# JianCao92/speaker-diarization

Measured on AMD Instinct MI355X. Metric: diarized audio throughput (CD gw/BIC + CL hi/BIC), higher is better.
Workload: dtype f64

## Files before the change

### include/spkd.h

```cpp
#ifndef SPKD_H
#define SPKD_H

#include <stddef.h>
#include <stdint.h>

#ifdef __cplusplus
extern "C" {
#endif

#define SPKD_ABI_VERSION 2
#define SPKD_DIM 39
#define SPKD_REC 820

typedef enum {
    SPKD_OK = 0,
    SPKD_EINVAL = 1,
    SPKD_EHIP = 2,
    SPKD_ENONFINITE = 3,
    SPKD_EOVERFLOW = 4,
    SPKD_ENOMEM = 5
} spkd_status;

typedef enum { SPKD_BIC = 0, SPKD_GLR = 1, SPKD_KL2 = 2, SPKD_KL2_PINV = 3 } spkd_kind;

// ... 73 lines not shown
                    int32_t *h_n_win, double *h_win_maxd, int32_t *h_win_det,
                    double *h_det_start, double *h_det_maxi, double *h_det_d,
                    double *h_final_start,
                    spkd_cand_log *h_log, int64_t log_cap, int64_t *h_log_count);

spkd_status spkd_gw_ex(spkd_ctx *ctx, const float *d_frames, int64_t n_frames,
                       const int64_t *h_turn_begin, const int64_t *h_turn_end, int64_t n_turns,
                       const spkd_cd_params *params, const int64_t *h_ev_off, int check_capacity,
                       int32_t *h_n_win, double *h_win_maxd, int32_t *h_win_det,
                       double *h_det_start, double *h_det_maxi, double *h_det_d,
                       double *h_final_start,
                       spkd_cand_log *h_log, int64_t log_cap, int64_t *h_log_count);

spkd_status spkd_gw_fused(spkd_ctx *ctx, const float *d_frames, int64_t n_frames,
                          const int64_t *h_turn_begin, const int64_t *h_turn_end, int64_t n_turns,
                          const spkd_cd_params *params, const int64_t *h_ev_off, int check_capacity,
                          int32_t *h_n_win, double *h_win_maxd, int32_t *h_win_det,
                          double *h_det_start, double *h_det_maxi, double *h_det_d,
                          double *h_final_start, double *d_seg_stats,
                          spkd_cand_log *h_log, int64_t log_cap, int64_t *h_log_count);

spkd_status spkd_gather_stats(spkd_ctx *ctx, const double *d_src, int64_t n_src,
                              const int64_t *h_src_index, const int64_t *h_dst_index,
                              int64_t n, int64_t n_dst, double *d_dst);

typedef struct {
    int64_t n_lines;
    int64_t n_redo;
    const int32_t *n_win;
    const double *times;
    const int32_t *turn;
    const int64_t *frame_b;
    const int64_t *frame_e;
    const int64_t *index;
    const int64_t *d_index;
    const int64_t *redo_line;
    const int64_t *redo_begin;
    const int64_t *redo_end;
} spkd_gw_lines_view;

spkd_status spkd_gw_batch(spkd_ctx *ctx, const float *d_frames, int64_t n_frames,
                          const int64_t *h_turn_begin, const int64_t *h_turn_end, int64_t n_turns,
                          const spkd_cd_params *params, const int64_t *h_ev_off,
                          const double *h_turn_start_s, const double *h_turn_end_s,
                          const int64_t *h_turn_file_off, const int64_t *h_turn_file_len,
                          double *d_seg_stats, int want_index, spkd_gw_lines_view *view);

int64_t spkd_sw_window_count(int64_t turn_len, double winsize, double winstep);
spkd_status spkd_sw(spkd_ctx *ctx, const float *d_frames, int64_t n_frames,
                    const int64_t *h_turn_begin, const int64_t *h_turn_end, int64_t n_turns,
                    const spkd_cd_params *params, const int64_t *h_d_off, double *h_d);

enum { SPKD_AHC_AUTO = 0, SPKD_AHC_MONO = 1, SPKD_AHC_WIDE = 2 };

typedef struct {
    int32_t variant;
    int32_t kind;
    int32_t max_spk;
    int32_t path;
    double lambdac;
    double threshold;
} spkd_ahc_params;

spkd_status spkd_ahc(spkd_ctx *ctx, const double *d_stats, const int64_t *h_seg_off,
                     int64_t n_problems, const spkd_ahc_params *params,
                     int32_t *h_n_merges, int32_t *h_merge_a, int32_t *h_merge_b,
                     double *h_merge_d, double *h_stat_max, double *h_stat_min);

spkd_status spkd_ahc_matrix(spkd_ctx *ctx, const double *d_stats, int64_t n, const spkd_ahc_params *params,
                            const double *d_matrix, double stat_max_in, double stat_min_in,
                            int32_t *h_n_merges, int32_t *h_merge_a, int32_t *h_merge_b,
                            double *h_merge_d, double *h_stat_max, double *h_stat_min);

spkd_status spkd_ahc_fused(spkd_ctx *ctx, const float *d_frames, int64_t n_frames,
                           const double *d_records, int64_t n_records, int64_t *d_line_index,
                           const int64_t *h_seg_off, int64_t n_problems,
                           const int64_t *h_redo_line, const int64_t *h_redo_begin,
                           const int64_t *h_redo_end, int64_t n_redo,
                           const spkd_ahc_params *params,
                           const int32_t **h_n_merges, const int32_t **h_merge_a,
                           const int32_t **h_merge_b, const double **h_merge_d,
                           const int32_t **h_labels);

typedef struct {
    int32_t sample_rate, frame_rate, window_width, n_fft, n_mel, n_cep;
    int32_t cms_left, cms_right;
    int32_t delta_width[2];
    float pre_emph;
    float delta_norm[2];
} spkd_mfcc_params;
spkd_status spkd_mfcc(spkd_ctx *ctx, const int16_t *d_pcm, int64_t n_samples,
                      const spkd_mfcc_params *params, const float *h_melfb, const float *h_dct,
                      const float *h_mean, const float *h_scale, const float *h_transform,
                      float *d_features, int64_t *h_n_frames);

typedef struct {
    int32_t n_kernels, n_states, dim;
    const float *mean;
    const float *inv_var;
    const float *log_norm;
    const int32_t *state_off;
    const int32_t *kernel;
    const float *log_weight;
} spkd_gmm_params;
spkd_status spkd_gmm_loglik(spkd_ctx *ctx, const float *d_features, int64_t n_frames,
                            const spkd_gmm_params *params, float *d_scores);

void spkd_py2_roundtrip(double *h_values, int64_t n);
spkd_status spkd_labels_from_merges(int64_t n, int64_t n_merges, const int32_t *h_a,
                                    const int32_t *h_b, int32_t *h_labels);
spkd_status spkd_labels_from_merges_batch(int64_t n_problems, const int64_t *h_seg_off,
                                          const int32_t *h_n_merges, const int32_t *h_a,
                                          const int32_t *h_b, int32_t *h_labels);

spkd_status spkd_count_flags(const int32_t *h_flags, const int64_t *h_off, const int32_t *h_n,
                             int64_t n_groups, int32_t *h_out);

spkd_status spkd_gw_lines(int64_t n_turns, const int64_t *h_off, const int32_t *h_n_det,
                          const double *h_det_start, const double *h_det_maxi,
                          const double *h_final_start, const double *h_turn_start_s,
                          const double *h_turn_end_s, const int64_t *h_turn_begin,
                          const int64_t *h_turn_end, double rate, int text_contract,
                          int64_t n_lines, double *h_times, int64_t *h_frame_b,
                          int64_t *h_frame_e, int64_t *h_index, int32_t *h_line_turn);

spkd_status spkd_vad_viterbi(int64_t n_frames, int32_t n_states, const float *h_scores,
                             int32_t n_words, const int32_t *h_word_state, const double *h_stay,
                             const double *h_exit, const double *h_enter, int64_t *h_tok_frame,
                             int32_t *h_tok_word, int64_t *h_n_tokens, double *h_score);

#ifdef __cplusplus
}
#endif
#endif
```

### speaker-diarization_amd/csrc/spkd_cluster.hpp

```cpp
#pragma once
#include "spkd_device.hpp"
#include "spkd_quad.hpp"
#include "spkd_tri.hpp"
#include "../../include/spkd.h"

namespace spkd {

constexpr double MAXINT_F = 9223372036854775808.0;
constexpr double PEN_UNIT = 39.0 + 0.5 * 39.0 * 40.0;
constexpr int AUX = 3 * DA;
constexpr int ERR_DEGENERATE_MERGE = 2;

__device__ __forceinline__ unsigned long long dkey(double v) {
    unsigned long long b = (unsigned long long)__double_as_longlong(v);
    return (b >> 63) ? ~b : (b | 0x8000000000000000ull);
}
__device__ __forceinline__ double dkey_inv(unsigned long long k) {
    unsigned long long b = (k >> 63) ? (k & 0x7fffffffffffffffull) : ~k;
    return __longlong_as_double((long long)b);
}
template <bool MAXOP>
__device__ __forceinline__ unsigned wave_red_u32(unsigned x) {
    auto op = [](unsigned a, unsigned b) { return MAXOP ? (a > b ? a : b) : (a < b ? a : b); };
    x = op(x, (unsigned)__builtin_amdgcn_update_dpp((int)x, (int)x, 0xB1, 0xf, 0xf, false));
// ... 271 lines not shown
    const int lane = lane_id();
    const int64_t pair = (int64_t)blockIdx.x * PT2_WAVES + wave;
    if (pair >= n_pairs) return;
    double* ldsA = slabs[wave][0];
    double* ldsB = slabs[wave][1];
    const double* A = stats + (int64_t)ia[pair] * REC;
    const double* B = stats + (int64_t)ib[pair] * REC;
    const double n1 = A[REC - 1], n2 = B[REC - 1];
    const double n = n1 + n2;
    const QuadLane L = quad_lane();
    int ta = L.t;
    asm volatile("" : "+v"(ta));
    QuadRows q;
    double sc[QS];
    quad_load_packed(B, ta, q, sc);
    quad_from_packed_lds(ldsA, A, lane);
    quad_from_packed_lds(ldsB, B, lane);
    const bool want_glr = (flags & SPKD_WANT_GLR) != 0;
    const int mode = (L.m == 3 && !want_glr) ? 2 : L.m;
    double wa, wc, k1a, k1c, w1, k2c, w2;
    {
        const double fA = 1.0 / (n1 - 1.0), fB = 1.0 / (n2 - 1.0), fU = 1.0 / (n - 1.0);
        const double al1 = (n1 / n) / (n1 - 1.0), al2 = (n2 / n) / (n2 - 1.0);
        wa = mode == 0 ? fA : (mode == 1 ? 0.0 : (mode == 2 ? fU : al1));
        wc = mode == 0 ? 0.0 : (mode == 1 ? fB : (mode == 2 ? fU : al2));
        k1a = mode == 1 ? 0.0 : 1.0;
        k1c = (mode == 1 || mode == 2) ? 1.0 : 0.0;
        w1 = mode == 0 ? -(fA / n1) : (mode == 1 ? -(fB / n2) : (mode == 2 ? -(fU / n) : -(al1 / n1)));
        k2c = mode == 3 ? 1.0 : 0.0;
        w2 = mode == 3 ? -(al2 / n2) : 0.0;
    }
    double v1[QS], v2[QS], c1[QS], c2[QS];
#pragma unroll
    for (int s = 0; s < QS; ++s) {
#pragma unroll
        for (int j = 0; j < tri_cols(s); ++j)
            q.r[s][j] = fma(wa, ldsA[(s * DA + j) * 16 + ta], wc * q.r[s][j]);
        const double sa = ldsA[(s * DA + D) * 16 + ta];
        v1[s] = fma(k1c, sc[s], k1a * sa);
        v2[s] = k2c * sc[s];
        c1[s] = w1 * v1[s];
        c2[s] = w2 * v2[s];
        __builtin_amdgcn_sched_barrier(0);
    }
    TriRank1<0>::run(q, c1, v1);
    TriRank1<0>::run(q, c2, v2);
    auto form_single = [&](int mi, double (&a)[DA]) {
        const int md = (mi == 3 && !want_glr) ? 2 : mi;
        if (md == 0) single_pair_matrix(SPKD_BIC, ldsA, ldsA, true, a);
        else if (md == 1) single_pair_matrix(SPKD_BIC, ldsB, ldsB, true, a);
        else single_pair_matrix(md == 2 ? SPKD_BIC : SPKD_GLR, ldsA, ldsB, false, a);
    };
    const double ld = log(tri_det(q, L.m, err, form_single));
    double res[4];
#pragma unroll
    for (int mi = 0; mi < 4; ++mi) res[mi] = __shfl(ld, 16 * mi);
    double kl = __builtin_nan("");
    if (flags & SPKD_WANT_KL2) {
        double* slab = ldsA;
        double a[DA];
        double ds[2], dp[2], mu[2];
#pragma unroll 1
        for (int t = 0; t < 2; ++t) {
            stage1(slab, t ? B : A);
            row_from_slab(slab, a);
            const double nn = t ? n2 : n1;
            const double mean_i = a[D] / nn;
            cov_rows(a, nn);
            kl2_lane_terms(a, mean_i, ds[t], dp[t], mu[t], pinv_ws);
        }
        kl = kl2_combine(ds[0], dp[0], mu[0], ds[1], dp[1], mu[1]);
    }
    if (lane == 0) {
        double* o = out + pair * 8;
        o[0] = n1; o[1] = n2; o[2] = res[0]; o[3] = res[1]; o[4] = res[2];
        o[5] = want_glr ? res[3] : __builtin_nan("");
        o[6] = kl; o[7] = 0.0;
    }
}

__global__ __launch_bounds__(PT_WAVES * WAVE) void k_cluster_prep(
        const double* __restrict__ qr, int64_t n_rec, int kind,
        double* __restrict__ ld, double* __restrict__ aux, int* err,
        double* pinv_ws) {
    const int wave = threadIdx.x >> 6;
    const int64_t w = (int64_t)blockIdx.x * PT_WAVES + wave;
    if (kind == SPKD_KL2) {
        if (w >= n_rec) return;
        const double* R = qr + w * QREC;
        double a[DA];
        single_rows_from_qr(R, a);
        const double n = qr_count(R);
        const double mean_i = a[D] / n;
        cov_rows(a, n);
        kl2_aux_from_cov(a, mean_i, aux + w * AUX, pinv_ws);
        if (lane_id() == 0) ld[w] = 0.0;
        return;
    }
    if (w * 4 >= n_rec) return;
    const QuadLane L = quad_lane();
    const double* recs[4];
    bool selfs[4];
#pragma unroll
    for (int mi = 0; mi < 4; ++mi) {
        int64_t c = w * 4 + mi;
        c = c < n_rec ? c : n_rec - 1;
        recs[mi] = qr + c * QREC;
        selfs[mi] = true;
    }
    int64_t c = w * 4 + L.m;
    const bool valid = c < n_rec;
    c = valid ? c : n_rec - 1;
    const double* R = qr + c * QREC;
    QuadRows q;
    double sv[QS];
    const double nR = qr_count(R), fR = fast_recip(nR - 1.0);
    quad_load_scaled(R, L.t, fR, q, sv);
    double c1[QS];
    const double gR = -(fR * fast_recip(nR));
#pragma unroll
    for (int s = 0; s < QS; ++s) c1[s] = gR * sv[s];
    TriRank1<0>::run(q, c1, sv);
    auto form_single = [&](int mi, double (&a)[DA]) { single_pair_matrix(kind, recs[mi], recs[mi], true, a); };
    const double v = tri_logdet(q, L.m, err, form_single);
    if (valid && L.t == 0) ld[c] = v;
}

__device__ __forceinline__ double finish_distance(int kind, double lambdac, double nA, double ldA,
                                                  double nC, double ldC, double ldx) {
#pragma clang fp contract(off)
    const double n = nA + nC;
    if (kind == SPKD_BIC) {
        double d = 0.5 * n * ldx - 0.5 * nA * ldA - 0.5 * nC * ldC;
        d -= lambdac * 0.5 * PEN_UNIT * log(n);
        return d;
    }
    return -(n / 2.0) * ((nA / n) * ldA + (nC / n) * ldC - ldx);
}

__device__ __forceinline__ int find_problem(const int64_t* __restrict__ seg_off, int64_t n_prob, int64_t g) {
    int64_t lo = 0, hi = n_prob;
    while (hi - lo > 1) {
        int64_t mid = (lo + hi) >> 1;
        if (seg_off[mid] <= g) lo = mid; else hi = mid;
    }
    return (int)lo;
}

#ifndef SPKD_MX_WAVES
#define SPKD_MX_WAVES 4
#endif
constexpr int MX_WAVES = SPKD_MX_WAVES;

template <bool TWO>
__global__ __launch_bounds__(MX_WAVES * WAVE, 2) void k_matrix(
        const double* __restrict__ ex, const double* __restrict__ pk, const int64_t* __restrict__ seg_off,
        const int32_t* __restrict__ rec_prob, const int32_t* __restrict__ sched, int variant, int kind, double lambdac,
        const double* __restrict__ ld, const double* __restrict__ aux,
        double* __restrict__ mat, const int64_t* __restrict__ mat_off,
        unsigned long long* stat_max, unsigned long long* stat_min, int* err) {
    __shared__ double ldsA[QREC];
    const int64_t g = sched[blockIdx.x];
    if (g < 0) return;
    const int p = rec_prob[g];
    const int64_t off = seg_off[p];
    const int64_t N = seg_off[p + 1] - off;
    const int64_t ra = g - off;
// ... 1053 lines not shown
```

### speaker-diarization_amd/csrc/spkd_handoff.hpp

```cpp
#pragma once
#include "spkd_cd.hpp"
#include "spkd_cluster.hpp"
#include "spkd_device.hpp"

namespace spkd {

__host__ __device__ inline int32_t count_detections(const int32_t* flags, int64_t n_win) {
    int32_t cnt = 0;
    for (int64_t i = 0; i < n_win; ++i) cnt += flags[i] != 0;
    return cnt;
}

struct RecipeLine {
    double start_s, end_s;
    int64_t frame_b, frame_e;
    int64_t index;
};

__host__ __device__ inline RecipeLine recipe_line(int64_t begin, int64_t len, int64_t ev_off, int64_t j, int64_t nd,
                                                  const double* det_start, const double* det_maxi,
                                                  const double* final_start, double ls, double le, double rate) {
#pragma clang fp contract(off)
    RecipeLine L;
    const bool tail = j == nd;
    double fs, fe;
    if (tail) {
        fs = *final_start;
        L.start_s = fs / rate + ls;
        L.end_s = ((le - ls) * rate) / rate + ls;
        fe = 0.0;
    } else {
        fs = det_start[ev_off + j];
        fe = fs + det_maxi[ev_off + j];
        L.start_s = fs / rate + ls;
        L.end_s = fe / rate + ls;
    }
    L.frame_b = begin + (int64_t)fs;
    L.frame_e = tail ? begin + len : begin + (int64_t)fe;
    L.index = ev_off + j;
    return L;
}

constexpr int CP_TPB = 256;
constexpr int CP_SCAN_TPB = 1024;

__global__ __launch_bounds__(CP_TPB) void k_cp_count(const TurnDesc* __restrict__ turns, int64_t n_turns,
                                                     const int32_t* __restrict__ n_win,
                                                     const int32_t* __restrict__ win_det, const int* __restrict__ err,
                                                     int32_t* __restrict__ n_det, int32_t* __restrict__ pos) {
    if (*err) return;
    const int64_t p = (int64_t)blockIdx.x * CP_TPB + threadIdx.x;
    if (p >= n_turns) return;
    const TurnDesc T = turns[p];
    int64_t nw = n_win[T.id];
    nw = nw < 0 ? 0 : (nw > T.ev_cap ? T.ev_cap : nw);
    n_det[T.id] = count_detections(win_det + T.ev_off, nw);
    pos[T.id] = (int32_t)p;
}

__global__ __launch_bounds__(CP_SCAN_TPB) void k_cp_scan(const int32_t* __restrict__ n_det, int64_t n_turns,
                                                         const int* __restrict__ err, int64_t* __restrict__ line_off) {
    __shared__ int64_t part[CP_SCAN_TPB];
    const int tid = threadIdx.x;
    if (*err) {
        if (tid == 0) line_off[n_turns] = 0;
        return;
    }
    const int64_t per = (n_turns + CP_SCAN_TPB - 1) / CP_SCAN_TPB;
    const int64_t lo = tid * per < n_turns ? tid * per : n_turns;
    const int64_t hi = lo + per < n_turns ? lo + per : n_turns;
    int64_t sum = 0;
    for (int64_t t = lo; t < hi; ++t) sum += (int64_t)n_det[t] + 1;
    part[tid] = sum;
    __syncthreads();
    for (int d = 1; d < CP_SCAN_TPB; d <<= 1) {
        const int64_t v = tid >= d ? part[tid - d] : 0;
        __syncthreads();
        part[tid] += v;
        __syncthreads();
    }
    int64_t run = part[tid] - sum;
    for (int64_t t = lo; t < hi; ++t) {
        line_off[t] = run;
        run += (int64_t)n_det[t] + 1;
    }
    if (tid == CP_SCAN_TPB - 1) line_off[n_turns] = part[tid];
}

__global__ __launch_bounds__(CP_TPB) void k_cp_lines(const TurnDesc* __restrict__ turns, int64_t n_turns,
                                                     const int32_t* __restrict__ n_det, const int32_t* __restrict__ pos,
                                                     const int64_t* __restrict__ line_off, int64_t n_lines,
                                                     const double* __restrict__ det_start,
                                                     const double* __restrict__ det_maxi,
                                                     const double* __restrict__ final_start,
                                                     const double* __restrict__ turn_start_s,
                                                     const double* __restrict__ turn_end_s, double rate,
                                                     const int* __restrict__ err, double* __restrict__ times,
                                                     int64_t* __restrict__ frame_b, int64_t* __restrict__ frame_e,
                                                     int64_t* __restrict__ index, int32_t* __restrict__ line_turn) {
    if (*err) return;
    const int64_t t = (int64_t)blockIdx.x * CP_TPB + threadIdx.x;
    if (t >= n_turns) return;
    const TurnDesc T = turns[pos[t]];
    const int64_t nd = n_det[t];
    const double ls = turn_start_s[t], le = turn_end_s[t];
    int64_t i = line_off[t];
    for (int64_t j = 0; j <= nd && i < n_lines; ++j, ++i) {
        const RecipeLine L = recipe_line(T.begin, T.len, T.ev_off, j, nd, det_start, det_maxi, final_start + t, ls, le, rate);
        times[2 * i] = L.start_s;
        times[2 * i + 1] = L.end_s;
        frame_b[i] = L.frame_b;
        frame_e[i] = L.frame_e;
        index[i] = L.index;
        line_turn[i] = (int32_t)t;
    }
}

__global__ __launch_bounds__(256) void k_patch_map(const int64_t* __restrict__ line, int64_t n, int64_t* __restrict__ map) {
    const int64_t k = (int64_t)blockIdx.x * 256 + threadIdx.x;
    if (k < n) map[line[k]] = -(k + 1);
}

__global__ __launch_bounds__(256) void k_records_from_map(const double* __restrict__ recs, int64_t n_recs,
                                                          const int64_t* __restrict__ map,
                                                          const double* __restrict__ redo, int64_t n_redo,
                                                          int64_t n_rec, double* __restrict__ qr,
                                                          double* __restrict__ packed, int* __restrict__ err) {
    const int64_t c = blockIdx.x;
    if (c >= n_rec) return;
    const int64_t m = map[c];
    const double* g;
    if (m >= 0 && m < n_recs) {
        g = recs + m * REC;
    } else if (m < 0 && -(m + 1) < n_redo) {
        g = redo + (-(m + 1)) * REC;
    } else {
        if (threadIdx.x == 0) atomicOr(err, 4);
        return;
    }
    quadrec_from_packed(g, qr + c * QREC, threadIdx.x);
    double* p = packed + c * REC;
    for (int e = threadIdx.x; e < REC; e += 256) p[e] = g[e];
}

__global__ __launch_bounds__(256) void k_gather_records(const double* __restrict__ src, const int64_t* __restrict__ si,
                                                        const int64_t* __restrict__ di, int64_t n,
                                                        double* __restrict__ dst) {
    const int64_t i = blockIdx.x;
    if (i >= n) return;
    const double2* s = reinterpret_cast<const double2*>(src + si[i] * REC);
    double2* d = reinterpret_cast<double2*>(dst + (di ? di[i] : i) * REC);
    for (int e = threadIdx.x; e < REC / 2; e += 256) d[e] = s[e];
}

__global__ __launch_bounds__(256) void k_take_pair_distance(const double* __restrict__ mat, int64_t n, double* __restrict__ out) {
    const int64_t p = (int64_t)blockIdx.x * 256 + threadIdx.x;
    if (p < n) out[p] = mat[4 * p + 1];
}

}
```

### speaker-diarization_amd/csrc/spkd_hip.hip

```cpp
#include <hip/hip_runtime.h>

#include <algorithm>
#include <cmath>
#include <cstdio>
#include <cstdlib>
#include <cstring>
#include <string>
#include <atomic>
#include <thread>
#include <vector>

#include "../../include/spkd.h"
#include "spkd_cd.hpp"
#include "spkd_cluster.hpp"
#include "spkd_device.hpp"
#include "spkd_handoff.hpp"
#include "spkd_stats.hpp"
#include "spkd_mfcc.hpp"
#include "spkd_vad.hpp"

using namespace spkd;

namespace {
constexpr int N_SLOTS = 40;
enum { PIN_GW_TURNS = 0, PIN_GW_LINES, PIN_AHC_OUT, N_PIN };
}

struct spkd_ctx {
    int device = 0;
    hipStream_t stream = nullptr;
    bool own_stream = false;
    bool gw_lds_ok = false;
    int gw_waves = 0;
    unsigned long long init_keys[2] = {0ull, ~0ull};
    int step_waves = 0;
    int step_partners = 0;
    int64_t last_gw_items = 0;
    std::string err;
    int* d_err = nullptr;
    unsigned long long* d_counter = nullptr;
    hipEvent_t ev0 = nullptr, ev1 = nullptr;
    float last_ms = 0.f;
    hipEvent_t ka[SPKD_N_TIMERS] = {}, kb[SPKD_N_TIMERS] = {};
    bool kused[SPKD_N_TIMERS] = {};
    float kms[SPKD_N_TIMERS] = {};
    void* slot[N_SLOTS] = {};
    size_t slot_bytes[N_SLOTS] = {};
    void* pinv_ws = nullptr;
    double* pinv_cur = nullptr;
    void* pin[N_PIN] = {};
    size_t pin_bytes[N_PIN] = {};
    std::vector<int64_t> redo_line, redo_begin, redo_end;
    std::vector<Chunk> redo_chunks;
    std::vector<int64_t> redo_setoff;
    std::vector<int32_t> redo_sets;
};

namespace {

spkd_status fail(spkd_ctx* c, spkd_status s, const std::string& msg) {
    if (c) c->err = msg;
    return s;
}

#define HIPCHK(c, call)                                                              \
    do {                                                                             \
        hipError_t e_ = (call);                                                      \
        if (e_ != hipSuccess)                                                        \
            return fail((c), SPKD_EHIP, std::string(#call) + ": " + hipGetErrorString(e_)); \
    } while (0)

#define TRY(expr) do { const spkd_status s_ = (expr); if (s_ != SPKD_OK) return s_; } while (0)

spkd_status scratch(spkd_ctx* c, int slot, size_t bytes, void** out) {
    if (bytes == 0) bytes = 16;
    if (c->slot_bytes[slot] < bytes) {
        if (c->slot[slot]) HIPCHK(c, hipFree(c->slot[slot]));
        c->slot[slot] = nullptr;
        c->slot_bytes[slot] = 0;
        size_t want = bytes + bytes / 4;
        hipError_t e = hipMalloc(&c->slot[slot], want);
        if (e != hipSuccess) {
            want = bytes;
            e = hipMalloc(&c->slot[slot], want);
        }
        if (e != hipSuccess) return fail(c, SPKD_ENOMEM, "scratch allocation failed");
        c->slot_bytes[slot] = want;
    }
    *out = c->slot[slot];
    return SPKD_OK;
}

spkd_status pinned(spkd_ctx* c, int which, size_t bytes, void** out) {
    if (bytes == 0) bytes = 16;
    if (c->pin_bytes[which] < bytes) {
        if (c->pin[which]) HIPCHK(c, hipHostFree(c->pin[which]));
        c->pin[which] = nullptr;
        c->pin_bytes[which] = 0;
        const size_t want = bytes + bytes / 4;
        if (hipHostMalloc(&c->pin[which], want, hipHostMallocDefault) != hipSuccess) {
            c->pin[which] = nullptr;
            return fail(c, SPKD_ENOMEM, "pinned host allocation failed");
        }
        c->pin_bytes[which] = want;
    }
    *out = c->pin[which];
    return SPKD_OK;
}

template <class T>
spkd_status upload(spkd_ctx* c, int slot, const T* h, size_t n, T** d) {
    void* p = nullptr;
    TRY(scratch(c, slot, n * sizeof(T), &p));
    if (n) HIPCHK(c, hipMemcpyAsync(p, h, n * sizeof(T), hipMemcpyHostToDevice, c->stream));
    *d = (T*)p;
    return SPKD_OK;
}

struct Call {
    spkd_ctx* const c;
    spkd_status opened;
    int herr = 0;
    bool drained = false;
    explicit Call(spkd_ctx* ctx) : c(ctx) { opened = open(); }
    ~Call() { if (!drained) (void)hipStreamSynchronize(c->stream); }
    spkd_status open() {
        HIPCHK(c, hipSetDevice(c->device));
        for (int i = 0; i < SPKD_N_TIMERS; ++i) c->kused[i] = false;
        HIPCHK(c, hipMemsetAsync(c->d_err, 0, sizeof(int), c->stream));
        HIPCHK(c, hipEventRecord(c->ev0, c->stream));
        return SPKD_OK;
    }

    spkd_status finish() {
        HIPCHK(c, hipEventRecord(c->ev1, c->stream));
        HIPCHK(c, hipMemcpyAsync(&herr, c->d_err, sizeof(int), hipMemcpyDeviceToHost, c->stream));
        HIPCHK(c, hipStreamSynchronize(c->stream));
        drained = true;
        HIPCHK(c, hipEventElapsedTime(&c->last_ms, c->ev0, c->ev1));
        c->kms[0] = c->last_ms;
        for (int i = 1; i < SPKD_N_TIMERS; ++i)
            if (c->kused[i]) HIPCHK(c, hipEventElapsedTime(&c->kms[i], c->ka[i], c->kb[i]));
        if (herr & ERR_SWEEP) return fail(c, SPKD_EHIP, "internal error: growing-window sweep order");
        if (herr & 4) return fail(c, SPKD_EOVERFLOW, "device scratch capacity exceeded");
        if (herr & ERR_DEGENERATE_MERGE) return fail(c, SPKD_EINVAL, "degenerate merge: a diagonal cell was the minimum");
        if (herr & ERR_NONFINITE) return fail(c, SPKD_ENONFINITE, "array must not contain infs or NaNs");
        return SPKD_OK;
    }
};

spkd_status use_kind(spkd_ctx* c, int kind, int* base) {
    c->pinv_cur = nullptr;
    *base = kind;
    if (kind != SPKD_KL2_PINV) return SPKD_OK;
    *base = SPKD_KL2;
    if (!c->pinv_ws) {
        if (hipMalloc(&c->pinv_ws, PINV_WS_BYTES) != hipSuccess) {
            c->pinv_ws = nullptr;
            return fail(c, SPKD_ENOMEM, "pinv workspace allocation failed");
        }
        HIPCHK(c, hipMemsetAsync(c->pinv_ws, 0, PINV_LOCK_BYTES, c->stream));
    }
    c->pinv_cur = (double*)c->pinv_ws;
    return SPKD_OK;
}

struct Timer {
    spkd_ctx* const c;
    const int idx;
    Timer(spkd_ctx* ctx, int i) : c(ctx), idx(i) { (void)hipEventRecord(c->ka[idx], c->stream); }
    ~Timer() { (void)hipEventRecord(c->kb[idx], c->stream); c->kused[idx] = true; }
};

enum {
    S_CHUNKS = 0, S_SETOFF, S_PARTIAL, S_IDXA, S_IDXB, S_TERMS, S_TURNS, S_SNAP, S_CAND,
    S_EV_I32A, S_EV_I32B, S_EV_D0, S_EV_D1, S_EV_D2, S_EV_D3, S_EV_D4, S_LOG,
    S_AHC_STATS, S_AHC_LD, S_AHC_AUX, S_AHC_MAT, S_AHC_MISC, S_AHC_OUT, S_AHC_OFF, S_AHC_PROB, S_AHC_PACKED, S_MFCC_TAB, S_MFCC_STATIC,
    S_STEP_EXM, S_STEP_PKM, S_STEP_MISC, S_GMM_TAB, S_GMM_IDX,
    S_CP_TURNS, S_CP_TIMES, S_CP_LINES, S_REDO_STATS, S_REDO_IDX, S_COUNT
};
static_assert(S_COUNT <= N_SLOTS, "scratch slot table too small");

}

extern "C" {

int spkd_abi_version(void) { return SPKD_ABI_VERSION; }

static spkd_status create_ctx(int device, void* stream, bool borrow, spkd_ctx** out) {
    if (!out) return SPKD_EINVAL;
    *out = nullptr;
    int count = 0;
    if (hipGetDeviceCount(&count) != hipSuccess || device < 0 || device >= count) return SPKD_EHIP;
    spkd_ctx* c = new spkd_ctx();
    c->device = device;
    if (hipSetDevice(device) != hipSuccess) { delete c; return SPKD_EHIP; }
    if (borrow) {
        c->stream = (hipStream_t)stream;
    } else {
        if (hipStreamCreateWithFlags(&c->stream, hipStreamDefault) != hipSuccess) { delete c; return SPKD_EHIP; }
        c->own_stream = true;
    }
    if (hipMalloc(&c->d_err, sizeof(int)) != hipSuccess ||
        hipMalloc(&c->d_counter, 2 * sizeof(unsigned long long)) != hipSuccess ||
        hipEventCreate(&c->ev0) != hipSuccess || hipEventCreate(&c->ev1) != hipSuccess) {
        spkd_destroy(c);
        return SPKD_EHIP;
    }
    for (int i = 0; i < SPKD_N_TIMERS; ++i)
        if (hipEventCreate(&c->ka[i]) != hipSuccess || hipEventCreate(&c->kb[i]) != hipSuccess) {
            spkd_destroy(c);
            return SPKD_EHIP;
        }
    int lds_max = 0;
    c->gw_lds_ok = hipDeviceGetAttribute(&lds_max, hipDeviceAttributeMaxSharedMemoryPerBlock, device) == hipSuccess &&
                   Gw<4>::LDS_BYTES <= lds_max &&
                   hipFuncSetAttribute((const void*)k_gw<8>, hipFuncAttributeMaxDynamicSharedMemorySize, Gw<8>::LDS_BYTES) == hipSuccess &&
                   hipFuncSetAttribute((const void*)k_gw<4>, hipFuncAttributeMaxDynamicSharedMemorySize, Gw<4>::LDS_BYTES) == hipSuccess &&
                   hipFuncSetAttribute((const void*)k_gw<2>, hipFuncAttributeMaxDynamicSharedMemorySize, Gw<2>::LDS_BYTES) == hipSuccess &&
                   hipFuncSetAttribute((const void*)k_gw<1>, hipFuncAttributeMaxDynamicSharedMemorySize, Gw<1>::LDS_BYTES) == hipSuccess;
    if (const char* e = getenv("SPKD_GW_WAVES")) c->gw_waves = atoi(e);
    if (const char* e = getenv("SPKD_STEP_WAVES")) { const int v = atoi(e); c->step_waves = (v == 4 || v == 8) ? v : 0; }
    if (const char* e = getenv("SPKD_STEP_PARTNERS")) { const int v = atoi(e); c->step_partners = (v == 3 || v == 7 || v == 15) ? v : 0; }
    *out = c;
    return SPKD_OK;
}

spkd_status spkd_create(int device, void* stream, spkd_ctx** out) {
    return create_ctx(device, stream, stream != nullptr, out);
}

spkd_status spkd_create_on_stream(int device, void* stream, spkd_ctx** out) {
    return create_ctx(device, stream, true, out);
}

void spkd_destroy(spkd_ctx* c) {
    if (!c) return;
    (void)hipSetDevice(c->device);
    if (c->stream) (void)hipStreamSynchronize(c->stream);
    for (int i = 0; i < N_SLOTS; ++i)
        if (c->slot[i]) (void)hipFree(c->slot[i]);
    if (c->d_err) (void)hipFree(c->d_err);
    if (c->pinv_ws) (void)hipFree(c->pinv_ws);
    for (int i = 0; i < N_PIN; ++i)
        if (c->pin[i]) (void)hipHostFree(c->pin[i]);
    if (c->d_counter) (void)hipFree(c->d_counter);
    if (c->ev0) (void)hipEventDestroy(c->ev0);
    if (c->ev1) (void)hipEventDestroy(c->ev1);
    for (int i = 0; i < SPKD_N_TIMERS; ++i) {
        if (c->ka[i]) (void)hipEventDestroy(c->ka[i]);
        if (c->kb[i]) (void)hipEventDestroy(c->kb[i]);
    }
    if (c->own_stream && c->stream) (void)hipStreamDestroy(c->stream);
    delete c;
}

const char* spkd_last_error(const spkd_ctx* c) { return c ? c->err.c_str() : "null context"; }

spkd_status spkd_sync(spkd_ctx* c) {
    if (!c) return SPKD_EINVAL;
    HIPCHK(c, hipStreamSynchronize(c->stream));
    return SPKD_OK;
}

spkd_status spkd_malloc(spkd_ctx* c, size_t bytes, void** d_ptr) {
    if (!c || !d_ptr) return SPKD_EINVAL;
    HIPCHK(c, hipSetDevice(c->device));
    hipError_t e = hipMalloc(d_ptr, bytes ? bytes : 16);
    if (e != hipSuccess) return fail(c, SPKD_ENOMEM, hipGetErrorString(e));
    return SPKD_OK;
}

spkd_status spkd_free(spkd_ctx* c, void* d_ptr) {
    if (!c) return SPKD_EINVAL;
    HIPCHK(c, hipFree(d_ptr));
    return SPKD_OK;
}

spkd_status spkd_memcpy_h2d(spkd_ctx* c, void* d_dst, const void* h_src, size_t bytes) {
    if (!c) return SPKD_EINVAL;
    HIPCHK(c, hipMemcpyAsync(d_dst, h_src, bytes, hipMemcpyHostToDevice, c->stream));
    HIPCHK(c, hipStreamSynchronize(c->stream));
    return SPKD_OK;
}

spkd_status spkd_memcpy_d2h(spkd_ctx* c, void* h_dst, const void* d_src, size_t bytes) {
    if (!c) return SPKD_EINVAL;
    HIPCHK(c, hipMemcpyAsync(h_dst, d_src, bytes, hipMemcpyDeviceToHost, c->stream));
    HIPCHK(c, hipStreamSynchronize(c->stream));
    return SPKD_OK;
}

spkd_status spkd_memcpy_d2d(spkd_ctx* c, void* d_dst, const void* d_src, size_t bytes) {
    if (!c) return SPKD_EINVAL;
    HIPCHK(c, hipMemcpyAsync(d_dst, d_src, bytes, hipMemcpyDeviceToDevice, c->stream));
    HIPCHK(c, hipStreamSynchronize(c->stream));
    return SPKD_OK;
}

spkd_status spkd_last_gw_items(spkd_ctx* c, int64_t* items) {
    if (!c || !items) return SPKD_EINVAL;
    *items = c->last_gw_items;
    return SPKD_OK;
}

spkd_status spkd_last_kernel_ms(spkd_ctx* c, int which, float* ms) {
    if (!c || !ms || which < 0 || which >= SPKD_N_TIMERS) return SPKD_EINVAL;
    *ms = c->kms[which];
    return SPKD_OK;
}

namespace {
spkd_status set_stats_launch(spkd_ctx* c, const float* d_frames, int64_t n_frames,
                             const int64_t* h_begin, const int64_t* h_end, const int32_t* h_set,
                             int64_t n_ranges, int64_t n_sets, double* d_stats,
                             std::vector<Chunk>& chunks, std::vector<int64_t>& set_off) {
    chunks.clear();
    set_off.assign((size_t)n_sets + 1, 0);
    int32_t prev = 0;
    for (int64_t r = 0; r < n_ranges; ++r) {
        const int64_t b = h_begin[r], e = h_end[r];
        const int32_t s = h_set[r];
        if (b < 0 || e < b || e > n_frames || s < prev || s >= n_sets)
            return fail(c, SPKD_EINVAL, "bad frame range or set id");
        prev = s;
        for (int64_t t = b; t < e; t += STATS_CHUNK) {
            Chunk ch;
            ch.begin = t;
            ch.len = (int32_t)std::min<int64_t>(STATS_CHUNK, e - t);
// ... 59 lines not shown
        hipLaunchKernelGGL(k_pair_terms, dim3(blocks), dim3(PT2_WAVES * WAVE), 0, c->stream,
                           d_stats, d_a, d_b, n_pairs, flags, (double*)d_terms, c->d_err, c->pinv_cur);
    }
    HIPCHK(c, hipGetLastError());
    HIPCHK(c, hipMemcpyAsync(h_terms, d_terms, (size_t)n_pairs * 8 * sizeof(double), hipMemcpyDeviceToHost, c->stream));
    return call.finish();
}

namespace {
struct AhcBuffers {
    double* ex;
    double* pk;
    double* ld;
    double* aux;
    double* mat;
    int64_t* seg_off;
    int64_t* mat_off;
    unsigned long long* smax;
    unsigned long long* smin;
};

unsigned long long host_dkey(double v) {
    unsigned long long b;
    std::memcpy(&b, &v, sizeof b);
    return (b >> 63) ? ~b : (b | 0x8000000000000000ull);
}

struct MatrixPlan {
    const double* d_init = nullptr;
    double init_max = NAN, init_min = NAN;
    int64_t row_begin = -1, row_end = -1;
    int64_t* d_map = nullptr;
    int64_t n_src = 0;
    const float* d_frames = nullptr;
    int64_t n_frames = 0;
    const int64_t *redo_line = nullptr, *redo_begin = nullptr, *redo_end = nullptr;
    int64_t n_redo = 0;
};

spkd_status ahc_prepare(spkd_ctx* c, const double* d_stats, const int64_t* h_seg_off, int64_t n_prob,
                        int variant, int kind, double lambdac, AhcBuffers& B, int64_t& n_total,
                        std::vector<int64_t>& offs, std::vector<int32_t>& prob_of,
                        const MatrixPlan& plan = MatrixPlan()) {
    n_total = h_seg_off[n_prob];
    offs.clear();
    offs.insert(offs.end(), h_seg_off, h_seg_off + n_prob + 1);
    int64_t cells = 0;
    for (int64_t p = 0; p < n_prob; ++p) {
        const int64_t n = h_seg_off[p + 1] - h_seg_off[p];
        if (n < 0) return fail(c, SPKD_EINVAL, "seg_off must be non-decreasing");
        offs.push_back(cells);
        cells += n * n;
    }
    offs.push_back(cells);
    prob_of.assign((size_t)n_total, 0);
    for (int64_t p = 0; p < n_prob; ++p)
        for (int64_t r = h_seg_off[p]; r < h_seg_off[p + 1]; ++r) prob_of[(size_t)r] = (int32_t)p;
    int64_t grid_rows = 0;
    {
        const int X = 8;
        std::vector<std::vector<int32_t>> lists(X);
        if (plan.row_begin >= 0) {
            for (int64_t r = plan.row_begin; r < plan.row_end; ++r) lists[(size_t)((r - plan.row_begin) % X)].push_back((int32_t)r);
        } else if (n_prob >= X) {
            std::vector<int64_t> order((size_t)n_prob);
            for (int64_t p = 0; p < n_prob; ++p) order[(size_t)p] = p;
            std::stable_sort(order.begin(), order.end(), [&](int64_t a, int64_t b) {
                return h_seg_off[a + 1] - h_seg_off[a] > h_seg_off[b + 1] - h_seg_off[b];
            });
            double load[X] = {0, 0, 0, 0, 0, 0, 0, 0};
            for (int64_t p : order) {
                int x = 0;
                for (int i = 1; i < X; ++i) if (load[i] < load[x]) x = i;
                const double n = (double)(h_seg_off[p + 1] - h_seg_off[p]);
                load[x] += n * n;
                for (int64_t r = h_seg_off[p]; r < h_seg_off[p + 1]; ++r) lists[x].push_back((int32_t)r);
            }
        } else {
            for (int64_t r = 0; r < n_total; ++r) lists[(size_t)(r % X)].push_back((int32_t)r);
        }
        size_t longest = 0;
        for (auto& l : lists) longest = std::max(longest, l.size());
        grid_rows = (int64_t)longest * X;
        prob_of.resize((size_t)(n_total + grid_rows), -1);
        for (int x = 0; x < X; ++x)
            for (size_t i = 0; i < lists[x].size(); ++i) prob_of[(size_t)n_total + i * X + x] = lists[x][i];
    }
    int64_t* d_offs = nullptr;
    int32_t* d_prob = nullptr;
    TRY(upload(c, S_AHC_OFF, offs.data(), offs.size(), &d_offs));
    TRY(upload(c, S_AHC_PROB, prob_of.data(), prob_of.size(), &d_prob));
    B.seg_off = d_offs;
    B.mat_off = d_offs + n_prob + 1;
    void* p = nullptr;
    TRY(scratch(c, S_AHC_LD, (size_t)n_total * sizeof(double), &p));
    B.ld = (double*)p;
    TRY(scratch(c, S_AHC_AUX, (size_t)n_total * AUX * sizeof(double), &p));
    B.aux = (double*)p;
    TRY(scratch(c, S_AHC_MAT, (size_t)cells * sizeof(double), &p));
    B.mat = (double*)p;
    TRY(scratch(c, S_AHC_MISC, (size_t)n_prob * 2 * sizeof(unsigned long long), &p));
    B.smax = (unsigned long long*)p;
    B.smin = B.smax + n_prob;
    HIPCHK(c, hipMemsetAsync(B.smax, 0x00, (size_t)n_prob * sizeof(unsigned long long), c->stream));
    HIPCHK(c, hipMemsetAsync(B.smin, 0xff, (size_t)n_prob * sizeof(unsigned long long), c->stream));
    if (plan.d_init && n_prob == 1) {
        c->init_keys[0] = plan.init_max == plan.init_max ? host_dkey(plan.init_max) : 0ull;
        c->init_keys[1] = plan.init_min == plan.init_min ? host_dkey(plan.init_min) : ~0ull;
        HIPCHK(c, hipMemcpyAsync(B.smax, &c->init_keys[0], sizeof(unsigned long long), hipMemcpyHostToDevice, c->stream));
        HIPCHK(c, hipMemcpyAsync(B.smin, &c->init_keys[1], sizeof(unsigned long long), hipMemcpyHostToDevice, c->stream));
    }
    TRY(scratch(c, S_AHC_STATS, (size_t)n_total * QREC * sizeof(double), &p));
    B.ex = (double*)p;
    TRY(scratch(c, S_AHC_PACKED, (size_t)n_total * REC * sizeof(double), &p));
    B.pk = (double*)p;
    if (n_total > 0) {
        if (plan.d_map) {
            void* d_redo = nullptr;
            if (plan.n_redo > 0) {
                int64_t* d_rl = nullptr;
                TRY(scratch(c, S_REDO_STATS, (size_t)plan.n_redo * REC * sizeof(double), &d_redo));
                TRY(upload(c, S_REDO_IDX, plan.redo_line, (size_t)plan.n_redo, &d_rl));
                c->redo_sets.resize((size_t)plan.n_redo);
                for (int64_t k = 0; k < plan.n_redo; ++k) c->redo_sets[(size_t)k] = (int32_t)k;
                TRY(set_stats_launch(c, plan.d_frames, plan.n_frames, plan.redo_begin, plan.redo_end, c->redo_sets.data(),
                                     plan.n_redo, plan.n_redo, (double*)d_redo, c->redo_chunks, c->redo_setoff));
                hipLaunchKernelGGL(k_patch_map, dim3((unsigned)((plan.n_redo + 255) / 256)), dim3(256), 0, c->stream,
                                   (const int64_t*)d_rl, plan.n_redo, plan.d_map);
            }
            hipLaunchKernelGGL(k_records_from_map, dim3((unsigned)n_total), dim3(256), 0, c->stream, d_stats, plan.n_src,
                               (const int64_t*)plan.d_map, (const double*)d_redo, plan.n_redo, n_total, B.ex, B.pk, c->d_err);
        } else {
            hipLaunchKernelGGL(k_to_quadrec, dim3((unsigned)n_total), dim3(256), 0, c->stream, d_stats, n_total, B.ex);
            HIPCHK(c, hipMemcpyAsync(B.pk, d_stats, (size_t)n_total * REC * sizeof(double), hipMemcpyDeviceToDevice, c->stream));
        }
        const int64_t per_block = kind == SPKD_KL2 ? PT_WAVES : 4 * PT_WAVES;
        const unsigned blocks = (unsigned)((n_total + per_block - 1) / per_block);
        {
            Timer t(c, SPKD_T_CLUSTER_PREP);
            hipLaunchKernelGGL(k_cluster_prep, dim3(blocks), dim3(PT_WAVES * WAVE), 0, c->stream,
                               (const double*)B.ex, n_total, kind, B.ld, B.aux, c->d_err, c->pinv_cur);
        }
        auto kmat = kind == SPKD_GLR ? k_matrix<true> : k_matrix<false>;
        if (plan.d_init) {
            HIPCHK(c, hipMemcpyAsync(B.mat, plan.d_init, (size_t)cells * sizeof(double), hipMemcpyDeviceToDevice, c->stream));
        } else if (grid_rows > 0) {
            Timer t(c, SPKD_T_MATRIX);
            hipLaunchKernelGGL(kmat, dim3((unsigned)grid_rows), dim3(MX_WAVES * WAVE), 0, c->stream,
                               (const double*)B.ex, (const double*)B.pk, (const int64_t*)B.seg_off, (const int32_t*)d_prob,
                               (const int32_t*)d_prob + n_total, variant, kind, lambdac,
                               (const double*)B.ld, (const double*)B.aux, B.mat, (const int64_t*)B.mat_off,
                               B.smax, B.smin, c->d_err);
        }
    }
    HIPCHK(c, hipGetLastError());
    return SPKD_OK;
}

double key_to_double(unsigned long long k, bool is_max) {
    if (is_max ? (k == 0ull) : (k == ~0ull)) return std::nan("");
    unsigned long long b = (k >> 63) ? (k & 0x7fffffffffffffffull) : ~k;
    double v;
    std::memcpy(&v, &b, sizeof v);
    return v;
}
}

spkd_status spkd_distance_matrix(spkd_ctx* c, int kind, double lambdac, const double* d_stats,
                                 int64_t n, double* d_matrix) {
    if (!c || n < 0 || kind < 0 || kind > 3) return SPKD_EINVAL;
    if (n == 0) return SPKD_OK;
    if (!d_stats || !d_matrix) return fail(c, SPKD_EINVAL, "null argument");
    const int64_t seg_off[2] = {0, n};
    AhcBuffers B;
    int64_t n_total = 0;
    std::vector<int64_t> offs;
    std::vector<int32_t> prob_of;
    Call call(c);
    TRY(call.opened);
    TRY(use_kind(c, kind, &kind));
    TRY(ahc_prepare(c, d_stats, seg_off, 1, 1, kind, lambdac, B, n_total, offs, prob_of));
    HIPCHK(c, hipMemcpyAsync(d_matrix, B.mat, (size_t)n * n * sizeof(double), hipMemcpyDeviceToDevice, c->stream));
    return call.finish();
}

spkd_status spkd_cluster_in(spkd_ctx* c, const double* d_stats, int64_t n, int kind, double lambdac, double threshold,
                            int32_t* h_label, double* h_dist, int64_t dist_cap, int64_t* h_dist_off,
                            int64_t* h_n_done, int64_t* h_n_clusters) {
    if (!c || n < 0 || dist_cap < 0 || kind < 0 || kind > 3) return SPKD_EINVAL;
    if (h_n_done) *h_n_done = 0;
    if (h_n_clusters) *h_n_clusters = 0;
    if (n == 0) return SPKD_OK;
    if (!d_stats || !h_label || !h_dist_off || !h_n_done || !h_n_clusters || (dist_cap > 0 && !h_dist))
        return fail(c, SPKD_EINVAL, "null argument");
    long long done2[2] = {0, 0};
    Call call(c);
    TRY(call.opened);
    TRY(use_kind(c, kind, &kind));
    void *p_ex = nullptr, *p_ld = nullptr, *p_aux = nullptr, *p_cex = nullptr, *p_cpk = nullptr, *p_misc = nullptr, *p_dist = nullptr;
    const size_t nn = (size_t)n;
    TRY(scratch(c, S_AHC_STATS, nn * QREC * sizeof(double), &p_ex));
    TRY(scratch(c, S_AHC_LD, nn * sizeof(double), &p_ld));
    TRY(scratch(c, S_AHC_AUX, nn * AUX * sizeof(double), &p_aux));
    TRY(scratch(c, S_STEP_EXM, nn * QREC * sizeof(double), &p_cex));
    TRY(scratch(c, S_STEP_PKM, nn * REC * sizeof(double), &p_cpk));
    const size_t misc_bytes = (2 + AUX) * nn * sizeof(double) + (nn + 1 + 2) * sizeof(long long) + nn * sizeof(int32_t) + 64;
    TRY(scratch(c, S_STEP_MISC, misc_bytes, &p_misc));
    TRY(scratch(c, S_AHC_MAT, (size_t)std::max<int64_t>(dist_cap, 1) * sizeof(double), &p_dist));
    double* clu_ld = (double*)p_misc;
    double* tmp = clu_ld + nn;
    double* clu_aux = tmp + nn;
    long long* d_off = (long long*)(clu_aux + nn * AUX);
    long long* d_done = d_off + nn + 1;
    int32_t* d_label = (int32_t*)(d_done + 2);
    HIPCHK(c, hipMemsetAsync(d_done, 0, 2 * sizeof(long long), c->stream));
    hipLaunchKernelGGL(k_to_quadrec, dim3((unsigned)n), dim3(256), 0, c->stream, d_stats, n, (double*)p_ex);
    {
        const int64_t per_block = 4 * PT_WAVES;
        const unsigned blocks = (unsigned)((n + per_block - 1) / per_block);
        {
            Timer t(c, SPKD_T_CLUSTER_PREP);
            hipLaunchKernelGGL(k_cluster_prep, dim3(blocks), dim3(PT_WAVES * WAVE), 0, c->stream,
                               (const double*)p_ex, n, kind == SPKD_KL2 ? (int)SPKD_BIC : kind, (double*)p_ld, (double*)p_aux, c->d_err,
                               c->pinv_cur);
        }
        if (kind == SPKD_KL2) {
            void* p_ld2 = nullptr;
            TRY(scratch(c, S_AHC_OUT, nn * sizeof(double), &p_ld2));
            const unsigned blocks1 = (unsigned)((n + PT_WAVES - 1) / PT_WAVES);
            hipLaunchKernelGGL(k_cluster_prep, dim3(blocks1), dim3(PT_WAVES * WAVE), 0, c->stream,
                               (const double*)p_ex, n, (int)SPKD_KL2, (double*)p_ld2, (double*)p_aux, c->d_err, c->pinv_cur);
        }
    }
    auto kin = kind == SPKD_GLR ? k_cluster_in<true> : k_cluster_in<false>;
    {
        Timer t(c, SPKD_T_AHC);
        hipLaunchKernelGGL(kin, dim3(1), dim3(CIN_TPB), 0, c->stream,
                           (const double*)p_ex, d_stats, (const double*)p_ld, (const double*)p_aux, (long long)n, kind, lambdac, threshold,
                           (double*)p_cex, (double*)p_cpk, clu_ld, clu_aux, tmp, d_label, (double*)p_dist, (long long)dist_cap,
                           d_off, d_done, c->d_err, c->pinv_cur);
    }
    HIPCHK(c, hipGetLastError());
    HIPCHK(c, hipMemcpyAsync(done2, d_done, sizeof done2, hipMemcpyDeviceToHost, c->stream));
    HIPCHK(c, hipMemcpyAsync(h_label, d_label, nn * sizeof(int32_t), hipMemcpyDeviceToHost, c->stream));
    HIPCHK(c, hipMemcpyAsync(h_dist_off, d_off, (nn + 1) * sizeof(long long), hipMemcpyDeviceToHost, c->stream));
    if (dist_cap > 0)
        HIPCHK(c, hipMemcpyAsync(h_dist, p_dist, (size_t)dist_cap * sizeof(double), hipMemcpyDeviceToHost, c->stream));
    const spkd_status st = call.finish();
    *h_n_done = done2[0];
    *h_n_clusters = done2[1];
    return st;
}

spkd_status spkd_distance_rows(spkd_ctx* c, int variant, int kind, double lambdac, const double* d_stats,
                               int64_t n, int64_t row_begin, int64_t row_end, double* d_rows,
                               double* h_stat_max, double* h_stat_min) {
    if (!c || n < 0 || kind < 0 || kind > 3 || (variant != 1 && variant != 2)) return SPKD_EINVAL;
    if (row_begin < 0 || row_end < row_begin || row_end > n) return fail(c, SPKD_EINVAL, "distance_rows: bad row block");
    if (h_stat_max) *h_stat_max = std::nan("");
    if (h_stat_min) *h_stat_min = std::nan("");
    if (n == 0 || row_end == row_begin) return SPKD_OK;
    if (!d_stats || !d_rows) return fail(c, SPKD_EINVAL, "null argument");
    const int64_t seg_off[2] = {0, n};
    AhcBuffers B;
    int64_t n_total = 0;
    std::vector<int64_t> offs;
    std::vector<int32_t> prob_of;
    MatrixPlan plan;
    plan.row_begin = row_begin;
    plan.row_end = row_end;
    unsigned long long keys[2] = {0ull, ~0ull};
    Call call(c);
    TRY(call.opened);
    TRY(use_kind(c, kind, &kind));
    TRY(ahc_prepare(c, d_stats, seg_off, 1, variant, kind, lambdac, B, n_total, offs, prob_of, plan));
    HIPCHK(c, hipMemcpyAsync(d_rows, B.mat + row_begin * n, (size_t)(row_end - row_begin) * n * sizeof(double),
                             hipMemcpyDeviceToDevice, c->stream));
    HIPCHK(c, hipMemcpyAsync(&keys[0], B.smax, sizeof(unsigned long long), hipMemcpyDeviceToHost, c->stream));
    HIPCHK(c, hipMemcpyAsync(&keys[1], B.smin, sizeof(unsigned long long), hipMemcpyDeviceToHost, c->stream));
    const spkd_status st = call.finish();
    if (h_stat_max) *h_stat_max = key_to_double(keys[0], true);
    if (h_stat_min) *h_stat_min = key_to_double(keys[1], false);
    return st;
}

namespace {
spkd_status ahc_impl(spkd_ctx* c, const double* d_stats, const int64_t* h_seg_off, int64_t n_prob,
                     const spkd_ahc_params* P, const MatrixPlan& plan, int32_t* h_n_merges, int32_t* h_merge_a,
                     int32_t* h_merge_b, double* h_merge_d, double* h_stat_max, double* h_stat_min) {
    if (!c || !P || n_prob < 0) return SPKD_EINVAL;
    if (n_prob == 0) return SPKD_OK;
    if (!d_stats || !h_seg_off || !h_n_merges || !h_merge_a || !h_merge_b || !h_merge_d ||
        !h_stat_max || !h_stat_min)
        return fail(c, SPKD_EINVAL, "null argument");
    if ((P->variant != 1 && P->variant != 2) || P->kind < 0 || P->kind > 3)
        return fail(c, SPKD_EINVAL, "bad variant / kind");
    for (int64_t p = 0; p < n_prob; ++p)
        if (h_seg_off[p + 1] - h_seg_off[p] < 1) return fail(c, SPKD_EINVAL, "empty clustering problem");
    int64_t n_max = 0;
    for (int64_t p = 0; p < n_prob; ++p) n_max = std::max<int64_t>(n_max, h_seg_off[p + 1] - h_seg_off[p]);
    if (n_max > AHC_MAX_N) return fail(c, SPKD_EINVAL, "clustering problem larger than 65536 records");
    int path = P->path;
    if (path != SPKD_AHC_MONO && path != SPKD_AHC_WIDE) path = n_prob <= 64 ? SPKD_AHC_WIDE : SPKD_AHC_MONO;
    const size_t lds = (size_t)(n_max + 4) * sizeof(int32_t);
    if (path == SPKD_AHC_MONO && lds > 150 * 1024) path = SPKD_AHC_WIDE;
    if (path == SPKD_AHC_WIDE && n_max > STEP_MAX_N)
        return fail(c, SPKD_EINVAL, "clustering problem larger than 16384 records (wide merge loop)");
    AhcBuffers B;
    int64_t n_total = 0;
    std::vector<int64_t> offs;
    std::vector<int32_t> prob_of;
    std::vector<unsigned long long> kmax((size_t)n_prob), kmin((size_t)n_prob);
    std::vector<double> fmax((size_t)n_prob), fmin((size_t)n_prob);
    Call call(c);
// ... 186 lines not shown
};

spkd_status gw_batch_upload(spkd_ctx* c, GwBatch& G, int64_t n_turns) {
    const size_t nt = (size_t)n_turns;
    void *p = nullptr, *h = nullptr;
    TRY(scratch(c, S_CP_TURNS, nt * (2 * sizeof(double) + 2 * sizeof(int32_t)) + (nt + 1) * sizeof(int64_t), &p));
    G.d_ls = (double*)p;
    G.d_le = G.d_ls + nt;
    G.d_line_off = (int64_t*)(G.d_le + nt);
    G.d_n_det = (int32_t*)(G.d_line_off + nt + 1);
    G.d_pos = G.d_n_det + nt;
    HIPCHK(c, hipMemcpyAsync(G.d_ls, G.turn_start_s, nt * sizeof(double), hipMemcpyHostToDevice, c->stream));
    HIPCHK(c, hipMemcpyAsync(G.d_le, G.turn_end_s, nt * sizeof(double), hipMemcpyHostToDevice, c->stream));
    TRY(pinned(c, PIN_GW_TURNS, 2 * sizeof(int64_t) + nt * sizeof(int32_t), &h));
    G.h_head = (int64_t*)h;
    G.h_n_win = (int32_t*)(G.h_head + 2);
    return SPKD_OK;
}

spkd_status gw_batch_compact(spkd_ctx* c, GwBatch& G, const TurnDesc* d_turns, int64_t n_turns,
                             const int32_t* d_n_win, const int32_t* d_win_det, const double* d_det_start,
                             const double* d_det_maxi, const double* d_final_start, double rate) {
    const unsigned blocks = (unsigned)((n_turns + CP_TPB - 1) / CP_TPB);
    hipLaunchKernelGGL(k_cp_count, dim3(blocks), dim3(CP_TPB), 0, c->stream, d_turns, n_turns, d_n_win, d_win_det,
                       (const int*)c->d_err, G.d_n_det, G.d_pos);
    hipLaunchKernelGGL(k_cp_scan, dim3(1), dim3(CP_SCAN_TPB), 0, c->stream, (const int32_t*)G.d_n_det, n_turns,
                       (const int*)c->d_err, G.d_line_off);
    HIPCHK(c, hipGetLastError());
    G.h_head[0] = 0;
    G.h_head[1] = 0;
    HIPCHK(c, hipMemcpyAsync(&G.h_head[0], G.d_line_off + n_turns, sizeof(int64_t), hipMemcpyDeviceToHost, c->stream));
    HIPCHK(c, hipMemcpyAsync(&G.h_head[1], c->d_err, sizeof(int), hipMemcpyDeviceToHost, c->stream));
    HIPCHK(c, hipMemcpyAsync(G.h_n_win, d_n_win, (size_t)n_turns * sizeof(int32_t), hipMemcpyDeviceToHost, c->stream));
    HIPCHK(c, hipStreamSynchronize(c->stream));
    if (G.h_head[1] != 0) return SPKD_OK;
    const int64_t n = G.h_head[0];
    if (n < n_turns) return fail(c, SPKD_EHIP, "internal error: fewer lines than turns");
    const size_t nn = (size_t)n;
    void *d_t = nullptr, *d_l = nullptr, *h = nullptr;
    TRY(scratch(c, S_CP_TIMES, nn * 2 * sizeof(double), &d_t));
    TRY(scratch(c, S_CP_LINES, nn * (3 * sizeof(int64_t) + sizeof(int32_t)), &d_l));
    TRY(pinned(c, PIN_GW_LINES, nn * (2 * sizeof(double) + 3 * sizeof(int64_t) + sizeof(int32_t)), &h));
    int64_t* d_fb = (int64_t*)d_l;
    int64_t* d_ix = d_fb + 2 * nn;
    int32_t* d_tn = (int32_t*)(d_ix + nn);
    hipLaunchKernelGGL(k_cp_lines, dim3(blocks), dim3(CP_TPB), 0, c->stream, d_turns, n_turns,
                       (const int32_t*)G.d_n_det, (const int32_t*)G.d_pos, (const int64_t*)G.d_line_off, n, d_det_start,
                       d_det_maxi, d_final_start, (const double*)G.d_ls, (const double*)G.d_le, rate,
                       (const int*)c->d_err, (double*)d_t, d_fb, d_fb + nn, d_ix, d_tn);
    HIPCHK(c, hipGetLastError());
    double* h_times = (double*)h;
    int64_t* h_fb = (int64_t*)(h_times + 2 * nn);
    int64_t* h_ix = h_fb + 2 * nn;
    int32_t* h_tn = (int32_t*)(h_ix + nn);
    HIPCHK(c, hipMemcpyAsync(h_times, d_t, nn * 2 * sizeof(double), hipMemcpyDeviceToHost, c->stream));
    HIPCHK(c, hipMemcpyAsync(h_fb, d_fb, nn * 2 * sizeof(int64_t), hipMemcpyDeviceToHost, c->stream));
    HIPCHK(c, hipMemcpyAsync(h_tn, d_tn, nn * sizeof(int32_t), hipMemcpyDeviceToHost, c->stream));
    if (G.want_index)
        HIPCHK(c, hipMemcpyAsync(h_ix, d_ix, nn * sizeof(int64_t), hipMemcpyDeviceToHost, c->stream));
    spkd_gw_lines_view& V = *G.view;
    V.n_lines = n;
    V.n_win = G.h_n_win;
    V.times = h_times;
    V.turn = h_tn;
    V.frame_b = h_fb;
    V.frame_e = h_fb + nn;
    V.index = G.want_index ? h_ix : nullptr;
    V.d_index = d_ix;
    G.n_lines = n;
    G.have_lines = true;
    return SPKD_OK;
}

spkd_status gw_batch_finish(spkd_ctx* c, GwBatch& G, int64_t n_turns, double rate) {
    spkd_gw_lines_view& V = *G.view;
    double* times = const_cast<double*>(V.times);
    spkd_py2_roundtrip(times, 2 * V.n_lines);
    c->redo_line.clear();
    c->redo_begin.clear();
    c->redo_end.clear();
    for (int64_t i = 0; i < V.n_lines; ++i) {
        const int64_t t = V.turn[i];
        if (t < 0 || t >= n_turns) return fail(c, SPKD_EHIP, "internal error: line of no turn");
        const int64_t fn = G.file_len[t];
        int64_t a0 = (int64_t)(times[2 * i] * rate), a1 = (int64_t)(times[2 * i + 1] * rate);
        a0 = a0 < 0 ? 0 : (a0 > fn ? fn : a0);
        a1 = a1 < 0 ? 0 : (a1 > fn ? fn : a1);
        if (a1 < a0) a1 = a0;
        const int64_t b = G.file_off[t] + a0, e = G.file_off[t] + a1;
        if (b != V.frame_b[i] || e != V.frame_e[i]) {
            c->redo_line.push_back(i);
            c->redo_begin.push_back(b);
            c->redo_end.push_back(e);
        }
    }
    V.n_redo = (int64_t)c->redo_line.size();
    V.redo_line = c->redo_line.data();
    V.redo_begin = c->redo_begin.data();
    V.redo_end = c->redo_end.data();
    return SPKD_OK;
}

struct GwIn {
    const float* d_frames = nullptr;
    int64_t n_frames = 0, n_turns = 0;
    const int64_t *hb = nullptr, *he = nullptr, *h_ev_off = nullptr;
    const spkd_cd_params* P = nullptr;
    int check_capacity = 0;
    double* d_seg_stats = nullptr;
};
struct GwOut {
    int32_t *h_n_win = nullptr, *h_win_det = nullptr;
    double *h_win_maxd = nullptr, *h_det_start = nullptr, *h_det_maxi = nullptr, *h_det_d = nullptr,
           *h_final_start = nullptr;
    spkd_cand_log* h_log = nullptr;
    int64_t log_cap = 0;
    int64_t* h_log_count = nullptr;
};

constexpr int64_t GW_WAVE_PER_TURN_FROM = 4096;
constexpr int64_t GW_EIGHT_WAVES_UP_TO = 256;
spkd_status gw_impl(spkd_ctx* c, const GwIn& in, const GwOut& out, GwBatch* batch = nullptr) {
    const int64_t n_turns = in.n_turns, log_cap = out.log_cap;
    const spkd_cd_params* P = in.P;
    if (!c || !P || n_turns < 0) return SPKD_EINVAL;
    if (out.h_log_count) *out.h_log_count = 0;
    if (n_turns == 0) return SPKD_OK;
    if (!in.d_frames || !in.hb || !in.he || !in.h_ev_off) return fail(c, SPKD_EINVAL, "null argument");
    if (!batch && (!out.h_n_win || !out.h_win_maxd || !out.h_win_det || !out.h_det_start || !out.h_det_maxi ||
                   !out.h_det_d || !out.h_final_start))
        return fail(c, SPKD_EINVAL, "null argument");
    if (P->kind < 0 || P->kind > 3) return fail(c, SPKD_EINVAL, "gw: bad kind");
    if (!(P->rate >= 10.0) || !(P->winsize >= 1.0) || !(P->winstep >= 1.0))
        return fail(c, SPKD_EINVAL, "gw: rate >= 10, winsize >= 1 frame and winstep >= 1 frame required");
    if (log_cap < 0 || (log_cap > 0 && !out.h_log)) return fail(c, SPKD_EINVAL, "gw: log capacity without a log buffer");
    if (!c->gw_lds_ok) return fail(c, SPKD_EHIP, "gw: the kernel's dynamic LDS size was not admitted on this device");
    std::vector<TurnDesc> turns;
    int64_t n_cand;
    TRY(build_turns(c, in.n_frames, in.hb, in.he, n_turns, P, in.h_ev_off, true, turns, n_cand));
    for (int64_t t = 0; in.check_capacity && t < n_turns; ++t)
        if (turns[(size_t)t].ev_cap < spkd_gw_event_capacity_p(turns[(size_t)t].len, P))
            return fail(c, SPKD_EINVAL, "gw: event capacity too small, see spkd_gw_event_capacity_p");
    unsigned long long cnt2[2] = {0ull, 0ull};
    Call call(c);
    TRY(call.opened);
    spkd_cd_params Pk = *P;
    TRY(use_kind(c, P->kind, &Pk.kind));
    P = &Pk;
    const int64_t n_ev = in.h_ev_off[n_turns];
    TurnDesc* d_turns = nullptr;
    void *d_snap = nullptr, *d_cand = nullptr, *d_i32a = nullptr, *d_i32b = nullptr, *d_d0 = nullptr, *d_d1 = nullptr,
         *d_d2 = nullptr, *d_d3 = nullptr, *d_d4 = nullptr, *d_log = nullptr;
    TRY(upload(c, S_TURNS, turns.data(), turns.size(), &d_turns));
    TRY(scratch(c, S_SNAP, (size_t)n_cand * REC * sizeof(double), &d_snap));
    TRY(scratch(c, S_CAND, (size_t)n_cand * 4 * sizeof(double), &d_cand));
    TRY(scratch(c, S_EV_I32A, (size_t)n_turns * sizeof(int32_t), &d_i32a));
    TRY(scratch(c, S_EV_I32B, (size_t)n_ev * sizeof(int32_t), &d_i32b));
    TRY(scratch(c, S_EV_D0, (size_t)n_ev * sizeof(double), &d_d0));
    TRY(scratch(c, S_EV_D1, (size_t)n_ev * sizeof(double), &d_d1));
    TRY(scratch(c, S_EV_D2, (size_t)n_ev * sizeof(double), &d_d2));
    TRY(scratch(c, S_EV_D3, (size_t)n_ev * sizeof(double), &d_d3));
    TRY(scratch(c, S_EV_D4, (size_t)n_turns * sizeof(double), &d_d4));
    TRY(scratch(c, S_LOG, (size_t)std::max<int64_t>(log_cap, 1) * sizeof(spkd_cand_log), &d_log));
    if (!d_turns || !d_snap || !d_cand || !d_i32a || !d_i32b || !d_d0 || !d_d1 || !d_d2 || !d_d3 || !d_d4 ||
        !d_log || !c->d_counter || !c->d_err)
        return fail(c, SPKD_EHIP, "gw: a device scratch buffer is missing");
    HIPCHK(c, hipMemsetAsync(c->d_counter, 0, 2 * sizeof(unsigned long long), c->stream));
    if (batch) TRY(gw_batch_upload(c, *batch, n_turns));
    int nw = c->gw_waves;
    if (nw != 1 && nw != 2 && nw != 4 && nw != 8)
        nw = n_turns >= GW_WAVE_PER_TURN_FROM ? 1 : (n_turns <= GW_EIGHT_WAVES_UP_TO ? 8 : 4);
#define SPKD_GW_LAUNCH(NW_)                                                                                     \
    hipLaunchKernelGGL(k_gw<NW_>, dim3((unsigned)n_turns), dim3(Gw<NW_>::TPB), Gw<NW_>::LDS_BYTES, c->stream, \
                       in.d_frames, (const TurnDesc*)d_turns, *P, (double*)d_snap, (double*)d_cand,            \
                       (int32_t*)d_i32a, (double*)d_d0, (int32_t*)d_i32b, (double*)d_d1, (double*)d_d2,        \
                       (double*)d_d3, (double*)d_d4, in.d_seg_stats, (spkd_cand_log*)d_log, (long long)log_cap,   \
                       c->d_counter, c->d_err, c->pinv_cur)
    {
        Timer t(c, SPKD_T_GW);
        if (nw == 1) SPKD_GW_LAUNCH(1); else if (nw == 2) SPKD_GW_LAUNCH(2);
        else if (nw == 8) SPKD_GW_LAUNCH(8); else SPKD_GW_LAUNCH(4);
    }
#undef SPKD_GW_LAUNCH
    HIPCHK(c, hipGetLastError());
    unsigned long long& cnt = cnt2[0];
    if (batch) {
        TRY(gw_batch_compact(c, *batch, d_turns, n_turns, (const int32_t*)d_i32a, (const int32_t*)d_i32b,
                             (const double*)d_d1, (const double*)d_d2, (const double*)d_d4, P->rate));
        HIPCHK(c, hipMemcpyAsync(cnt2, c->d_counter, sizeof cnt2, hipMemcpyDeviceToHost, c->stream));
        const spkd_status st = call.finish();
        c->last_gw_items = (int64_t)cnt2[1];
        if (st != SPKD_OK) return st;
        if (!batch->have_lines) return fail(c, SPKD_EHIP, "internal error: no lines from a clean call");
        return gw_batch_finish(c, *batch, n_turns, P->rate);
    }
    HIPCHK(c, hipMemcpyAsync(out.h_n_win, d_i32a, (size_t)n_turns * sizeof(int32_t), hipMemcpyDeviceToHost, c->stream));
    HIPCHK(c, hipMemcpyAsync(out.h_win_maxd, d_d0, (size_t)n_ev * sizeof(double), hipMemcpyDeviceToHost, c->stream));
    HIPCHK(c, hipMemcpyAsync(out.h_win_det, d_i32b, (size_t)n_ev * sizeof(int32_t), hipMemcpyDeviceToHost, c->stream));
    HIPCHK(c, hipMemcpyAsync(out.h_det_start, d_d1, (size_t)n_ev * sizeof(double), hipMemcpyDeviceToHost, c->stream));
    HIPCHK(c, hipMemcpyAsync(out.h_det_maxi, d_d2, (size_t)n_ev * sizeof(double), hipMemcpyDeviceToHost, c->stream));
    HIPCHK(c, hipMemcpyAsync(out.h_det_d, d_d3, (size_t)n_ev * sizeof(double), hipMemcpyDeviceToHost, c->stream));
    HIPCHK(c, hipMemcpyAsync(out.h_final_start, d_d4, (size_t)n_turns * sizeof(double), hipMemcpyDeviceToHost, c->stream));
    HIPCHK(c, hipMemcpyAsync(cnt2, c->d_counter, sizeof cnt2, hipMemcpyDeviceToHost, c->stream));
    const spkd_status st = call.finish();
    c->last_gw_items = (int64_t)cnt2[1];
    if (out.h_log_count) *out.h_log_count = (int64_t)cnt;
    if (out.h_log && log_cap > 0 && cnt > 0) {
        const size_t ncopy = (size_t)std::min<int64_t>((int64_t)cnt, log_cap);
        HIPCHK(c, hipMemcpy(out.h_log, d_log, ncopy * sizeof(spkd_cand_log), hipMemcpyDeviceToHost));
    }
    if (st == SPKD_OK && (int64_t)cnt > log_cap && out.h_log)
        return fail(c, SPKD_EOVERFLOW, "candidate log too small");
    return st;
}
}

spkd_status spkd_gw(spkd_ctx* c, const float* d_frames, int64_t n_frames, const int64_t* hb,
                    const int64_t* he, int64_t n_turns, const spkd_cd_params* P, const int64_t* h_ev_off,
                    int32_t* h_n_win, double* h_win_maxd, int32_t* h_win_det, double* h_det_start,
                    double* h_det_maxi, double* h_det_d, double* h_final_start, spkd_cand_log* h_log,
                    int64_t log_cap, int64_t* h_log_count) {
    GwIn in;
    in.d_frames = d_frames; in.n_frames = n_frames; in.hb = hb; in.he = he; in.n_turns = n_turns;
    in.P = P; in.h_ev_off = h_ev_off; in.check_capacity = 1;
    GwOut out;
    out.h_n_win = h_n_win; out.h_win_maxd = h_win_maxd; out.h_win_det = h_win_det; out.h_det_start = h_det_start;
    out.h_det_maxi = h_det_maxi; out.h_det_d = h_det_d; out.h_final_start = h_final_start;
    out.h_log = h_log; out.log_cap = log_cap; out.h_log_count = h_log_count;
    return gw_impl(c, in, out);
}

spkd_status spkd_gw_ex(spkd_ctx* c, const float* d_frames, int64_t n_frames, const int64_t* hb,
                       const int64_t* he, int64_t n_turns, const spkd_cd_params* P, const int64_t* h_ev_off,
                       int check_capacity, int32_t* h_n_win, double* h_win_maxd, int32_t* h_win_det,
                       double* h_det_start, double* h_det_maxi, double* h_det_d, double* h_final_start,
                       spkd_cand_log* h_log, int64_t log_cap, int64_t* h_log_count) {
    GwIn in;
    in.d_frames = d_frames; in.n_frames = n_frames; in.hb = hb; in.he = he; in.n_turns = n_turns;
    in.P = P; in.h_ev_off = h_ev_off; in.check_capacity = check_capacity;
    GwOut out;
    out.h_n_win = h_n_win; out.h_win_maxd = h_win_maxd; out.h_win_det = h_win_det; out.h_det_start = h_det_start;
    out.h_det_maxi = h_det_maxi; out.h_det_d = h_det_d; out.h_final_start = h_final_start;
    out.h_log = h_log; out.log_cap = log_cap; out.h_log_count = h_log_count;
    return gw_impl(c, in, out);
}

spkd_status spkd_gw_fused(spkd_ctx* c, const float* d_frames, int64_t n_frames, const int64_t* hb,
                          const int64_t* he, int64_t n_turns, const spkd_cd_params* P, const int64_t* h_ev_off,
                          int check_capacity, int32_t* h_n_win, double* h_win_maxd, int32_t* h_win_det,
                          double* h_det_start, double* h_det_maxi, double* h_det_d, double* h_final_start,
                          double* d_seg_stats, spkd_cand_log* h_log, int64_t log_cap, int64_t* h_log_count) {
    if (c && !d_seg_stats) return fail(c, SPKD_EINVAL, "gw_fused: null statistics buffer");
    GwIn in;
    in.d_frames = d_frames; in.n_frames = n_frames; in.hb = hb; in.he = he; in.n_turns = n_turns;
    in.P = P; in.h_ev_off = h_ev_off; in.check_capacity = check_capacity; in.d_seg_stats = d_seg_stats;
    GwOut out;
    out.h_n_win = h_n_win; out.h_win_maxd = h_win_maxd; out.h_win_det = h_win_det; out.h_det_start = h_det_start;
    out.h_det_maxi = h_det_maxi; out.h_det_d = h_det_d; out.h_final_start = h_final_start;
    out.h_log = h_log; out.log_cap = log_cap; out.h_log_count = h_log_count;
    return gw_impl(c, in, out);
}

spkd_status spkd_gw_batch(spkd_ctx* c, const float* d_frames, int64_t n_frames, const int64_t* hb,
                          const int64_t* he, int64_t n_turns, const spkd_cd_params* P, const int64_t* h_ev_off,
                          const double* h_turn_start_s, const double* h_turn_end_s, const int64_t* h_turn_file_off,
                          const int64_t* h_turn_file_len, double* d_seg_stats, int want_index,
                          spkd_gw_lines_view* view) {
    if (!c || !view) return SPKD_EINVAL;
    std::memset(view, 0, sizeof *view);
    if (!d_seg_stats) return fail(c, SPKD_EINVAL, "gw_batch: null statistics buffer");
    if (n_turns > 0 && (!h_turn_start_s || !h_turn_end_s || !h_turn_file_off || !h_turn_file_len))
        return fail(c, SPKD_EINVAL, "gw_batch: null turn arrays");
    GwBatch G;
    G.turn_start_s = h_turn_start_s;
    G.turn_end_s = h_turn_end_s;
    G.file_off = h_turn_file_off;
    G.file_len = h_turn_file_len;
    G.want_index = want_index;
    G.view = view;
    GwIn in;
    in.d_frames = d_frames; in.n_frames = n_frames; in.hb = hb; in.he = he; in.n_turns = n_turns;
    in.P = P; in.h_ev_off = h_ev_off; in.d_seg_stats = d_seg_stats;
    const spkd_status st = gw_impl(c, in, GwOut(), &G);
    if (st != SPKD_OK) std::memset(view, 0, sizeof *view);
    return st;
}

spkd_status spkd_ahc_fused(spkd_ctx* c, const float* d_frames, int64_t n_frames, const double* d_records,
                           int64_t n_records, int64_t* d_line_index, const int64_t* h_seg_off, int64_t n_prob,
                           const int64_t* h_redo_line, const int64_t* h_redo_begin, const int64_t* h_redo_end,
                           int64_t n_redo, const spkd_ahc_params* P, const int32_t** h_n_merges,
                           const int32_t** h_merge_a, const int32_t** h_merge_b, const double** h_merge_d,
                           const int32_t** h_labels) {
    if (!c || !P || n_prob < 0 || n_redo < 0) return SPKD_EINVAL;
    if (!h_n_merges || !h_merge_a || !h_merge_b || !h_merge_d || !h_labels)
        return fail(c, SPKD_EINVAL, "ahc_fused: null output");
    *h_n_merges = *h_merge_a = *h_merge_b = *h_labels = nullptr;
    *h_merge_d = nullptr;
    if (n_prob == 0) return SPKD_OK;
    if (!d_records || !d_line_index || !h_seg_off || n_records < 1 || h_seg_off[0] != 0)
        return fail(c, SPKD_EINVAL, "ahc_fused: null argument or first offset not 0");
    for (int64_t p = 0; p < n_prob; ++p)
        if (h_seg_off[p + 1] < h_seg_off[p]) return fail(c, SPKD_EINVAL, "seg_off must be non-decreasing");
    const int64_t n_total = h_seg_off[n_prob];
    if (n_redo > 0 && (!h_redo_line || !h_redo_begin || !h_redo_end || !d_frames))
        return fail(c, SPKD_EINVAL, "ahc_fused: null redo arrays");
    for (int64_t k = 0; k < n_redo; ++k)
        if (h_redo_line[k] < 0 || h_redo_line[k] >= n_total || (k > 0 && h_redo_line[k] <= h_redo_line[k - 1]))
            return fail(c, SPKD_EINVAL, "ahc_fused: redo lines must be ascending line indices");
    const size_t nt = (size_t)n_total, np = (size_t)n_prob;
    void* h = nullptr;
    TRY(pinned(c, PIN_AHC_OUT, (nt + 2 * np) * sizeof(double) + (3 * nt + np) * sizeof(int32_t), &h));
    double* md = (double*)h;
    double* smax = md + nt;
    double* smin = smax + np;
    int32_t* ma = (int32_t*)(smin + np);
    int32_t* mb = ma + nt;
    int32_t* lab = mb + nt;
    int32_t* nm = lab + nt;
    MatrixPlan plan;
    plan.d_map = d_line_index;
    plan.n_src = n_records;
    plan.d_frames = d_frames;
    plan.n_frames = n_frames;
    plan.redo_line = h_redo_line;
    plan.redo_begin = h_redo_begin;
    plan.redo_end = h_redo_end;
    plan.n_redo = n_redo;
    TRY(ahc_impl(c, d_records, h_seg_off, n_prob, P, plan, nm, ma, mb, md, smax, smin));
    if (spkd_labels_from_merges_batch(n_prob, h_seg_off, nm, ma, mb, lab) != SPKD_OK)
        return fail(c, SPKD_EHIP, "internal error: merge log does not replay");
    *h_n_merges = nm;
    *h_merge_a = ma;
    *h_merge_b = mb;
    *h_merge_d = md;
    *h_labels = lab;
    return SPKD_OK;
}

spkd_status spkd_gather_stats(spkd_ctx* c, const double* d_src, int64_t n_src, const int64_t* h_src_index,
                              const int64_t* h_dst_index, int64_t n, int64_t n_dst, double* d_dst) {
    if (!c || n < 0) return SPKD_EINVAL;
    if (n == 0) return SPKD_OK;
    if (!d_src || !h_src_index || !d_dst) return fail(c, SPKD_EINVAL, "null argument");
    for (int64_t i = 0; i < n; ++i) {
        if (h_src_index[i] < 0 || h_src_index[i] >= n_src) return fail(c, SPKD_EINVAL, "gather: source index out of range");
        const int64_t d = h_dst_index ? h_dst_index[i] : i;
        if (d < 0 || d >= n_dst) return fail(c, SPKD_EINVAL, "gather: destination index out of range");
    }
    Call call(c);
    TRY(call.opened);
    int64_t *d_si = nullptr, *d_di = nullptr;
    TRY(upload(c, S_IDXA, h_src_index, (size_t)n, &d_si));
    if (h_dst_index) TRY(upload(c, S_IDXB, h_dst_index, (size_t)n, &d_di));
    hipLaunchKernelGGL(k_gather_records, dim3((unsigned)n), dim3(256), 0, c->stream, d_src,
                       (const int64_t*)d_si, (const int64_t*)d_di, n, d_dst);
    HIPCHK(c, hipGetLastError());
    return call.finish();
}

spkd_status spkd_sw(spkd_ctx* c, const float* d_frames, int64_t n_frames, const int64_t* hb,
                    const int64_t* he, int64_t n_turns, const spkd_cd_params* P, const int64_t* h_d_off,
                    double* h_d) {
    if (!c || !P || n_turns < 0) return SPKD_EINVAL;
    if (n_turns == 0) return SPKD_OK;
    if (!d_frames || !hb || !he || !h_d_off || !h_d) return fail(c, SPKD_EINVAL, "null argument");
    if (P->kind < 0 || P->kind > 3) return fail(c, SPKD_EINVAL, "bad kind");
    if (!(P->winsize >= 1.0) || !(P->winstep >= 1.0)) return fail(c, SPKD_EINVAL, "sw: window and step must be >= 1 frame");
    const int64_t n_d = h_d_off[n_turns];
    std::vector<int64_t> rb, re;
    std::vector<int32_t> rs;
    rb.reserve((size_t)(2 * n_d)); re.reserve((size_t)(2 * n_d)); rs.reserve((size_t)(2 * n_d));
    const int64_t wsz = (int64_t)P->winsize;
    for (int64_t t = 0; t < n_turns; ++t) {
        if (hb[t] < 0 || he[t] < hb[t] || he[t] > n_frames) return fail(c, SPKD_EINVAL, "bad turn range");
        const int64_t len = he[t] - hb[t];
        const int64_t W = spkd_sw_window_count(len, P->winsize, P->winstep);
        if (h_d_off[t + 1] - h_d_off[t] != W) return fail(c, SPKD_EINVAL, "sw: offsets do not match spkd_sw_window_count");
        for (int64_t w = 0; w < W; ++w) {
            const int64_t a = hb[t] + (int64_t)((double)w * P->winstep);
            const int32_t s0 = (int32_t)(2 * (h_d_off[t] + w));
            rb.push_back(a); re.push_back(a + wsz); rs.push_back(s0);
            rb.push_back(a + wsz); re.push_back(a + 2 * wsz); rs.push_back(s0 + 1);
        }
    }
    if (n_d == 0) return SPKD_OK;
    if (2 * n_d > 0x7fffffffLL) return fail(c, SPKD_EINVAL, "sw: too many windows in one call");
    std::vector<Chunk> chunks;
    std::vector<int64_t> set_off, offs;
    std::vector<int32_t> prob_of;
    Call call(c);
    TRY(call.opened);
    spkd_cd_params Pk = *P;
    TRY(use_kind(c, P->kind, &Pk.kind));
    P = &Pk;
    void *d_rec = nullptr, *d_out = nullptr;
    TRY(scratch(c, S_SNAP, (size_t)(2 * n_d) * REC * sizeof(double), &d_rec));
    TRY(scratch(c, S_EV_D0, (size_t)n_d * sizeof(double), &d_out));
    {
        Timer t(c, SPKD_T_SW);
        TRY(set_stats_launch(c, d_frames, n_frames, rb.data(), re.data(), rs.data(), 2 * n_d, 2 * n_d, (double*)d_rec,
                             chunks, set_off));
        std::vector<int64_t> seg_off((size_t)n_d + 1);
        for (int64_t w = 0; w <= n_d; ++w) seg_off[(size_t)w] = 2 * w;
        AhcBuffers B;
        int64_t n_total = 0;
        TRY(ahc_prepare(c, (const double*)d_rec, seg_off.data(), n_d, 1, P->kind, P->lambdac, B, n_total, offs, prob_of));
        hipLaunchKernelGGL(k_take_pair_distance, dim3((unsigned)((n_d + 255) / 256)), dim3(256), 0, c->stream,
                           (const double*)B.mat, n_d, (double*)d_out);
    }
    HIPCHK(c, hipGetLastError());
    HIPCHK(c, hipMemcpyAsync(h_d, d_out, (size_t)n_d * sizeof(double), hipMemcpyDeviceToHost, c->stream));
    return call.finish();
}

spkd_status spkd_mfcc(spkd_ctx* c, const int16_t* d_pcm, int64_t n_samples, const spkd_mfcc_params* P,
                      const float* h_melfb, const float* h_dct, const float* h_mean, const float* h_scale,
                      const float* h_transform, float* d_features, int64_t* h_n_frames) {
    if (!c || !P || !h_n_frames) return SPKD_EINVAL;
// ... 19 lines not shown
    if (!d_pcm || !d_features) return fail(c, SPKD_EINVAL, "mfcc: null device buffer");
    std::vector<float> tab;
    tab.insert(tab.end(), h_melfb, h_melfb + MF_MEL * MF_BINS);
    tab.insert(tab.end(), h_dct, h_dct + MF_CEP * MF_MEL);
    tab.insert(tab.end(), h_mean, h_mean + MF_DIM);
    tab.insert(tab.end(), h_scale, h_scale + MF_DIM);
    tab.insert(tab.end(), h_transform, h_transform + MF_DIM * MF_DIM);
    Call call(c);
    TRY(call.opened);
    float* d_tab = nullptr;
    void* d_static = nullptr;
    TRY(upload(c, S_MFCC_TAB, tab.data(), tab.size(), &d_tab));
    TRY(scratch(c, S_MFCC_STATIC, (size_t)T * MF_STATIC * sizeof(float), &d_static));
    const float* d_fb = d_tab;
    const float* d_dct = d_fb + MF_MEL * MF_BINS;
    const float* d_mean = d_dct + MF_CEP * MF_MEL;
    const float* d_scale = d_mean + MF_DIM;
    const float* d_tr = d_scale + MF_DIM;
    if (P->window_width == MF_WIN)
        hipLaunchKernelGGL(k_mfcc_static<MF_WIN>, dim3((unsigned)((T + MF_FR - 1) / MF_FR)), dim3(MF_TPB), 0, c->stream,
                           d_pcm, (long long)n_samples, (long long)T, hop, P->pre_emph, d_fb, d_dct, (float*)d_static);
    else
        hipLaunchKernelGGL(k_mfcc_static<MF_WIN_VAD>, dim3((unsigned)((T + MF_FR - 1) / MF_FR)), dim3(MF_TPB), 0,
                           c->stream, d_pcm, (long long)n_samples, (long long)T, hop, P->pre_emph, d_fb, d_dct,
                           (float*)d_static);
    hipLaunchKernelGGL(k_mfcc_post, dim3((unsigned)((T + MP_FR - 1) / MP_FR)), dim3(MF_TPB), lds, c->stream,
                       (const float*)d_static, (long long)T, P->cms_left, P->cms_right, P->delta_width[0],
                       P->delta_norm[0], P->delta_width[1], P->delta_norm[1], d_mean, d_scale, d_tr, d_features);
    if (hipGetLastError() != hipSuccess) return fail(c, SPKD_EHIP, "mfcc: kernel launch failed");
    return call.finish();
}

spkd_status spkd_gmm_loglik(spkd_ctx* c, const float* d_features, int64_t n_frames, const spkd_gmm_params* P,
                            float* d_scores) {
    if (!c || !P) return SPKD_EINVAL;
    const int K = P->n_kernels, S = P->n_states;
    if (P->dim != GM_DIM || K < 1 || K > GM_MAX_K || S < 1 || S > GM_MAX_S || n_frames < 0)
        return fail(c, SPKD_EINVAL, "gmm_loglik: dim must be 39, 1 <= kernels <= 256, 1 <= states <= 16");
    if (!P->mean || !P->inv_var || !P->log_norm || !P->state_off || !P->kernel || !P->log_weight)
        return fail(c, SPKD_EINVAL, "gmm_loglik: null model array");
    if (P->state_off[0] != 0) return fail(c, SPKD_EINVAL, "gmm_loglik: state_off[0] must be 0");
    for (int s = 0; s < S; ++s)
        if (P->state_off[s + 1] < P->state_off[s] || P->state_off[s + 1] - P->state_off[s] > K)
            return fail(c, SPKD_EINVAL, "gmm_loglik: state_off must be non-decreasing, at most 256 kernels a state");
    const int nnz = P->state_off[S];
    for (int j = 0; j < nnz; ++j) {
        const float lw = P->log_weight[j];
        if (P->kernel[j] < 0 || P->kernel[j] >= K || std::isnan(lw) || lw == INFINITY)
            return fail(c, SPKD_EINVAL, "gmm_loglik: kernel index out of range or log weight NaN / +inf");
    }
    for (int64_t i = 0; i < (int64_t)K * GM_DIM; ++i)
        if (!std::isfinite(P->mean[i]) || !std::isfinite(P->inv_var[i]) || !(P->inv_var[i] > 0.f))
            return fail(c, SPKD_EINVAL, "gmm_loglik: means must be finite, inverse variances finite and positive");
    for (int k = 0; k < K; ++k)
        if (!std::isfinite(P->log_norm[k])) return fail(c, SPKD_EINVAL, "gmm_loglik: non-finite normalising constant");
    if (n_frames == 0) return SPKD_OK;
    if (!d_features || !d_scores) return fail(c, SPKD_EINVAL, "gmm_loglik: null device buffer");
    const int64_t n_blocks = (n_frames + GM_TPB - 1) / GM_TPB;
    if (n_blocks > 0x7fffffffLL) return fail(c, SPKD_EINVAL, "gmm_loglik: too many frames in one call");
    std::vector<float> tab;
    tab.insert(tab.end(), P->mean, P->mean + (size_t)K * GM_DIM);
    tab.insert(tab.end(), P->inv_var, P->inv_var + (size_t)K * GM_DIM);
    tab.insert(tab.end(), P->log_norm, P->log_norm + K);
    tab.insert(tab.end(), P->log_weight, P->log_weight + nnz);
    std::vector<int32_t> idx(P->state_off, P->state_off + S + 1);
    idx.insert(idx.end(), P->kernel, P->kernel + nnz);
    Call call(c);
    TRY(call.opened);
    float* d_tab = nullptr;
    int32_t* d_idx = nullptr;
    TRY(upload(c, S_GMM_TAB, tab.data(), tab.size(), &d_tab));
    TRY(upload(c, S_GMM_IDX, idx.data(), idx.size(), &d_idx));
    const float* d_mean = d_tab;
    const float* d_iv = d_mean + (size_t)K * GM_DIM;
    const float* d_c = d_iv + (size_t)K * GM_DIM;
    const float* d_lw = d_c + K;
    hipLaunchKernelGGL(k_gmm_loglik, dim3((unsigned)n_blocks), dim3(GM_TPB), 0, c->stream, d_features,
                       (long long)n_frames, d_mean, d_iv, d_c, (const int*)d_idx, (const int*)(d_idx + S + 1), d_lw,
                       S, d_scores);
    if (hipGetLastError() != hipSuccess) return fail(c, SPKD_EHIP, "gmm_loglik: kernel launch failed");
    return call.finish();
}

static const double kPow10[23] = {1e0, 1e1, 1e2, 1e3, 1e4, 1e5, 1e6, 1e7, 1e8, 1e9, 1e10, 1e11,
                                  1e12, 1e13, 1e14, 1e15, 1e16, 1e17, 1e18, 1e19, 1e20, 1e21, 1e22};
static const uint64_t kPow10u[20] = {1ull, 10ull, 100ull, 1000ull, 10000ull, 100000ull, 1000000ull,
                                     10000000ull, 100000000ull, 1000000000ull, 10000000000ull,
                                     100000000000ull, 1000000000000ull, 10000000000000ull,
                                     100000000000000ull, 1000000000000000ull, 10000000000000000ull,
                                     100000000000000000ull, 1000000000000000000ull,
                                     10000000000000000000ull};

static bool roundtrip_fast(double x, double* out) {
    if (!(x >= 1e-3 && x < 1e11)) return false;
    int e10 = (int)std::floor(std::log10(x));
    if (e10 < -3) e10 = -3;
    if (e10 >= 0) { if (x < kPow10[e10]) --e10; else if (e10 + 1 <= 22 && x >= kPow10[e10 + 1]) ++e10; }
    else { if (x * kPow10[-e10] < 1.0) --e10; else if (x * kPow10[-e10 - 1] >= 1.0) ++e10; }
    if (e10 < -3 || e10 > 10) return false;
    int s = 11 - e10;
    int k;
    const double fr = std::frexp(x, &k);
    const uint64_t m = (uint64_t)std::ldexp(fr, 53);
    k -= 53;
    unsigned __int128 prod = (unsigned __int128)m * kPow10u[s];
    uint64_t q;
    if (k >= 0) {
        if (k > 20) return false;
        q = (uint64_t)(prod << k);
    } else {
        const int sh = -k;
        if (sh >= 120) return false;
        const unsigned __int128 one = 1;
        const unsigned __int128 fl = prod >> sh;
        const unsigned __int128 remn = prod & ((one << sh) - 1);
        const unsigned __int128 half = one << (sh - 1);
        q = (uint64_t)fl;
        if (remn > half || (remn == half && (q & 1))) ++q;
    }
    if (q >= 1000000000000ull) {
        if (q != 1000000000000ull) return false;
        q = 100000000000ull;
        s -= 1;
    } else if (q < 100000000000ull) {
        return false;
    }
    *out = s >= 0 ? (double)q / kPow10[s] : (double)q * kPow10[-s];
    return true;
}

static void roundtrip_range(double* v, int64_t lo, int64_t hi) {
    char buf[64];
    for (int64_t i = lo; i < hi; ++i) {
        double r;
        if (roundtrip_fast(v[i], &r)) { v[i] = r; continue; }
        std::snprintf(buf, sizeof buf, "%.12g", v[i]);
        v[i] = std::strtod(buf, nullptr);
    }
}

void spkd_py2_roundtrip(double* v, int64_t n) {
    const int64_t kMinPerThread = 8192;
    int nthreads = (int)std::min<int64_t>(8, n / kMinPerThread);
    if (nthreads <= 1) { roundtrip_range(v, 0, n); return; }
    std::vector<std::thread> pool;
    const int64_t step = (n + nthreads - 1) / nthreads;
    for (int t = 0; t < nthreads; ++t) {
        const int64_t lo = t * step, hi = std::min<int64_t>(n, lo + step);
        if (lo < hi) pool.emplace_back(roundtrip_range, v, lo, hi);
    }
    for (auto& th : pool) th.join();
}

spkd_status spkd_labels_from_merges(int64_t n, int64_t n_merges, const int32_t* h_a, const int32_t* h_b,
                                    int32_t* h_labels) {
    if (n < 0 || n_merges < 0 || (n > 0 && !h_labels) || (n_merges > 0 && (!h_a || !h_b))) return SPKD_EINVAL;
    std::vector<int32_t> ids((size_t)n), parent((size_t)n);
    for (int64_t i = 0; i < n; ++i) ids[(size_t)i] = parent[(size_t)i] = (int32_t)i;
    int64_t m = n;
    for (int64_t k = 0; k < n_merges; ++k) {
        const int32_t a = h_a[k], b = h_b[k];
        if (a < 0 || b <= a || b >= m) return SPKD_EINVAL;
        parent[(size_t)ids[(size_t)b]] = ids[(size_t)a];
        ids.erase(ids.begin() + b);
        --m;
    }
    std::vector<int32_t> where((size_t)n, -1);
    for (int64_t p = 0; p < m; ++p) where[(size_t)ids[(size_t)p]] = (int32_t)p;
    for (int64_t i = 0; i < n; ++i) {
        int32_t r = (int32_t)i;
        while (parent[(size_t)r] != r) r = parent[(size_t)r];
        int32_t c = (int32_t)i;
        while (parent[(size_t)c] != r) { const int32_t nx = parent[(size_t)c]; parent[(size_t)c] = r; c = nx; }
        h_labels[i] = where[(size_t)r] + 1;
    }
    return SPKD_OK;
}

spkd_status spkd_count_flags(const int32_t* h_flags, const int64_t* h_off, const int32_t* h_n, int64_t n_groups,
                             int32_t* h_out) {
    if (n_groups < 0 || (n_groups > 0 && (!h_flags || !h_off || !h_n || !h_out))) return SPKD_EINVAL;
    for (int64_t g = 0; g < n_groups; ++g) {
        if (h_n[g] < 0 || h_off[g] < 0) return SPKD_EINVAL;
        h_out[g] = count_detections(h_flags + h_off[g], h_n[g]);
    }
    return SPKD_OK;
}

spkd_status spkd_gw_lines(int64_t n_turns, const int64_t* h_off, const int32_t* h_n_det, const double* h_det_start,
                          const double* h_det_maxi, const double* h_final_start, const double* h_turn_start_s,
                          const double* h_turn_end_s, const int64_t* h_turn_begin, const int64_t* h_turn_end,
                          double rate, int text_contract, int64_t n_lines, double* h_times, int64_t* h_frame_b,
                          int64_t* h_frame_e, int64_t* h_index, int32_t* h_line_turn) {
    if (n_turns < 0 || n_lines < 0) return SPKD_EINVAL;
    if (n_turns > 0 && (!h_off || !h_n_det || !h_det_start || !h_det_maxi || !h_final_start || !h_turn_start_s ||
                        !h_turn_end_s || !h_turn_begin || !h_turn_end || !h_times))
        return SPKD_EINVAL;
    int64_t i = 0;
    for (int64_t t = 0; t < n_turns; ++t) {
        const int64_t nd = h_n_det[t];
        if (nd < 0 || i + nd + 1 > n_lines) return SPKD_EINVAL;
        const double ls = h_turn_start_s[t], le = h_turn_end_s[t];
        for (int64_t j = 0; j <= nd; ++j, ++i) {
            const RecipeLine L = recipe_line(h_turn_begin[t], h_turn_end[t] - h_turn_begin[t], h_off[t], j, nd,
                                             h_det_start, h_det_maxi, h_final_start + t, ls, le, rate);
            h_times[2 * i] = L.start_s;
            h_times[2 * i + 1] = L.end_s;
            if (h_frame_b) h_frame_b[i] = L.frame_b;
            if (h_frame_e) h_frame_e[i] = L.frame_e;
            if (h_index) h_index[i] = L.index;
            if (h_line_turn) h_line_turn[i] = (int32_t)t;
        }
    }
    if (i != n_lines) return SPKD_EINVAL;
    if (text_contract) spkd_py2_roundtrip(h_times, 2 * n_lines);
    return SPKD_OK;
}

spkd_status spkd_vad_viterbi(int64_t n_frames, int32_t n_states, const float* h_scores, int32_t n_words,
                             const int32_t* h_word_state, const double* h_stay, const double* h_exit,
                             const double* h_enter, int64_t* h_tok_frame, int32_t* h_tok_word, int64_t* h_n_tokens,
// ... 115 lines not shown
```

### speaker-diarization_amd/hipabi.py

```python
import ctypes as C
import os

import numpy as np

HERE = os.path.dirname(os.path.abspath(__file__))
LIB_PATH = os.environ.get('SPKD_HIP_LIBRARY') or os.path.join(HERE, 'csrc', 'libspkd_hip.so')

SPKD_OK, SPKD_EINVAL, SPKD_EHIP, SPKD_ENONFINITE, SPKD_EOVERFLOW, SPKD_ENOMEM = range(6)
KINDS = {'BIC': 0, 'GLR': 1, 'KL2': 2, 'KL2P': 3}
WANT_GLR, WANT_KL2, WANT_KL2_PINV = 1, 2, 4
TIMERS = {n: i for i, n in enumerate(['call', 'chunk_stats', 'reduce_sets', 'pair_terms',
                                        'cluster_prep', 'matrix', 'ahc', 'gw', 'sw'])}
REC = 820
DIM = 39

EXPORTS = ['spkd_abi_version', 'spkd_create', 'spkd_create_on_stream', 'spkd_destroy', 'spkd_last_error', 'spkd_sync',
           'spkd_malloc', 'spkd_free', 'spkd_memcpy_h2d', 'spkd_memcpy_d2h', 'spkd_memcpy_d2d',
           'spkd_last_kernel_ms', 'spkd_last_gw_items', 'spkd_set_stats', 'spkd_pair_terms',
           'spkd_distance_matrix', 'spkd_gw_event_capacity', 'spkd_gw_event_capacity_p', 'spkd_gw', 'spkd_gw_ex', 'spkd_gw_fused', 'spkd_gw_batch', 'spkd_ahc_fused', 'spkd_gather_stats', 'spkd_mfcc',
           'spkd_sw_window_count', 'spkd_sw', 'spkd_ahc', 'spkd_ahc_matrix', 'spkd_distance_rows', 'spkd_cluster_in', 'spkd_py2_roundtrip',
           'spkd_labels_from_merges', 'spkd_labels_from_merges_batch', 'spkd_count_flags', 'spkd_gw_lines',
           'spkd_gmm_loglik', 'spkd_vad_viterbi']


class CdParams(C.Structure):
    _fields_ = [('kind', C.c_int32), ('trace', C.c_int32), ('lambdac', C.c_double),
                ('threshold', C.c_double), ('winsize', C.c_double), ('winstep', C.c_double),
                ('deltaws', C.c_double), ('rate', C.c_double)]


class CandLog(C.Structure):
    _fields_ = [('turn', C.c_int32), ('coarse', C.c_int32), ('seq', C.c_int64),
                ('start', C.c_double), ('i', C.c_double), ('d', C.c_double),
                ('n1', C.c_int64), ('n2', C.c_int64)]


class GwLinesView(C.Structure):
    _fields_ = [('n_lines', C.c_int64), ('n_redo', C.c_int64), ('n_win', C.c_void_p), ('times', C.c_void_p),
                ('turn', C.c_void_p), ('frame_b', C.c_void_p), ('frame_e', C.c_void_p), ('index', C.c_void_p),
                ('d_index', C.c_void_p), ('redo_line', C.c_void_p), ('redo_begin', C.c_void_p),
                ('redo_end', C.c_void_p)]


AHC_AUTO, AHC_MONO, AHC_WIDE = 0, 1, 2


class MfccParams(C.Structure):
    _fields_ = [('sample_rate', C.c_int32), ('frame_rate', C.c_int32), ('window_width', C.c_int32),
                ('n_fft', C.c_int32), ('n_mel', C.c_int32), ('n_cep', C.c_int32), ('cms_left', C.c_int32),
                ('cms_right', C.c_int32), ('delta_width', C.c_int32 * 2), ('pre_emph', C.c_float),
                ('delta_norm', C.c_float * 2)]


class GmmParams(C.Structure):
    _fields_ = [('n_kernels', C.c_int32), ('n_states', C.c_int32), ('dim', C.c_int32), ('mean', C.c_void_p),
                ('inv_var', C.c_void_p), ('log_norm', C.c_void_p), ('state_off', C.c_void_p), ('kernel', C.c_void_p),
                ('log_weight', C.c_void_p)]


class AhcParams(C.Structure):
    _fields_ = [('variant', C.c_int32), ('kind', C.c_int32), ('max_spk', C.c_int32),
                ('path', C.c_int32), ('lambdac', C.c_double), ('threshold', C.c_double)]


class SpkdError(RuntimeError):
    def __init__(self, status, text):
        RuntimeError.__init__(self, 'spkd status %d: %s' % (status, text))
        self.status = status


_lib = None


def _one_hip_runtime():
    import sys
    if 'torch' in sys.modules or os.environ.get('SPKD_SYSTEM_HIP'):
        return
    try:
        import importlib.util
        spec = importlib.util.find_spec('torch')
        where = list(spec.submodule_search_locations)[0] if spec and spec.submodule_search_locations else None
    except (ImportError, ValueError, AttributeError):
        where = None
    if where:
        rt = os.path.join(where, 'lib', 'libamdhip64.so')
        if os.path.exists(rt):
            try:
                C.CDLL(rt, mode=C.RTLD_GLOBAL)
            except OSError:
                pass


def mapped_hip_runtimes():
    found = set()
    try:
        with open('/proc/self/maps') as f:
            for line in f:
                path = line.rsplit(None, 1)[-1] if '/' in line else ''
                if os.path.basename(path).startswith('libamdhip64.so'):
                    found.add(os.path.realpath(path))
    except OSError:
        pass
    return sorted(found)


def _check_one_runtime():
    rts = mapped_hip_runtimes()
    if len(rts) > 1:
        raise ImportError('two HIP runtimes are mapped into this process (%s): libspkd_hip.so and the PyTorch '
                          'wheel link against different libamdhip64 sonames.  Set SPKD_SYSTEM_HIP=1 for a '
                          'torch-free process, or import torch before this package.' % ', '.join(rts))


def load_library(path=None):
    global _lib
    if _lib is not None and path is None:
        return _lib
    p = path or LIB_PATH
    if not os.path.exists(p):
        raise ImportError('HIP extension %s is not built: run `python -c "import __graft_entry__ as g; '
                          'g.build()"` (or make -C speaker-diarization_amd/csrc)' % p)
    _one_hip_runtime()
    lib = C.CDLL(p)
    _check_one_runtime()
    vp, i64, i32, dbl = C.c_void_p, C.c_int64, C.c_int32, C.c_double
    P = C.POINTER
    lib.spkd_abi_version.restype = C.c_int
    lib.spkd_create.argtypes = [C.c_int, vp, P(vp)]
    lib.spkd_create_on_stream.argtypes = [C.c_int, vp, P(vp)]
    lib.spkd_destroy.argtypes = [vp]
    lib.spkd_destroy.restype = None
    lib.spkd_last_error.argtypes = [vp]
    lib.spkd_last_error.restype = C.c_char_p
    lib.spkd_sync.argtypes = [vp]
    lib.spkd_malloc.argtypes = [vp, C.c_size_t, P(vp)]
    lib.spkd_free.argtypes = [vp, vp]
    lib.spkd_memcpy_h2d.argtypes = [vp, vp, vp, C.c_size_t]
    lib.spkd_memcpy_d2h.argtypes = [vp, vp, vp, C.c_size_t]
    lib.spkd_memcpy_d2d.argtypes = [vp, vp, vp, C.c_size_t]
    lib.spkd_last_kernel_ms.argtypes = [vp, C.c_int, P(C.c_float)]
    lib.spkd_last_gw_items.argtypes = [vp, P(C.c_int64)]
    lib.spkd_set_stats.argtypes = [vp, vp, i64, vp, vp, vp, i64, i64, vp]
    lib.spkd_pair_terms.argtypes = [vp, vp, vp, vp, i64, C.c_int, vp]
    lib.spkd_distance_matrix.argtypes = [vp, C.c_int, dbl, vp, i64, vp]
    lib.spkd_gw_event_capacity.argtypes = [i64, dbl]
    lib.spkd_gw_event_capacity.restype = i64
    lib.spkd_gw_event_capacity_p.argtypes = [i64, P(CdParams)]
    lib.spkd_gw_event_capacity_p.restype = i64
    lib.spkd_gw.argtypes = [vp, vp, i64, vp, vp, i64, P(CdParams), vp, vp, vp, vp, vp, vp, vp, vp,
                            vp, i64, P(i64)]
    lib.spkd_gw_ex.argtypes = [vp, vp, i64, vp, vp, i64, P(CdParams), vp, C.c_int, vp, vp, vp, vp, vp, vp,
                               vp, vp, i64, P(i64)]
    lib.spkd_gw_fused.argtypes = [vp, vp, i64, vp, vp, i64, P(CdParams), vp, C.c_int, vp, vp, vp, vp, vp, vp,
                                  vp, vp, vp, i64, P(i64)]
    lib.spkd_gw_batch.argtypes = [vp, vp, i64, vp, vp, i64, P(CdParams), vp, vp, vp, vp, vp, vp, C.c_int, P(GwLinesView)]
    lib.spkd_ahc_fused.argtypes = [vp, vp, i64, vp, i64, vp, vp, i64, vp, vp, vp, i64, P(AhcParams),
                                   P(vp), P(vp), P(vp), P(vp), P(vp)]
    lib.spkd_gather_stats.argtypes = [vp, vp, i64, vp, vp, i64, i64, vp]
    lib.spkd_mfcc.argtypes = [vp, vp, i64, P(MfccParams), vp, vp, vp, vp, vp, vp, P(i64)]
    lib.spkd_sw_window_count.argtypes = [i64, dbl, dbl]
    lib.spkd_sw_window_count.restype = i64
    lib.spkd_sw.argtypes = [vp, vp, i64, vp, vp, i64, P(CdParams), vp, vp]
    lib.spkd_ahc.argtypes = [vp, vp, vp, i64, P(AhcParams), vp, vp, vp, vp, vp, vp]
    lib.spkd_ahc_matrix.argtypes = [vp, vp, i64, P(AhcParams), vp, dbl, dbl, vp, vp, vp, vp, vp, vp]
    lib.spkd_distance_rows.argtypes = [vp, C.c_int, C.c_int, dbl, vp, i64, i64, i64, vp, P(dbl), P(dbl)]
    lib.spkd_cluster_in.argtypes = [vp, vp, i64, C.c_int, dbl, dbl, vp, vp, i64, vp, P(i64), P(i64)]
    lib.spkd_py2_roundtrip.argtypes = [vp, i64]
    lib.spkd_py2_roundtrip.restype = None
    lib.spkd_labels_from_merges.argtypes = [i64, i64, vp, vp, vp]
    lib.spkd_labels_from_merges_batch.argtypes = [i64, vp, vp, vp, vp, vp]
    lib.spkd_count_flags.argtypes = [vp, vp, vp, i64, vp]
    lib.spkd_gmm_loglik.argtypes = [vp, vp, i64, P(GmmParams), vp]
    lib.spkd_vad_viterbi.argtypes = [i64, i32, vp, i32, vp, vp, vp, vp, vp, vp, P(i64), P(dbl)]
    lib.spkd_gw_lines.argtypes = [i64, vp, vp, vp, vp, vp, vp, vp, vp, vp, dbl, C.c_int, i64, vp, vp, vp, vp, vp]
    if lib.spkd_abi_version() != 2:
        raise ImportError('libspkd_hip.so ABI version mismatch')
    if path is None:
        _lib = lib
    return lib


def _ptr(a):
    return a.ctypes.data_as(C.c_void_p)


def _view(addr, n, dtype):
    if not addr or n <= 0:
        return np.zeros(0, dtype=dtype)
    ct = {np.int32: C.c_int32, np.int64: C.c_int64, np.float64: C.c_double}[dtype]
    return np.ctypeslib.as_array(C.cast(C.c_void_p(addr), C.POINTER(ct)), shape=(int(n),))


def py2_roundtrip(values):
    v = np.ascontiguousarray(values, dtype=np.float64).copy()
    if v.size:
        load_library().spkd_py2_roundtrip(_ptr(v), v.size)
    return v


def labels_from_merges(n, a, b):
    a = np.ascontiguousarray(a, dtype=np.int32)
    b = np.ascontiguousarray(b, dtype=np.int32)
    out = np.zeros(n, dtype=np.int32)
    st = load_library().spkd_labels_from_merges(n, len(a), _ptr(a), _ptr(b), _ptr(out))
    if st != SPKD_OK:
        raise SpkdError(st, 'bad merge log')
    return out


def count_flags(flags, off, n):
    flags = np.ascontiguousarray(flags, dtype=np.int32)
    off = np.ascontiguousarray(off, dtype=np.int64)
    n = np.ascontiguousarray(n, dtype=np.int32)
    if len(off) != len(n):
        raise SpkdError(SPKD_EINVAL, 'one offset per group')
    if len(n) and (int((off + n).max()) > len(flags) or int(n.min()) < 0 or int(off.min()) < 0):
        raise SpkdError(SPKD_EINVAL, 'flag ranges outside the array')
    out = np.zeros(len(n), dtype=np.int32)
    st = load_library().spkd_count_flags(_ptr(flags), _ptr(off), _ptr(n), len(n), _ptr(out))
    if st != SPKD_OK:
        raise SpkdError(st, 'bad flag ranges')
    return out


def gw_lines(off, n_det, det_start, det_maxi, final_start, turn_start_s, turn_end_s, turn_begin, turn_end,
             rate, text_contract=True, want_frames=False):
    c = np.ascontiguousarray
    off = c(off, dtype=np.int64); n_det = c(n_det, dtype=np.int32)
    nt = len(n_det)
    arrs = [c(det_start, dtype=np.float64), c(det_maxi, dtype=np.float64), c(final_start, dtype=np.float64),
            c(turn_start_s, dtype=np.float64), c(turn_end_s, dtype=np.float64), c(turn_begin, dtype=np.int64),
            c(turn_end, dtype=np.int64)]
    if len(off) != nt or any(len(a) != nt for a in arrs[2:]):
        raise SpkdError(SPKD_EINVAL, 'one entry per turn')
    if nt and (int(n_det.min()) < 0 or int(off.min()) < 0 or int((off + n_det).max()) > min(len(arrs[0]), len(arrs[1]))):
        raise SpkdError(SPKD_EINVAL, 'detections outside the event arrays')
    n_lines = int(n_det.sum(dtype=np.int64)) + nt
    times = np.empty((n_lines, 2), dtype=np.float64)
    turn = np.empty(n_lines, dtype=np.int32)
    fb = np.empty(n_lines, dtype=np.int64) if want_frames else None
    fe = np.empty(n_lines, dtype=np.int64) if want_frames else None
    ix = np.empty(n_lines, dtype=np.int64) if want_frames else None
    p = lambda a: _ptr(a) if a is not None else None
    st = load_library().spkd_gw_lines(nt, _ptr(off), _ptr(n_det), *[_ptr(a) for a in arrs], float(rate),
                                      1 if text_contract else 0, n_lines, _ptr(times), p(fb), p(fe), p(ix), _ptr(turn))
    if st != SPKD_OK:
        raise SpkdError(st, 'bad growing-window result')
    return {'times': times, 'turn': turn, 'frame_b': fb, 'frame_e': fe, 'index': ix}


def vad_viterbi(scores, word_state, stay, exit_, enter):
    c = np.ascontiguousarray
    scores = c(scores, dtype=np.float32)
    if scores.ndim != 2:
        raise SpkdError(SPKD_EINVAL, 'scores must be [frames, states]')
    ws = c(word_state, dtype=np.int32)
    consts = [c(a, dtype=np.float64) for a in (stay, exit_, enter)]
    if any(len(a) != len(ws) for a in consts):
        raise SpkdError(SPKD_EINVAL, 'one constant of each kind per word')
    T, S = scores.shape
    tf = np.zeros(max(T, 1), dtype=np.int64)
    tw = np.zeros(max(T, 1), dtype=np.int32)
    n = C.c_int64(0)
    sc = C.c_double(0.0)
    st = load_library().spkd_vad_viterbi(T, S, _ptr(scores), len(ws), _ptr(ws), *[_ptr(a) for a in consts],
                                         _ptr(tf), _ptr(tw), C.byref(n), C.byref(sc))
    if st != SPKD_OK:
        raise SpkdError(st, 'bad decoder input')
    return tf[:n.value].copy(), tw[:n.value].copy(), sc.value


def labels_from_merges_batch(seg_off, n_merges, a, b):
    seg_off = np.ascontiguousarray(seg_off, dtype=np.int64)
    n_merges = np.ascontiguousarray(n_merges, dtype=np.int32)
    a = np.ascontiguousarray(a, dtype=np.int32)
    b = np.ascontiguousarray(b, dtype=np.int32)
    out = np.zeros(int(seg_off[-1]), dtype=np.int32)
    st = load_library().spkd_labels_from_merges_batch(len(seg_off) - 1, _ptr(seg_off), _ptr(n_merges),
                                                      _ptr(a), _ptr(b), _ptr(out))
    if st != SPKD_OK:
# ... 111 lines not shown
        self.check(st, allow=(SPKD_ENONFINITE,))
        return out, st

    def distance_matrix(self, kind, lambdac, d_stats, n, d_matrix):
        st = self.lib.spkd_distance_matrix(self.h, KINDS[kind], lambdac, C.c_void_p(d_stats), n,
                                           C.c_void_p(d_matrix))
        return self.check(st, allow=(SPKD_ENONFINITE,))

    def _buf(self, name, n, dtype):
        cache = self.__dict__.setdefault('_bufs', {})
        arr = cache.get(name)
        if arr is None or arr.shape[0] < n or arr.dtype != np.dtype(dtype):
            arr = cache[name] = np.empty(max(n, 1), dtype=dtype)
        return arr[:n]

    def gather_stats(self, d_src, n_src, src_index, d_dst, n_dst, dst_index=None):
        si = np.ascontiguousarray(src_index, dtype=np.int64)
        di = None if dst_index is None else np.ascontiguousarray(dst_index, dtype=np.int64)
        self.check(self.lib.spkd_gather_stats(self.h, C.c_void_p(d_src), n_src, _ptr(si),
                                              None if di is None else _ptr(di), len(si), n_dst,
                                              C.c_void_p(d_dst)))

    def gw(self, d_frames, n_frames, begins, ends, params, log_cap=4096, tight=False, reuse=False,
           seg_stats=None, first_guess_scale=1.0):
        b = np.ascontiguousarray(begins, dtype=np.int64)
        e = np.ascontiguousarray(ends, dtype=np.int64)
        nt = len(b)
        for off in _gw_capacity_ladder(e - b, params, tight, first_guess_scale):
            nev = int(off[-1])
            mk = self._buf if reuse else (lambda name, n, dt: np.empty(n, dtype=dt))
            n_win = mk('n_win', nt, np.int32)
            win_maxd = mk('win_maxd', nev, np.float64)
            win_det = mk('win_det', nev, np.int32)
            det_start = mk('det_start', nev, np.float64)
            det_maxi = mk('det_maxi', nev, np.float64)
            det_d = mk('det_d', nev, np.float64)
            final_start = mk('final_start', nt, np.float64)
            d_seg = None if seg_stats is None else seg_stats(nev)
            while True:
                log = (CandLog * max(log_cap, 1))()
                cnt = C.c_int64(0)
                if seg_stats is None:
                    st = self.lib.spkd_gw_ex(self.h, C.c_void_p(d_frames), n_frames, _ptr(b), _ptr(e), nt,
                                             C.byref(params), _ptr(off), 0, _ptr(n_win),
                                             _ptr(win_maxd), _ptr(win_det), _ptr(det_start), _ptr(det_maxi),
                                             _ptr(det_d), _ptr(final_start), C.cast(log, C.c_void_p), log_cap,
                                             C.byref(cnt))
                else:
                    st = self.lib.spkd_gw_fused(self.h, C.c_void_p(d_frames), n_frames, _ptr(b), _ptr(e), nt,
                                                C.byref(params), _ptr(off), 0, _ptr(n_win),
                                                _ptr(win_maxd), _ptr(win_det), _ptr(det_start), _ptr(det_maxi),
                                                _ptr(det_d), _ptr(final_start), C.c_void_p(d_seg),
                                                C.cast(log, C.c_void_p), log_cap, C.byref(cnt))
                if not (st == SPKD_EOVERFLOW and cnt.value > log_cap):
                    break
                log_cap = int(cnt.value) + 16
            if st != SPKD_EOVERFLOW:
                break
        self.check(st, allow=(SPKD_ENONFINITE,))
        return dict(status=st, off=off, n_ev=nev, n_win=n_win, win_maxd=win_maxd, win_det=win_det,
                    det_start=det_start, det_maxi=det_maxi, det_d=det_d, final_start=final_start,
                    log=log, log_count=min(int(cnt.value), log_cap))

    def gw_batch(self, d_frames, n_frames, begins, ends, params, turn_start_s, turn_end_s, file_off, file_len,
                 seg_stats, tight=True, first_guess_scale=1.0, want_index=False):
        c = np.ascontiguousarray
        b = c(begins, dtype=np.int64)
        e = c(ends, dtype=np.int64)
        nt = len(b)
        host = [c(turn_start_s, dtype=np.float64), c(turn_end_s, dtype=np.float64), c(file_off, dtype=np.int64),
                c(file_len, dtype=np.int64)]
        if any(len(a) != nt for a in host):
            raise SpkdError(SPKD_EINVAL, 'one entry per turn')
        view = GwLinesView()
        for off in _gw_capacity_ladder(e - b, params, tight, first_guess_scale):
            nev = int(off[-1])
            d_seg = seg_stats(nev)
            st = self.lib.spkd_gw_batch(self.h, C.c_void_p(d_frames), n_frames, _ptr(b), _ptr(e), nt, C.byref(params),
                                        _ptr(off), *[_ptr(a) for a in host], C.c_void_p(d_seg),
                                        1 if want_index else 0, C.byref(view))
            if st != SPKD_EOVERFLOW:
                break
        self.check(st, allow=(SPKD_ENONFINITE,))
        n, nr = int(view.n_lines), int(view.n_redo)
        return dict(status=st, off=off, n_ev=nev, d_seg=d_seg, n_lines=n, n_win=_view(view.n_win, nt if n else 0, np.int32),
                    times=_view(view.times, 2 * n, np.float64).reshape(-1, 2), turn=_view(view.turn, n, np.int32),
                    frame_b=_view(view.frame_b, n, np.int64), frame_e=_view(view.frame_e, n, np.int64),
                    index=_view(view.index, n, np.int64) if want_index else None, d_index=view.d_index,
                    redo_line=_view(view.redo_line, nr, np.int64), redo_begin=_view(view.redo_begin, nr, np.int64),
                    redo_end=_view(view.redo_end, nr, np.int64))

    def ahc_fused(self, d_frames, n_frames, d_records, n_records, d_line_index, seg_off, redo_line, redo_begin,
                  redo_end, params):
        c = np.ascontiguousarray
        seg_off = c(seg_off, dtype=np.int64)
        rl, rb, re_ = c(redo_line, dtype=np.int64), c(redo_begin, dtype=np.int64), c(redo_end, dtype=np.int64)
        if not (len(rl) == len(rb) == len(re_)):
            raise SpkdError(SPKD_EINVAL, 'one range per redo line')
        npb, nt = len(seg_off) - 1, int(seg_off[-1])
        out = [C.c_void_p() for _ in range(5)]
        st = self.lib.spkd_ahc_fused(self.h, C.c_void_p(d_frames), n_frames, C.c_void_p(d_records), n_records,
                                     C.c_void_p(d_line_index), _ptr(seg_off), npb, _ptr(rl), _ptr(rb), _ptr(re_), len(rl),
                                     C.byref(params), *[C.byref(o) for o in out])
        self.check(st, allow=(SPKD_ENONFINITE,))
        if st != SPKD_OK:
            return dict(status=st)
        return dict(status=st, n_merges=_view(out[0].value, npb, np.int32), a=_view(out[1].value, nt, np.int32),
                    b=_view(out[2].value, nt, np.int32), d=_view(out[3].value, nt, np.float64),
                    labels=_view(out[4].value, nt, np.int32))

    def sw(self, d_frames, n_frames, begins, ends, params):
        b = np.ascontiguousarray(begins, dtype=np.int64)
        e = np.ascontiguousarray(ends, dtype=np.int64)
        nt = len(b)
        cnt = [self.lib.spkd_sw_window_count(int(e[t] - b[t]), params.winsize, params.winstep)
               for t in range(nt)]
        if any(c < 0 for c in cnt):
            raise SpkdError(SPKD_EINVAL, 'window size and step must be at least one frame')
        off = np.zeros(nt + 1, dtype=np.int64)
        off[1:] = np.cumsum(cnt)
        d = np.zeros(int(off[-1]), dtype=np.float64)
        st = self.lib.spkd_sw(self.h, C.c_void_p(d_frames), n_frames, _ptr(b), _ptr(e), nt,
                              C.byref(params), _ptr(off), _ptr(d))
        self.check(st, allow=(SPKD_ENONFINITE,))
        return st, off, d

    def mfcc(self, d_pcm, n_samples, params, melfb, dct, mean, scale, transform, d_features):
        arrs = [np.ascontiguousarray(a, dtype=np.float32) for a in (melfb, dct, mean, scale, transform)]
        n = C.c_int64(0)
        self.check(self.lib.spkd_mfcc(self.h, C.c_void_p(d_pcm), n_samples, C.byref(params), *[_ptr(a) for a in arrs],
                                      C.c_void_p(d_features), C.byref(n)))
        return int(n.value)

    def gmm_loglik(self, d_features, n_frames, gmm, d_scores):
        a = {k: np.ascontiguousarray(gmm[k], dtype=np.int32 if k in ('state_off', 'kernel') else np.float32)
             for k in ('mean', 'inv_var', 'log_norm', 'state_off', 'kernel', 'log_weight')}
        K, S = len(a['log_norm']), len(a['state_off']) - 1
        if a['mean'].size != K * DIM or a['inv_var'].size != K * DIM or S < 1 or \
                len(a['kernel']) != len(a['log_weight']) or int(a['state_off'][-1]) != len(a['kernel']):
            raise SpkdError(SPKD_EINVAL, 'inconsistent model array sizes')
        p = GmmParams(K, S, a['mean'].shape[-1] if a['mean'].ndim == 2 else DIM,
                      *[_ptr(a[k]) for k in ('mean', 'inv_var', 'log_norm', 'state_off', 'kernel', 'log_weight')])
        self.check(self.lib.spkd_gmm_loglik(self.h, C.c_void_p(d_features), int(n_frames), C.byref(p),
                                            C.c_void_p(d_scores)))

    def ahc(self, d_stats, seg_off, params):
        seg_off = np.ascontiguousarray(seg_off, dtype=np.int64)
        npb = len(seg_off) - 1
        nt = int(seg_off[-1])
        n_merges = np.zeros(npb, dtype=np.int32)
        ma = np.zeros(nt, dtype=np.int32)
        mb = np.zeros(nt, dtype=np.int32)
        md = np.zeros(nt, dtype=np.float64)
        smax = np.zeros(npb, dtype=np.float64)
        smin = np.zeros(npb, dtype=np.float64)
        st = self.lib.spkd_ahc(self.h, C.c_void_p(d_stats), _ptr(seg_off), npb, C.byref(params),
                               _ptr(n_merges), _ptr(ma), _ptr(mb), _ptr(md), _ptr(smax), _ptr(smin))
        self.check(st, allow=(SPKD_ENONFINITE,))
        return dict(status=st, n_merges=n_merges, a=ma, b=mb, d=md, stat_max=smax, stat_min=smin)

    def distance_rows(self, variant, kind, lambdac, d_stats, n, row_begin, row_end, d_rows):
        smax, smin = C.c_double(), C.c_double()
        st = self.lib.spkd_distance_rows(self.h, int(variant), KINDS[kind] if isinstance(kind, str) else int(kind),
                                         float(lambdac), C.c_void_p(d_stats), int(n), int(row_begin), int(row_end),
                                         C.c_void_p(d_rows), C.byref(smax), C.byref(smin))
        self.check(st, allow=(SPKD_ENONFINITE,))
        if st == SPKD_ENONFINITE:
            raise ValueError('array must not contain infs or NaNs')
        return smax.value, smin.value

    def cluster_in(self, d_stats, n, kind, lambdac, threshold):
        n = int(n)
        label = np.zeros(max(n, 1), dtype=np.int32)
# ... 32 lines not shown
```

### speaker-diarization_amd/pipeline.py

```python
import time

import numpy as np

from . import hipabi
from .recipe import py2_float_str

DIA2_CD = dict(kind='BIC', lambdac=1.0, threshold=0.0, winsize_s=1.0, winstep_s=3.0, deltaws_s=0.1)
DIA2_CL = dict(variant=1, kind='BIC', lambdac=1.3, threshold=0.0, max_spk=0)


class BatchFile(object):

    def __init__(self, frame_off, n_frames, vad):
        self.frame_off = int(frame_off)
        self.n_frames = int(n_frames)
        self.vad = [(float(s), float(e)) for (s, e) in vad]
        self.vad_arr = np.array(self.vad, dtype=np.float64).reshape(-1, 2)


class FusedStats(object):

    def __init__(self, d_buf, n_buf, index, begin, end):
        self.d_buf, self.n_buf, self.index, self.begin, self.end = d_buf, n_buf, index, begin, end

# ... 112 lines not shown
    return out


def segment_stats(ctx, d_frames, total_frames, files, segments, rate=125.0, timings=None, fused=None,
                  scratch_name='segment_stats'):
    cnt = [len(s) for s in segments]
    seg_off = np.zeros(len(files) + 1, dtype=np.int64)
    seg_off[1:] = np.cumsum(cnt)
    n = int(seg_off[-1])
    allseg = np.concatenate([np.asarray(s, dtype=np.float64).reshape(-1, 2) for s in segments]) if n else np.zeros((0, 2))
    owner = np.repeat(np.arange(len(files)), cnt)
    foff = np.array([f.frame_off for f in files], dtype=np.int64)[owner]
    fn = np.array([f.n_frames for f in files], dtype=np.int64)[owner]
    a0 = np.clip((allseg[:, 0] * rate).astype(np.int64), 0, fn)
    a1 = np.maximum(a0, np.clip((allseg[:, 1] * rate).astype(np.int64), 0, fn))
    b, e = foff + a0, foff + a1
    d_stats = ctx.dev_scratch(scratch_name, max(n, 1) * hipabi.REC * 8)
    _t1 = time.perf_counter()
    if fused is None:
        ctx.set_stats(d_frames, total_frames, b, e, np.arange(n, dtype=np.int32), n, d_stats)
        redo = np.arange(n)
    else:
        same = (fused.begin == b) & (fused.end == e)
        keep = np.nonzero(same)[0]
        redo = np.nonzero(~same)[0]
        ctx.gather_stats(fused.d_buf, fused.n_buf, fused.index[keep], d_stats, n, keep)
        if len(redo):
            d_tmp = ctx.dev_scratch(scratch_name + '_redo', len(redo) * hipabi.REC * 8)
            ctx.set_stats(d_frames, total_frames, b[redo], e[redo], np.arange(len(redo), dtype=np.int32),
                          len(redo), d_tmp)
            ctx.gather_stats(d_tmp, len(redo), np.arange(len(redo)), d_stats, n, redo)
    if timings is not None:
        _time_stats(ctx, timings, n, b[redo], e[redo])
    return d_stats, seg_off, n, _t1


def cluster_batch(ctx, d_frames, total_frames, files, segments, rate=125.0, cl=DIA2_CL, timings=None,
                  want_merges=False, fused=None):
    rate = float(rate)
    cnt = [len(s) for s in segments]
    keep = _problems(cnt)[0]
    if len(keep) < len(files):
        out = [(np.zeros(0, dtype=np.int32), [] if want_merges else None) for _ in files]
        if len(keep):
            sub = cluster_batch(ctx, d_frames, total_frames, [files[i] for i in keep],
                                [segments[i] for i in keep], rate, cl, timings, want_merges, fused)
            for i, r in zip(keep, sub):
                out[i] = r
        return out
    _t0 = time.perf_counter()
    d_stats, seg_off, n, _t1 = segment_stats(ctx, d_frames, total_frames, files, segments, rate, timings, fused)
    _t2 = time.perf_counter()
    r = ctx.ahc(d_stats, seg_off, _ahc_params(cl))
    _t3 = time.perf_counter()
    _clustering_done(ctx, timings, seg_off, r)
    all_labels = hipabi.labels_from_merges_batch(seg_off, r['n_merges'], r['a'], r['b'])
    out = []
    for fi in range(len(files)):
        o, c = int(seg_off[fi]), cnt[fi]
        merges = None
        if want_merges:
            nm = int(r['n_merges'][fi])
            merges = list(zip(r['a'][o:o + nm].tolist(), r['b'][o:o + nm].tolist(), r['d'][o:o + nm].tolist()))
        out.append((all_labels[o:o + c], merges))
    if timings is not None:
        _t4 = time.perf_counter()
        timings.setdefault('wall_cl_prepare', []).append(1e3 * (_t1 - _t0))
        timings.setdefault('wall_cl_stats_call', []).append(1e3 * (_t2 - _t1))
        timings.setdefault('wall_cl_ahc_call', []).append(1e3 * (_t3 - _t2))
        timings.setdefault('wall_cl_finish', []).append(1e3 * (_t4 - _t3))
    return out


def diarize_batch_device(ctx, d_frames, total_frames, files, rate=125.0, cd=DIA2_CD, cl=DIA2_CL, timings=None,
                         detail=None, first_guess_scale=1.0):
    rate = float(rate)
    _t0 = time.perf_counter()
    table = _turn_table(files, rate)
    if table is None:
        return [np.zeros((0, 3)) for _ in files]
    owner, foff, fn, ls, le, tb, te = table
    ls, le = np.ascontiguousarray(ls), np.ascontiguousarray(le)
    p = _cd_params(cd, rate)
    _t1 = time.perf_counter()
    r = ctx.gw_batch(d_frames, total_frames, tb, te, p, ls, le, foff, fn,
                     lambda n_rec: ctx.dev_scratch('fused_segment_stats', max(n_rec, 1) * hipabi.REC * 8),
                     tight=True, first_guess_scale=first_guess_scale, want_index=detail is not None)
    _t2 = time.perf_counter()
    _detector_done(ctx, timings, tb, te, r)
    line_file = owner[r['turn']]
    bounds = np.searchsorted(line_file, np.arange(len(files) + 1))
    _t3 = time.perf_counter()
    seg_off = _problems(np.diff(bounds))[1]
    ap = _ahc_params(cl)
    _t4 = time.perf_counter()
    a = ctx.ahc_fused(d_frames, total_frames, r['d_seg'], r['n_ev'], r['d_index'], seg_off, r['redo_line'],
                      r['redo_begin'], r['redo_end'], ap)
    _t5 = time.perf_counter()
    if timings is not None:
        _time_stats(ctx, timings, r['n_lines'], r['redo_begin'], r['redo_end'])
    _clustering_done(ctx, timings, seg_off, a)
    if detail is not None:
        detail['lines'] = {k: (np.array(v) if isinstance(v, np.ndarray) else v) for k, v in r.items()}
        detail['merges'] = [list(zip(a['a'][o:o + m].tolist(), a['b'][o:o + m].tolist(), a['d'][o:o + m].tolist()))
                            for o, m in zip(seg_off[:-1].tolist(), a['n_merges'].tolist())]
    rows = _recipe_rows(r['times'], line_file, a['labels'], rate)
    out = [rows[bounds[i]:bounds[i + 1]] for i in range(len(files))]
    if timings is not None:
        _t6 = time.perf_counter()
        timings.setdefault('wall_cd_prepare', []).append(1e3 * (_t1 - _t0))
        timings.setdefault('wall_cd_call', []).append(1e3 * (_t2 - _t1))
        timings.setdefault('wall_cd_finish', []).append(1e3 * (_t3 - _t2))
        timings.setdefault('wall_cl_prepare', []).append(1e3 * (_t4 - _t3))
        timings.setdefault('wall_cl_stats_call', []).append(0.0)
        timings.setdefault('wall_cl_ahc_call', []).append(1e3 * (_t5 - _t4))
        timings.setdefault('wall_cl_finish', []).append(1e3 * (_t6 - _t5))
    return out


def diarize_batch(ctx, d_frames, total_frames, files, rate=125.0, cd=DIA2_CD, cl=DIA2_CL, timings=None,
                  text_contract=True, fused=False, handoff=None):
    if handoff is None:
        handoff = 'device' if fused and text_contract else 'host'
    if handoff == 'device':
        if not (fused and text_contract):
            raise ValueError('the device hand-off is the fused mode with the text contract')
        return diarize_batch_device(ctx, d_frames, total_frames, files, rate, cd, cl, timings)
    if handoff != 'host':
        raise ValueError('handoff: device or host')
    box = [] if fused else None
    segs = change_detect_batch(ctx, d_frames, total_frames, files, rate, cd, timings, text_contract, box)
    fs = box[0] if box else None
    if fused and fs is None:
        return [np.zeros((0, 3)) for _ in files]
    return _cluster_and_order(ctx, d_frames, total_frames, files, segs, rate, cl, timings, fs)


def _cluster_and_order(ctx, d_frames, total_frames, files, segs, rate, cl, timings, fs):
    res = cluster_batch(ctx, d_frames, total_frames, files, segs, rate, cl, timings, fused=fs)
    cnt = [len(s) for s in segs]
    if sum(cnt) == 0:
        return [np.zeros((0, 3)) for _ in segs]
    allseg = np.concatenate([np.asarray(s, dtype=np.float64).reshape(-1, 2) for s in segs])
    labels = np.concatenate([lab for (lab, _) in res])
    rows = _recipe_rows(allseg, np.repeat(np.arange(len(segs)), cnt), labels, rate)
    bounds = np.zeros(len(segs) + 1, dtype=np.int64)
    bounds[1:] = np.cumsum(cnt)
    out = [rows[bounds[i]:bounds[i + 1]] for i in range(len(segs))]
    return out


def in_flight(contexts, n_jobs, job):
    import threading
    if len(contexts) == 1 or n_jobs <= 1:
        for k in range(n_jobs):
            yield job(contexts[0], k)
        return
    results = [None] * n_jobs
    done = [threading.Event() for _ in range(n_jobs)]
    nxt = [0]
    lock = threading.Lock()
    failure = []

    def worker(ctx):
        while not failure:
            with lock:
                k = nxt[0]
                nxt[0] += 1
            if k >= n_jobs:
                return
            try:
                results[k] = job(ctx, k)
            except BaseException as e:
                failure.append(e)
            finally:
                done[k].set()

    threads = [threading.Thread(target=worker, args=(c,)) for c in contexts]
    for th in threads:
        th.start()
# ... 15 lines not shown
```

Before: 1456.

## Fuse change detection and clustering handoff into one device-side batch step

Adds a spkd_batch_step entry point that runs the detector-to-clustering handoff on the GPU. New kernels do the py2 float roundtrip of line times, recompute clustering ranges, build the redo/chunk lists, and lay out problem offsets and the XCD schedule. Clustering prep now reads its record count from device memory, which avoids host round trips and synchronisation between the gw and AHC calls. Cases the fast path cannot handle (inexact roundtrip, capacity overflow) fall back to the old two-call path, at the cost of added complexity and serial single-block scans.

```diff
diff --git a/include/spkd.h b/include/spkd.h
--- a/include/spkd.h
+++ b/include/spkd.h
@@ -179,6 +179,29 @@
                            const int32_t **h_merge_b, const double **h_merge_d,
                            const int32_t **h_labels);
 
+enum { SPKD_STEP_WANT_INDEX = 1, SPKD_STEP_FORCE_SLOW = 2 };
+enum { SPKD_STEP_DONE = 0, SPKD_STEP_NOT_APPLICABLE = 1, SPKD_STEP_CAPACITY = 2, SPKD_STEP_SLOW_PATH = 3 };
+
+typedef struct {
+    int32_t fallback;
+    int32_t reserved;
+    const int64_t *seg_off;
+    const int32_t *n_merges;
+    const int32_t *merge_a;
+    const int32_t *merge_b;
+    const double *merge_d;
+    const int32_t *labels;
+} spkd_batch_step_result;
+
+spkd_status spkd_batch_step(spkd_ctx *ctx, const float *d_frames, int64_t n_frames,
+                            const int64_t *h_turn_begin, const int64_t *h_turn_end, int64_t n_turns,
+                            const spkd_cd_params *params, const int64_t *h_ev_off,
+                            const double *h_turn_start_s, const double *h_turn_end_s,
+                            const int64_t *h_turn_file_off, const int64_t *h_turn_file_len,
+                            const int32_t *h_turn_problem, int64_t n_problems, double *d_seg_stats,
+                            const spkd_ahc_params *ahc_params, int flags, spkd_gw_lines_view *view,
+                            spkd_batch_step_result *result);
+
 typedef struct {
     int32_t sample_rate, frame_rate, window_width, n_fft, n_mel, n_cep;
     int32_t cms_left, cms_right;
@@ -204,6 +227,7 @@
                             const spkd_gmm_params *params, float *d_scores);
 
 void spkd_py2_roundtrip(double *h_values, int64_t n);
+int64_t spkd_py2_roundtrip_rule(const double *h_values, int64_t n, double *h_out, int32_t *h_decided);
 spkd_status spkd_labels_from_merges(int64_t n, int64_t n_merges, const int32_t *h_a,
                                     const int32_t *h_b, int32_t *h_labels);
 spkd_status spkd_labels_from_merges_batch(int64_t n_problems, const int64_t *h_seg_off,
diff --git a/speaker-diarization_amd/csrc/spkd_cluster.hpp b/speaker-diarization_amd/csrc/spkd_cluster.hpp
--- a/speaker-diarization_amd/csrc/spkd_cluster.hpp
+++ b/speaker-diarization_amd/csrc/spkd_cluster.hpp
@@ -377,7 +377,8 @@
 __global__ __launch_bounds__(PT_WAVES * WAVE) void k_cluster_prep(
         const double* __restrict__ qr, int64_t n_rec, int kind,
         double* __restrict__ ld, double* __restrict__ aux, int* err,
-        double* pinv_ws) {
+        double* pinv_ws, const int64_t* __restrict__ n_rec_dev) {
+    if (n_rec_dev) n_rec = *n_rec_dev;
     const int wave = threadIdx.x >> 6;
     const int64_t w = (int64_t)blockIdx.x * PT_WAVES + wave;
     if (kind == SPKD_KL2) {
diff --git a/speaker-diarization_amd/csrc/spkd_handoff.hpp b/speaker-diarization_amd/csrc/spkd_handoff.hpp
--- a/speaker-diarization_amd/csrc/spkd_handoff.hpp
+++ b/speaker-diarization_amd/csrc/spkd_handoff.hpp
@@ -1,7 +1,10 @@
 #pragma once
+#include <cstdint>
+#include <cstring>
 #include "spkd_cd.hpp"
 #include "spkd_cluster.hpp"
 #include "spkd_device.hpp"
+#include "spkd_stats.hpp"
 
 namespace spkd {
 
@@ -39,6 +42,49 @@
     L.frame_e = tail ? begin + len : begin + (int64_t)fe;
     L.index = ev_off + j;
     return L;
+}
+
+__host__ __device__ inline bool py2_roundtrip_fast(double x, double* out) {
+#pragma clang fp contract(off)
+    constexpr uint64_t P10[15] = {1ull, 10ull, 100ull, 1000ull, 10000ull, 100000ull, 1000000ull, 10000000ull,
+                                  100000000ull, 1000000000ull, 10000000000ull, 100000000000ull,
+                                  1000000000000ull, 10000000000000ull, 100000000000000ull};
+    if (x == 0.0) { *out = x; return true; }
+    if (!(x >= 1e-3 && x < 1e11)) return false;
+    int e10 = 0;
+    if (x >= 1.0) { while (e10 < 10 && x >= (double)P10[e10 + 1]) ++e10; }
+    else e10 = x >= 0.1 ? -1 : (x >= 0.01 ? -2 : -3);
+    int s = 11 - e10;
+    uint64_t bits;
+    memcpy(&bits, &x, sizeof bits);
+    const int sh = 1075 - (int)((bits >> 52) & 0x7ff);
+    const uint64_t m = (bits & 0xfffffffffffffull) | 0x10000000000000ull;
+    if (sh < 1 || sh > 100) return false;
+    const unsigned __int128 one = 1;
+    const unsigned __int128 prod = (unsigned __int128)m * P10[s];
+    const unsigned __int128 remn = prod & ((one << sh) - 1), half = one << (sh - 1);
+    uint64_t q = (uint64_t)(prod >> sh);
+    if (remn > half || (remn == half && (q & 1))) ++q;
+    if (q >= 1000000000000ull) {
+        if (q != 1000000000000ull) return false;
+        q = 100000000000ull;
+        s -= 1;
+    } else if (q < 100000000000ull) {
+        return false;
+    }
+    *out = (double)q / (double)P10[s];
+    return true;
+}
+
+__host__ __device__ inline void clustering_range(double t0, double t1, double rate, int64_t file_off, int64_t file_len,
+                                                 int64_t* begin, int64_t* end) {
+#pragma clang fp contract(off)
+    int64_t a0 = (int64_t)(t0 * rate), a1 = (int64_t)(t1 * rate);
+    a0 = a0 < 0 ? 0 : (a0 > file_len ? file_len : a0);
+    a1 = a1 < 0 ? 0 : (a1 > file_len ? file_len : a1);
+    if (a1 < a0) a1 = a0;
+    *begin = file_off + a0;
+    *end = file_off + a1;
 }
 
 constexpr int CP_TPB = 256;
@@ -121,13 +167,10 @@
     if (k < n) map[line[k]] = -(k + 1);
 }
 
-__global__ __launch_bounds__(256) void k_records_from_map(const double* __restrict__ recs, int64_t n_recs,
-                                                          const int64_t* __restrict__ map,
-                                                          const double* __restrict__ redo, int64_t n_redo,
-                                                          int64_t n_rec, double* __restrict__ qr,
-                                                          double* __restrict__ packed, int* __restrict__ err) {
-    const int64_t c = blockIdx.x;
-    if (c >= n_rec) return;
+__device__ __forceinline__ void record_from_map(const double* __restrict__ recs, int64_t n_recs,
+                                                const int64_t* __restrict__ map, const double* __restrict__ redo,
+                                                int64_t n_redo, int64_t c, double* __restrict__ qr,
+                                                double* __restrict__ packed, int* __restrict__ err) {
     const int64_t m = map[c];
     const double* g;
     if (m >= 0 && m < n_recs) {
@@ -143,6 +186,16 @@
     for (int e = threadIdx.x; e < REC; e += 256) p[e] = g[e];
 }
 
+__global__ __launch_bounds__(256) void k_records_from_map(const double* __restrict__ recs, int64_t n_recs,
+                                                          const int64_t* __restrict__ map,
+                                                          const double* __restrict__ redo, int64_t n_redo,
+                                                          int64_t n_rec, double* __restrict__ qr,
+                                                          double* __restrict__ packed, int* __restrict__ err) {
+    const int64_t c = blockIdx.x;
+    if (c >= n_rec) return;
+    record_from_map(recs, n_recs, map, redo, n_redo, c, qr, packed, err);
+}
+
 __global__ __launch_bounds__(256) void k_gather_records(const double* __restrict__ src, const int64_t* __restrict__ si,
                                                         const int64_t* __restrict__ di, int64_t n,
                                                         double* __restrict__ dst) {
@@ -158,4 +211,234 @@
     if (p < n) out[p] = mat[4 * p + 1];
 }
 
-}
+enum { HO_N_LINES = 0, HO_N_REDO, HO_N_CHUNKS, HO_CELLS, HO_N_MAX, HO_LONGEST, HO_STATUS, HO_N_EFF, HO_N_REDO_EFF, HO_N };
+enum { HO_SLOW = 1, HO_CAPACITY = 2, HO_ERR = 4 };
+constexpr int HO_TPB = 1024;
+constexpr int HO_MAX_PROB = 1024;
+constexpr int HO_XCDS = 8;
+
+struct HoCaps {
+    int64_t lines, redo, chunks, cells, n_max, list;
+};
+
+__device__ __forceinline__ int* ho_status(int64_t* ho) { return reinterpret_cast<int*>(ho + HO_STATUS); }
+
+__device__ __forceinline__ int64_t ho_block_scan(int64_t v, int64_t* part, int64_t* total) {
+    const int tid = threadIdx.x;
+    __syncthreads();
+    part[tid] = v;
+    __syncthreads();
+    for (int d = 1; d < HO_TPB; d <<= 1) {
+        const int64_t a = tid >= d ? part[tid - d] : 0;
+        __syncthreads();
+        part[tid] += a;
+        __syncthreads();
+    }
+    *total = part[HO_TPB - 1];
+    return part[tid] - v;
+}
+
+__global__ __launch_bounds__(CP_TPB) void k_ho_roundtrip(const int64_t* __restrict__ n_lines_dev, int64_t line_cap,
+                                                         const int* __restrict__ err, double* __restrict__ times,
+                                                         const int64_t* __restrict__ frame_b,
+                                                         const int64_t* __restrict__ frame_e,
+                                                         const int32_t* __restrict__ line_turn,
+                                                         const int64_t* __restrict__ file_off,
+                                                         const int64_t* __restrict__ file_len, double rate,
+                                                         int force_slow, int64_t* __restrict__ range_b,
+                                                         int64_t* __restrict__ range_e, int32_t* __restrict__ moved,
+                                                         int64_t* __restrict__ ho) {
+    if (*err) return;
+    int64_t n = *n_lines_dev;
+    n = n > line_cap ? line_cap : n;
+    const int64_t i = (int64_t)blockIdx.x * CP_TPB + threadIdx.x;
+    if (i >= n) return;
+    double r0, r1;
+    const bool ok0 = py2_roundtrip_fast(times[2 * i], &r0), ok1 = py2_roundtrip_fast(times[2 * i + 1], &r1);
+    if (!ok0 || !ok1 || force_slow) {
+        atomicOr(ho_status(ho), HO_SLOW);
+        moved[i] = 0;
+        return;
+    }
+    times[2 * i] = r0;
+    times[2 * i + 1] = r1;
+    const int32_t t = line_turn[i];
+    int64_t b, e;
+    clustering_range(r0, r1, rate, file_off[t], file_len[t], &b, &e);
+    range_b[i] = b;
+    range_e[i] = e;
+    moved[i] = (b != frame_b[i] || e != frame_e[i]) ? 1 : 0;
+}
+
+__global__ __launch_bounds__(HO_TPB) void k_ho_redo(const int64_t* __restrict__ n_lines_dev, const int* __restrict__ err,
+                                                    HoCaps cap, const int32_t* __restrict__ moved,
+                                                    const int64_t* __restrict__ range_b,
+                                                    const int64_t* __restrict__ range_e, int64_t* __restrict__ redo_line,
+                                                    int64_t* __restrict__ redo_begin, int64_t* __restrict__ redo_end,
+                                                    Chunk* __restrict__ chunks, int64_t* __restrict__ set_off,
+                                                    int64_t* __restrict__ map, int64_t* __restrict__ ho) {
+    __shared__ int64_t part[HO_TPB];
+    const int tid = threadIdx.x;
+    const int64_t n = *n_lines_dev;
+    bool ok = !*err && *ho_status(ho) == 0 && n <= cap.lines;
+    int64_t n_redo = 0, n_chunks = 0;
+    if (ok) {
+        const int64_t per = (n + HO_TPB - 1) / HO_TPB;
+        const int64_t lo = tid * per < n ? tid * per : n, hi = lo + per < n ? lo + per : n;
+        int64_t my_r = 0, my_c = 0;
+        for (int64_t i = lo; i < hi; ++i)
+            if (moved[i]) {
+                ++my_r;
+                my_c += (range_e[i] - range_b[i] + STATS_CHUNK - 1) / STATS_CHUNK;
+            }
+        int64_t k = ho_block_scan(my_r, part, &n_redo);
+        int64_t ci = ho_block_scan(my_c, part, &n_chunks);
+        ok = n_redo <= cap.redo && n_chunks <= cap.chunks;
+        if (ok)
+            for (int64_t i = lo; i < hi; ++i)
+                if (moved[i]) {
+                    const int64_t b = range_b[i], e = range_e[i];
+                    redo_line[k] = i;
+                    redo_begin[k] = b;
+                    redo_end[k] = e;
+                    set_off[k] = ci;
+                    for (int64_t f = b; f < e; f += STATS_CHUNK, ++ci) {
+                        Chunk ch;
+                        ch.begin = f;
+                        ch.len = (int32_t)(e - f < STATS_CHUNK ? e - f : STATS_CHUNK);
+                        ch.set = (int32_t)k;
+                        chunks[ci] = ch;
+                    }
+                    map[i] = -(k + 1);
+                    ++k;
+                }
+    }
+    if (tid == 0) {
+        ho[HO_N_LINES] = n;
+        ho[HO_N_REDO] = n_redo;
+        ho[HO_N_CHUNKS] = n_chunks;
+        ho[HO_N_REDO_EFF] = ok ? n_redo : 0;
+        if (!ok) atomicOr(ho_status(ho), *err ? HO_ERR : HO_CAPACITY);
+    }
+    const int64_t r0 = ok ? n_redo : 0, c0 = ok ? n_chunks : 0;
+    for (int64_t k = r0 + tid; k <= cap.redo; k += HO_TPB) set_off[k] = c0;
+    for (int64_t ci = c0 + tid; ci < cap.chunks; ci += HO_TPB) {
+        Chunk ch;
+        ch.begin = 0;
+        ch.len = 0;
+        ch.set = 0;
+        chunks[ci] = ch;
+    }
+}
+
+__global__ __launch_bounds__(HO_TPB) void k_ho_problems(const int64_t* __restrict__ line_off, int64_t n_turns,
+                                                        const int* __restrict__ err, HoCaps cap,
+                                                        const int64_t* __restrict__ turn_first, int n_prob,
+                                                        int64_t* __restrict__ seg_off, int64_t* __restrict__ mat_off,
+                                                        int64_t* __restrict__ prob_slot, int32_t* __restrict__ sched,
+                                                        double* __restrict__ mat, int64_t* __restrict__ ho) {
+    __shared__ int64_t s_off[HO_MAX_PROB + 1];
+    __shared__ int32_t s_order[HO_MAX_PROB], s_xcd[HO_MAX_PROB];
+    __shared__ int64_t s_start[HO_MAX_PROB];
+    __shared__ int s_ok;
+    const int tid = threadIdx.x;
+    const int64_t n = line_off[n_turns];
+    if (tid == 0) s_ok = (!*err && *ho_status(ho) == 0 && n <= cap.lines && n_prob <= HO_MAX_PROB) ? 1 : 0;
+    __syncthreads();
+    if (s_ok) {
+        for (int p = tid; p <= n_prob; p += HO_TPB) s_off[p] = p < n_prob ? line_off[turn_first[p]] : n;
+        __syncthreads();
+        for (int p = tid; p < n_prob; p += HO_TPB) {
+            const int64_t np = s_off[p + 1] - s_off[p];
+            int place = 0;
+            for (int q = 0; q < n_prob; ++q) {
+                const int64_t nq = s_off[q + 1] - s_off[q];
+                place += (nq > np || (nq == np && q < p)) ? 1 : 0;
+            }
+            s_order[place] = p;
+        }
+        __syncthreads();
+        if (tid == 0) {
+            int64_t cells = 0, n_max = 0, longest = 0, len[HO_XCDS];
+            double load[HO_XCDS];
+            bool fine = true;
+            for (int x = 0; x < HO_XCDS; ++x) { len[x] = 0; load[x] = 0.0; }
+            for (int p = 0; p < n_prob; ++p) {
+                const int64_t np = s_off[p + 1] - s_off[p];
+                fine = fine && np >= 1;
+                n_max = np > n_max ? np : n_max;
+                cells += np * np;
+            }
+            for (int r = 0; r < n_prob; ++r) {
+                const int p = s_order[r];
+                int x = 0;
+                for (int i = 1; i < HO_XCDS; ++i) if (load[i] < load[x]) x = i;
+                const double np = (double)(s_off[p + 1] - s_off[p]);
+                load[x] += np * np;
+                s_xcd[p] = x;
+                s_start[p] = len[x];
+                len[x] += s_off[p + 1] - s_off[p];
+                longest = len[x] > longest ? len[x] : longest;
+            }
+            if (n_prob < HO_XCDS) longest = (n + HO_XCDS - 1) / HO_XCDS;
+            ho[HO_CELLS] = cells;
+            ho[HO_N_MAX] = n_max;
+            ho[HO_LONGEST] = longest;
+            if (!fine || cells > cap.cells || n_max > cap.n_max || longest > cap.list) {
+                atomicOr(ho_status(ho), HO_CAPACITY);
+                s_ok = 0;
+            }
+        }
+        __syncthreads();
+    }
+    const bool ok = s_ok != 0;
+    if (tid == 0) ho[HO_N_EFF] = ok ? n : 0;
+    for (int64_t b = tid; b < cap.list * HO_XCDS; b += HO_TPB) sched[b] = -1;
+    if (!ok) {
+        if (tid == 0 && *err) atomicOr(ho_status(ho), HO_ERR);
+        for (int p = tid; p <= n_prob; p += HO_TPB) {
+            seg_off[p] = p;
+            mat_off[p] = p;
+            if (p < n_prob) mat[p] = MAXINT_F;
+        }
+        return;
+    }
+    __syncthreads();
+    if (tid == 0) {
+        int64_t cells = 0;
+        for (int p = 0; p < n_prob; ++p) {
+            const int64_t np = s_off[p + 1] - s_off[p];
+            mat_off[p] = cells;
+            cells += np * np;
+        }
+        mat_off[n_prob] = cells;
+    }
+    for (int p = tid; p <= n_prob; p += HO_TPB) seg_off[p] = s_off[p];
+    for (int p = tid; p < n_prob; p += HO_TPB) prob_slot[p] = s_start[p] * HO_XCDS + s_xcd[p];
+}
+
+__global__ __launch_bounds__(CP_TPB) void k_ho_sched(const int64_t* __restrict__ ho, int n_prob,
+                                                     const int32_t* __restrict__ line_turn,
+                                                     const int32_t* __restrict__ turn_prob,
+                                                     const int64_t* __restrict__ seg_off,
+                                                     const int64_t* __restrict__ prob_slot,
+                                                     int32_t* __restrict__ rec_prob, int32_t* __restrict__ sched) {
+    const int64_t g = (int64_t)blockIdx.x * CP_TPB + threadIdx.x;
+    if (g >= ho[HO_N_EFF]) return;
+    const int p = turn_prob[line_turn[g]];
+    rec_prob[g] = p;
+    sched[n_prob < HO_XCDS ? g : prob_slot[p] + (g - seg_off[p]) * HO_XCDS] = (int32_t)g;
+}
+
+__global__ __launch_bounds__(256) void k_records_from_map_dev(const double* __restrict__ recs, int64_t n_recs,
+                                                              const int64_t* __restrict__ map,
+                                                              const double* __restrict__ redo,
+                                                              const int64_t* __restrict__ ho,
+                                                              double* __restrict__ qr, double* __restrict__ packed,
+                                                              int* __restrict__ err) {
+    const int64_t c = blockIdx.x;
+    if (c >= ho[HO_N_EFF]) return;
+    record_from_map(recs, n_recs, map, redo, ho[HO_N_REDO_EFF], c, qr, packed, err);
+}
+
+}
diff --git a/speaker-diarization_amd/csrc/spkd_hip.hip b/speaker-diarization_amd/csrc/spkd_hip.hip
--- a/speaker-diarization_amd/csrc/spkd_hip.hip
+++ b/speaker-diarization_amd/csrc/spkd_hip.hip
@@ -22,8 +22,8 @@
 using namespace spkd;
 
 namespace {
-constexpr int N_SLOTS = 40;
-enum { PIN_GW_TURNS = 0, PIN_GW_LINES, PIN_AHC_OUT, N_PIN };
+constexpr int N_SLOTS = 48;
+enum { PIN_GW_TURNS = 0, PIN_GW_LINES, PIN_AHC_OUT, PIN_STEP_MISC, N_PIN };
 }
 
 struct spkd_ctx {
@@ -54,6 +54,11 @@
     std::vector<Chunk> redo_chunks;
     std::vector<int64_t> redo_setoff;
     std::vector<int32_t> redo_sets;
+    int64_t hw_lines = 0, hw_redo = 0, hw_chunks = 0, hw_cells = 0, hw_nmax = 0, hw_list = 0;
+    hipStream_t side = nullptr;
+    hipEvent_t ev_side[2] = {};
+    bool side_used = false;
+    std::vector<int64_t> step_first;
 };
 
 namespace {
@@ -123,7 +128,12 @@
     int herr = 0;
     bool drained = false;
     explicit Call(spkd_ctx* ctx) : c(ctx) { opened = open(); }
-    ~Call() { if (!drained) (void)hipStreamSynchronize(c->stream); }
+    ~Call() {
+        if (drained) return;
+        (void)hipStreamSynchronize(c->stream);
+        if (c->side_used) (void)hipStreamSynchronize(c->side);
+        c->side_used = false;
+    }
     spkd_status open() {
         HIPCHK(c, hipSetDevice(c->device));
         for (int i = 0; i < SPKD_N_TIMERS; ++i) c->kused[i] = false;
@@ -136,6 +146,8 @@
         HIPCHK(c, hipEventRecord(c->ev1, c->stream));
         HIPCHK(c, hipMemcpyAsync(&herr, c->d_err, sizeof(int), hipMemcpyDeviceToHost, c->stream));
         HIPCHK(c, hipStreamSynchronize(c->stream));
+        if (c->side_used) HIPCHK(c, hipStreamSynchronize(c->side));
+        c->side_used = false;
         drained = true;
         HIPCHK(c, hipEventElapsedTime(&c->last_ms, c->ev0, c->ev1));
         c->kms[0] = c->last_ms;
@@ -177,7 +189,7 @@
     S_EV_I32A, S_EV_I32B, S_EV_D0, S_EV_D1, S_EV_D2, S_EV_D3, S_EV_D4, S_LOG,
     S_AHC_STATS, S_AHC_LD, S_AHC_AUX, S_AHC_MAT, S_AHC_MISC, S_AHC_OUT, S_AHC_OFF, S_AHC_PROB, S_AHC_PACKED, S_MFCC_TAB, S_MFCC_STATIC,
     S_STEP_EXM, S_STEP_PKM, S_STEP_MISC, S_GMM_TAB, S_GMM_IDX,
-    S_CP_TURNS, S_CP_TIMES, S_CP_LINES, S_REDO_STATS, S_REDO_IDX, S_COUNT
+    S_CP_TURNS, S_CP_TIMES, S_CP_LINES, S_REDO_STATS, S_REDO_IDX, S_HO_TURNS, S_HO_LINES, S_HO_REDO, S_HO_COUNTS, S_COUNT
 };
 static_assert(S_COUNT <= N_SLOTS, "scratch slot table too small");
 
@@ -245,6 +257,9 @@
     for (int i = 0; i < N_PIN; ++i)
         if (c->pin[i]) (void)hipHostFree(c->pin[i]);
     if (c->d_counter) (void)hipFree(c->d_counter);
+    if (c->side) (void)hipStreamDestroy(c->side);
+    for (hipEvent_t e : c->ev_side)
+        if (e) (void)hipEventDestroy(e);
     if (c->ev0) (void)hipEventDestroy(c->ev0);
     if (c->ev1) (void)hipEventDestroy(c->ev1);
     for (int i = 0; i < SPKD_N_TIMERS; ++i) {
@@ -470,6 +485,17 @@
         size_t longest = 0;
         for (auto& l : lists) longest = std::max(longest, l.size());
         grid_rows = (int64_t)longest * X;
+        if (plan.d_map) {
+            c->hw_lines = n_total;
+            c->hw_cells = cells;
+            c->hw_list = (int64_t)longest;
+            c->hw_nmax = 0;
+            for (int64_t p = 0; p < n_prob; ++p) c->hw_nmax = std::max(c->hw_nmax, h_seg_off[p + 1] - h_seg_off[p]);
+            c->hw_redo = plan.n_redo;
+            c->hw_chunks = 0;
+            for (int64_t k = 0; k < plan.n_redo; ++k)
+                c->hw_chunks += (plan.redo_end[k] - plan.redo_begin[k] + STATS_CHUNK - 1) / STATS_CHUNK;
+        }
         prob_of.resize((size_t)(n_total + grid_rows), -1);
         for (int x = 0; x < X; ++x)
             for (size_t i = 0; i < lists[x].size(); ++i) prob_of[(size_t)n_total + i * X + x] = lists[x][i];
@@ -527,7 +553,7 @@
         {
             Timer t(c, SPKD_T_CLUSTER_PREP);
             hipLaunchKernelGGL(k_cluster_prep, dim3(blocks), dim3(PT_WAVES * WAVE), 0, c->stream,
-                               (const double*)B.ex, n_total, kind, B.ld, B.aux, c->d_err, c->pinv_cur);
+                               (const double*)B.ex, n_total, kind, B.ld, B.aux, c->d_err, c->pinv_cur, (const int64_t*)nullptr);
         }
         auto kmat = kind == SPKD_GLR ? k_matrix<true> : k_matrix<false>;
         if (plan.d_init) {
@@ -610,14 +636,14 @@
             Timer t(c, SPKD_T_CLUSTER_PREP);
             hipLaunchKernelGGL(k_cluster_prep, dim3(blocks), dim3(PT_WAVES * WAVE), 0, c->stream,
                                (const double*)p_ex, n, kind == SPKD_KL2 ? (int)SPKD_BIC : kind, (double*)p_ld, (double*)p_aux, c->d_err,
-                               c->pinv_cur);
+                               c->pinv_cur, (const int64_t*)nullptr);
         }
         if (kind == SPKD_KL2) {
             void* p_ld2 = nullptr;
             TRY(scratch(c, S_AHC_OUT, nn * sizeof(double), &p_ld2));
             const unsigned blocks1 = (unsigned)((n + PT_WAVES - 1) / PT_WAVES);
             hipLaunchKernelGGL(k_cluster_prep, dim3(blocks1), dim3(PT_WAVES * WAVE), 0, c->stream,
-                               (const double*)p_ex, n, (int)SPKD_KL2, (double*)p_ld2, (double*)p_aux, c->d_err, c->pinv_cur);
+                               (const double*)p_ex, n, (int)SPKD_KL2, (double*)p_ld2, (double*)p_aux, c->d_err, c->pinv_cur, (const int64_t*)nullptr);
         }
     }
     auto kin = kind == SPKD_GLR ? k_cluster_in<true> : k_cluster_in<false>;
@@ -970,12 +996,8 @@
     for (int64_t i = 0; i < V.n_lines; ++i) {
         const int64_t t = V.turn[i];
         if (t < 0 || t >= n_turns) return fail(c, SPKD_EHIP, "internal error: line of no turn");
-        const int64_t fn = G.file_len[t];
-        int64_t a0 = (int64_t)(times[2 * i] * rate), a1 = (int64_t)(times[2 * i + 1] * rate);
-        a0 = a0 < 0 ? 0 : (a0 > fn ? fn : a0);
-        a1 = a1 < 0 ? 0 : (a1 > fn ? fn : a1);
-        if (a1 < a0) a1 = a0;
-        const int64_t b = G.file_off[t] + a0, e = G.file_off[t] + a1;
+        int64_t b, e;
+        clustering_range(times[2 * i], times[2 * i + 1], rate, G.file_off[t], G.file_len[t], &b, &e);
         if (b != V.frame_b[i] || e != V.frame_e[i]) {
             c->redo_line.push_back(i);
             c->redo_begin.push_back(b);
@@ -1008,12 +1030,9 @@
 
 constexpr int64_t GW_WAVE_PER_TURN_FROM = 4096;
 constexpr int64_t GW_EIGHT_WAVES_UP_TO = 256;
-spkd_status gw_impl(spkd_ctx* c, const GwIn& in, const GwOut& out, GwBatch* batch = nullptr) {
-    const int64_t n_turns = in.n_turns, log_cap = out.log_cap;
+
+spkd_status gw_check(spkd_ctx* c, const GwIn& in, const GwOut& out, bool batch) {
     const spkd_cd_params* P = in.P;
-    if (!c || !P || n_turns < 0) return SPKD_EINVAL;
-    if (out.h_log_count) *out.h_log_count = 0;
-    if (n_turns == 0) return SPKD_OK;
     if (!in.d_frames || !in.hb || !in.he || !in.h_ev_off) return fail(c, SPKD_EINVAL, "null argument");
     if (!batch && (!out.h_n_win || !out.h_win_maxd || !out.h_win_det || !out.h_det_start || !out.h_det_maxi ||
                    !out.h_det_d || !out.h_final_start))
@@ -1021,24 +1040,25 @@
     if (P->kind < 0 || P->kind > 3) return fail(c, SPKD_EINVAL, "gw: bad kind");
     if (!(P->rate >= 10.0) || !(P->winsize >= 1.0) || !(P->winstep >= 1.0))
         return fail(c, SPKD_EINVAL, "gw: rate >= 10, winsize >= 1 frame and winstep >= 1 frame required");
-    if (log_cap < 0 || (log_cap > 0 && !out.h_log)) return fail(c, SPKD_EINVAL, "gw: log capacity without a log buffer");
+    if (out.log_cap < 0 || (out.log_cap > 0 && !out.h_log)) return fail(c, SPKD_EINVAL, "gw: log capacity without a log buffer");
     if (!c->gw_lds_ok) return fail(c, SPKD_EHIP, "gw: the kernel's dynamic LDS size was not admitted on this device");
-    std::vector<TurnDesc> turns;
-    int64_t n_cand;
-    TRY(build_turns(c, in.n_frames, in.hb, in.he, n_turns, P, in.h_ev_off, true, turns, n_cand));
-    for (int64_t t = 0; in.check_capacity && t < n_turns; ++t)
-        if (turns[(size_t)t].ev_cap < spkd_gw_event_capacity_p(turns[(size_t)t].len, P))
-            return fail(c, SPKD_EINVAL, "gw: event capacity too small, see spkd_gw_event_capacity_p");
-    unsigned long long cnt2[2] = {0ull, 0ull};
-    Call call(c);
-    TRY(call.opened);
-    spkd_cd_params Pk = *P;
-    TRY(use_kind(c, P->kind, &Pk.kind));
-    P = &Pk;
-    const int64_t n_ev = in.h_ev_off[n_turns];
+    return SPKD_OK;
+}
+
+struct GwDev {
     TurnDesc* d_turns = nullptr;
     void *d_snap = nullptr, *d_cand = nullptr, *d_i32a = nullptr, *d_i32b = nullptr, *d_d0 = nullptr, *d_d1 = nullptr,
          *d_d2 = nullptr, *d_d3 = nullptr, *d_d4 = nullptr, *d_log = nullptr;
+    int64_t n_ev = 0;
+};
+
+spkd_status gw_enqueue(spkd_ctx* c, const GwIn& in, int64_t log_cap, const spkd_cd_params* P,
+                       const std::vector<TurnDesc>& turns, int64_t n_cand, GwBatch* batch, GwDev& dv) {
+    const int64_t n_turns = in.n_turns;
+    const int64_t n_ev = dv.n_ev = in.h_ev_off[n_turns];
+    TurnDesc*& d_turns = dv.d_turns;
+    void *&d_snap = dv.d_snap, *&d_cand = dv.d_cand, *&d_i32a = dv.d_i32a, *&d_i32b = dv.d_i32b, *&d_d0 = dv.d_d0,
+         *&d_d1 = dv.d_d1, *&d_d2 = dv.d_d2, *&d_d3 = dv.d_d3, *&d_d4 = dv.d_d4, *&d_log = dv.d_log;
     TRY(upload(c, S_TURNS, turns.data(), turns.size(), &d_turns));
     TRY(scratch(c, S_SNAP, (size_t)n_cand * REC * sizeof(double), &d_snap));
     TRY(scratch(c, S_CAND, (size_t)n_cand * 4 * sizeof(double), &d_cand));
@@ -1071,6 +1091,34 @@
     }
 #undef SPKD_GW_LAUNCH
     HIPCHK(c, hipGetLastError());
+    return SPKD_OK;
+}
+
+spkd_status gw_impl(spkd_ctx* c, const GwIn& in, const GwOut& out, GwBatch* batch = nullptr) {
+    const int64_t n_turns = in.n_turns, log_cap = out.log_cap;
+    const spkd_cd_params* P = in.P;
+    if (!c || !P || n_turns < 0) return SPKD_EINVAL;
+    if (out.h_log_count) *out.h_log_count = 0;
+    if (n_turns == 0) return SPKD_OK;
+    TRY(gw_check(c, in, out, batch != nullptr));
+    std::vector<TurnDesc> turns;
+    int64_t n_cand;
+    TRY(build_turns(c, in.n_frames, in.hb, in.he, n_turns, P, in.h_ev_off, true, turns, n_cand));
+    for (int64_t t = 0; in.check_capacity && t < n_turns; ++t)
+        if (turns[(size_t)t].ev_cap < spkd_gw_event_capacity_p(turns[(size_t)t].len, P))
+            return fail(c, SPKD_EINVAL, "gw: event capacity too small, see spkd_gw_event_capacity_p");
+    unsigned long long cnt2[2] = {0ull, 0ull};
+    Call call(c);
+    TRY(call.opened);
+    spkd_cd_params Pk = *P;
+    TRY(use_kind(c, P->kind, &Pk.kind));
+    P = &Pk;
+    GwDev dv;
+    TRY(gw_enqueue(c, in, log_cap, P, turns, n_cand, batch, dv));
+    const int64_t n_ev = dv.n_ev;
+    TurnDesc* const d_turns = dv.d_turns;
+    void *const d_i32a = dv.d_i32a, *const d_i32b = dv.d_i32b, *const d_d0 = dv.d_d0, *const d_d1 = dv.d_d1,
+         *const d_d2 = dv.d_d2, *const d_d3 = dv.d_d3, *const d_d4 = dv.d_d4, *const d_log = dv.d_log;
     unsigned long long& cnt = cnt2[0];
     if (batch) {
         TRY(gw_batch_compact(c, *batch, d_turns, n_turns, (const int32_t*)d_i32a, (const int32_t*)d_i32b,
@@ -1223,6 +1271,283 @@
     *h_merge_b = mb;
     *h_merge_d = md;
     *h_labels = lab;
+    return SPKD_OK;
+}
+
+spkd_status spkd_batch_step(spkd_ctx* c, const float* d_frames, int64_t n_frames, const int64_t* hb, const int64_t* he,
+                            int64_t n_turns, const spkd_cd_params* P, const int64_t* h_ev_off,
+                            const double* h_turn_start_s, const double* h_turn_end_s, const int64_t* h_turn_file_off,
+                            const int64_t* h_turn_file_len, const int32_t* h_turn_problem, int64_t n_prob,
+                            double* d_seg_stats, const spkd_ahc_params* A, int flags, spkd_gw_lines_view* view,
+                            spkd_batch_step_result* res) {
+    if (!c || !view || !res || !P || !A) return SPKD_EINVAL;
+    std::memset(view, 0, sizeof *view);
+    std::memset(res, 0, sizeof *res);
+    res->fallback = SPKD_STEP_NOT_APPLICABLE;
+    if (n_turns < 1 || n_prob < 1) return SPKD_OK;
+    if (!d_seg_stats) return fail(c, SPKD_EINVAL, "batch_step: null statistics buffer");
+    if (!h_turn_start_s || !h_turn_end_s || !h_turn_file_off || !h_turn_file_len || !h_turn_problem)
+        return fail(c, SPKD_EINVAL, "batch_step: null turn arrays");
+    if ((A->variant != 1 && A->variant != 2) || A->kind < 0 || A->kind > 3)
+        return fail(c, SPKD_EINVAL, "bad variant / kind");
+    GwIn in;
+    in.d_frames = d_frames; in.n_frames = n_frames; in.hb = hb; in.he = he; in.n_turns = n_turns;
+    in.P = P; in.h_ev_off = h_ev_off; in.d_seg_stats = d_seg_stats;
+    TRY(gw_check(c, in, GwOut(), true));
+    std::vector<int64_t>& first = c->step_first;
+    first.assign((size_t)n_prob + 1, n_turns);
+    for (int64_t t = 0, prev = -1; t < n_turns; ++t) {
+        const int64_t p = h_turn_problem[t];
+        if (p != prev && p != prev + 1) return fail(c, SPKD_EINVAL, "batch_step: a turn's problem must be its predecessor's or the next");
+        if (p >= n_prob) return fail(c, SPKD_EINVAL, "batch_step: problem index out of range");
+        if (p != prev) first[(size_t)p] = t;
+        prev = p;
+        if (h_turn_file_off[t] < 0 || h_turn_file_len[t] < 0 || h_turn_file_off[t] + h_turn_file_len[t] > n_frames)
+            return fail(c, SPKD_EINVAL, "batch_step: a turn's file lies outside the frame array");
+    }
+    if (h_turn_problem[n_turns - 1] != n_prob - 1) return fail(c, SPKD_EINVAL, "batch_step: a problem without a turn");
+    int path = A->path;
+    if (path != SPKD_AHC_MONO && path != SPKD_AHC_WIDE) path = n_prob <= 64 ? SPKD_AHC_WIDE : SPKD_AHC_MONO;
+    if (path != SPKD_AHC_MONO || n_prob > HO_MAX_PROB || c->hw_lines < n_prob) return SPKD_OK;
+    auto room = [](int64_t v) { return v + v / 8 + 64; };
+    HoCaps cap;
+    cap.lines = std::max<int64_t>(room(c->hw_lines), n_turns);
+    cap.redo = room(c->hw_redo);
+    cap.chunks = room(c->hw_chunks);
+    cap.cells = std::max<int64_t>(c->hw_cells + c->hw_cells / 4 + 1024, n_prob);
+    cap.n_max = std::min<int64_t>(room(c->hw_nmax), AHC_MAX_N);
+    cap.list = room(c->hw_list);
+    const size_t lds = (size_t)(cap.n_max + 4) * sizeof(int32_t);
+    if (lds > 150 * 1024) return SPKD_OK;
+    std::vector<TurnDesc> turns;
+    int64_t n_cand;
+    TRY(build_turns(c, n_frames, hb, he, n_turns, P, h_ev_off, true, turns, n_cand));
+    if (!c->side) {
+        if (hipStreamCreateWithFlags(&c->side, hipStreamNonBlocking) != hipSuccess) {
+            c->side = nullptr;
+            return fail(c, SPKD_EHIP, "batch_step: no stream for the result copies");
+        }
+        for (hipEvent_t& e : c->ev_side) HIPCHK(c, hipEventCreateWithFlags(&e, hipEventDisableTiming));
+    }
+    const size_t nl = (size_t)cap.lines, nr = (size_t)cap.redo, np = (size_t)n_prob, nt = (size_t)n_turns;
+    void *hm = nullptr, *ho_out = nullptr;
+    TRY(pinned(c, PIN_STEP_MISC, (HO_N + np + 1 + 3 * nr + 5 * nl) * sizeof(int64_t) + (nl + nt) * sizeof(int32_t), &hm));
+    int64_t* h_ho = (int64_t*)hm;
+    int64_t* h_seg = h_ho + HO_N;
+    int64_t* h_redo = h_seg + np + 1;
+    double* h_times = (double*)(h_redo + 3 * nr);
+    int64_t* h_fb = (int64_t*)(h_times + 2 * nl);
+    int64_t* h_ix = h_fb + 2 * nl;
+    int32_t* h_tn = (int32_t*)(h_ix + nl);
+    int32_t* h_nwin = h_tn + nl;
+    TRY(pinned(c, PIN_AHC_OUT, (nl + 2 * np) * sizeof(double) + (3 * nl + np) * sizeof(int32_t), &ho_out));
+    double* md = (double*)ho_out;
+    int32_t* ma = (int32_t*)(md + nl + 2 * np);
+    int32_t* mb = ma + nl;
+    int32_t* lab = mb + nl;
+    int32_t* nm = lab + nl;
+    unsigned long long cnt2[2] = {0ull, 0ull};
+    for (int i = 0; i < HO_N; ++i) h_ho[i] = -1;
+
+    Call call(c);
+    TRY(call.opened);
+    spkd_cd_params Pk = *P;
+    TRY(use_kind(c, P->kind, &Pk.kind));
+    spkd_ahc_params Ak = *A;
+    {
+        double* const pinv_gw = c->pinv_cur;
+        TRY(use_kind(c, A->kind, &Ak.kind));
+        if (pinv_gw != c->pinv_cur) return fail(c, SPKD_EINVAL, "batch_step: both stages with the pseudo-inverse or neither");
+    }
+    void* p = nullptr;
+    TRY(scratch(c, S_HO_TURNS, (2 * nt + np + 1) * sizeof(int64_t) + nt * sizeof(int32_t), &p));
+    int64_t* d_foff = (int64_t*)p;
+    int64_t* d_flen = d_foff + nt;
+    int64_t* d_first = d_flen + nt;
+    int32_t* d_tprob = (int32_t*)(d_first + np + 1);
+    HIPCHK(c, hipMemcpyAsync(d_foff, h_turn_file_off, nt * sizeof(int64_t), hipMemcpyHostToDevice, c->stream));
+    HIPCHK(c, hipMemcpyAsync(d_flen, h_turn_file_len, nt * sizeof(int64_t), hipMemcpyHostToDevice, c->stream));
+    HIPCHK(c, hipMemcpyAsync(d_first, first.data(), (np + 1) * sizeof(int64_t), hipMemcpyHostToDevice, c->stream));
+    HIPCHK(c, hipMemcpyAsync(d_tprob, h_turn_problem, nt * sizeof(int32_t), hipMemcpyHostToDevice, c->stream));
+    TRY(scratch(c, S_HO_COUNTS, HO_N * sizeof(int64_t), &p));
+    int64_t* d_ho = (int64_t*)p;
+    HIPCHK(c, hipMemsetAsync(d_ho, 0, HO_N * sizeof(int64_t), c->stream));
+    TRY(scratch(c, S_HO_LINES, nl * (2 * sizeof(int64_t) + sizeof(int32_t)), &p));
+    int64_t* d_rb = (int64_t*)p;
+    int64_t* d_re = d_rb + nl;
+    int32_t* d_moved = (int32_t*)(d_re + nl);
+    TRY(scratch(c, S_HO_REDO, 3 * nr * sizeof(int64_t), &p));
+    int64_t* d_redo = (int64_t*)p;
+    void *d_t = nullptr, *d_l = nullptr, *d_redo_stats = nullptr, *d_partial = nullptr, *d_chunks = nullptr, *d_setoff = nullptr;
+    TRY(scratch(c, S_CP_TIMES, nl * 2 * sizeof(double), &d_t));
+    TRY(scratch(c, S_CP_LINES, nl * (3 * sizeof(int64_t) + sizeof(int32_t)), &d_l));
+    int64_t* d_fb = (int64_t*)d_l;
+    int64_t* d_ix = d_fb + 2 * nl;
+    int32_t* d_tn = (int32_t*)(d_ix + nl);
+    TRY(scratch(c, S_REDO_STATS, (nr + 1) * REC * sizeof(double), &d_redo_stats));
+    TRY(scratch(c, S_CHUNKS, (size_t)cap.chunks * sizeof(Chunk), &d_chunks));
+    TRY(scratch(c, S_SETOFF, (nr + 1) * sizeof(int64_t), &d_setoff));
+    TRY(scratch(c, S_PARTIAL, (size_t)cap.chunks * REC * sizeof(double), &d_partial));
+    AhcBuffers B;
+    TRY(scratch(c, S_AHC_OFF, 3 * (np + 1) * sizeof(int64_t), &p));
+    B.seg_off = (int64_t*)p;
+    B.mat_off = B.seg_off + np + 1;
+    int64_t* d_slot = B.mat_off + np + 1;
+    TRY(scratch(c, S_AHC_PROB, (nl + (size_t)cap.list * HO_XCDS) * sizeof(int32_t), &p));
+    int32_t* d_prob = (int32_t*)p;
+    int32_t* d_sched = d_prob + nl;
+    TRY(scratch(c, S_AHC_LD, nl * sizeof(double), &p));
+    B.ld = (double*)p;
+    TRY(scratch(c, S_AHC_AUX, nl * AUX * sizeof(double), &p));
+    B.aux = (double*)p;
+    TRY(scratch(c, S_AHC_MAT, (size_t)cap.cells * sizeof(double), &p));
+    B.mat = (double*)p;
+    TRY(scratch(c, S_AHC_MISC, np * 2 * sizeof(unsigned long long), &p));
+    B.smax = (unsigned long long*)p;
+    B.smin = B.smax + n_prob;
+    HIPCHK(c, hipMemsetAsync(B.smax, 0x00, np * sizeof(unsigned long long), c->stream));
+    HIPCHK(c, hipMemsetAsync(B.smin, 0xff, np * sizeof(unsigned long long), c->stream));
+    TRY(scratch(c, S_AHC_STATS, nl * QREC * sizeof(double), &p));
+    B.ex = (double*)p;
+    TRY(scratch(c, S_AHC_PACKED, nl * REC * sizeof(double), &p));
+    B.pk = (double*)p;
+    void* op = nullptr;
+    TRY(scratch(c, S_AHC_OUT, nl * (6 * sizeof(int32_t) + 3 * sizeof(double)) + np * (sizeof(int32_t) + 2 * sizeof(double)) + 64, &op));
+    double* d_merge_d = (double*)op;
+    double* d_tmp = d_merge_d + nl;
+    double* d_rmin = d_tmp + nl;
+    double* d_fmax = d_rmin + nl;
+    double* d_fmin = d_fmax + np;
+    int32_t* d_a = (int32_t*)(d_fmin + np);
+    int32_t* d_b = d_a + nl;
+    int32_t* d_alive = d_b + nl;
+    int32_t* d_rcache = d_alive + nl;
+    int32_t* d_n = d_rcache + 3 * nl;
+
+    GwBatch G;
+    G.turn_start_s = h_turn_start_s;
+    G.turn_end_s = h_turn_end_s;
+    GwDev dv;
+    TRY(gw_enqueue(c, in, 0, &Pk, turns, n_cand, &G, dv));
+    const unsigned tblocks = (unsigned)((n_turns + CP_TPB - 1) / CP_TPB), lblocks = (unsigned)((cap.lines + CP_TPB - 1) / CP_TPB);
+    const int64_t* d_n_lines = G.d_line_off + n_turns;
+    hipLaunchKernelGGL(k_cp_count, dim3(tblocks), dim3(CP_TPB), 0, c->stream, (const TurnDesc*)dv.d_turns, n_turns,
+                       (const int32_t*)dv.d_i32a, (const int32_t*)dv.d_i32b, (const int*)c->d_err, G.d_n_det, G.d_pos);
+    hipLaunchKernelGGL(k_cp_scan, dim3(1), dim3(CP_SCAN_TPB), 0, c->stream, (const int32_t*)G.d_n_det, n_turns,
+                       (const int*)c->d_err, G.d_line_off);
+    hipLaunchKernelGGL(k_cp_lines, dim3(tblocks), dim3(CP_TPB), 0, c->stream, (const TurnDesc*)dv.d_turns, n_turns,
+                       (const int32_t*)G.d_n_det, (const int32_t*)G.d_pos, (const int64_t*)G.d_line_off, cap.lines,
+                       (const double*)dv.d_d1, (const double*)dv.d_d2, (const double*)dv.d_d4, (const double*)G.d_ls,
+                       (const double*)G.d_le, Pk.rate, (const int*)c->d_err, (double*)d_t, d_fb, d_fb + nl, d_ix, d_tn);
+    hipLaunchKernelGGL(k_ho_roundtrip, dim3(lblocks), dim3(CP_TPB), 0, c->stream, d_n_lines, cap.lines, (const int*)c->d_err,
+                       (double*)d_t, (const int64_t*)d_fb, (const int64_t*)(d_fb + nl), (const int32_t*)d_tn,
+                       (const int64_t*)d_foff, (const int64_t*)d_flen, Pk.rate, (flags & SPKD_STEP_FORCE_SLOW) ? 1 : 0,
+                       d_rb, d_re, d_moved, d_ho);
+    HIPCHK(c, hipGetLastError());
+    c->side_used = true;
+    HIPCHK(c, hipEventRecord(c->ev_side[0], c->stream));
+    HIPCHK(c, hipStreamWaitEvent(c->side, c->ev_side[0], 0));
+    HIPCHK(c, hipMemcpyAsync(h_times, d_t, nl * 2 * sizeof(double), hipMemcpyDeviceToHost, c->side));
+    HIPCHK(c, hipMemcpyAsync(h_fb, d_fb, nl * 2 * sizeof(int64_t), hipMemcpyDeviceToHost, c->side));
+    HIPCHK(c, hipMemcpyAsync(h_tn, d_tn, nl * sizeof(int32_t), hipMemcpyDeviceToHost, c->side));
+    HIPCHK(c, hipMemcpyAsync(h_nwin, dv.d_i32a, nt * sizeof(int32_t), hipMemcpyDeviceToHost, c->side));
+    if (flags & SPKD_STEP_WANT_INDEX)
+        HIPCHK(c, hipMemcpyAsync(h_ix, d_ix, nl * sizeof(int64_t), hipMemcpyDeviceToHost, c->stream));
+    hipLaunchKernelGGL(k_ho_redo, dim3(1), dim3(HO_TPB), 0, c->stream, d_n_lines, (const int*)c->d_err, cap,
+                       (const int32_t*)d_moved, (const int64_t*)d_rb, (const int64_t*)d_re, d_redo, d_redo + nr,
+                       d_redo + 2 * nr, (Chunk*)d_chunks, (int64_t*)d_setoff, d_ix, d_ho);
+    hipLaunchKernelGGL(k_ho_problems, dim3(1), dim3(HO_TPB), 0, c->stream, (const int64_t*)G.d_line_off, n_turns,
+                       (const int*)c->d_err, cap, (const int64_t*)d_first, (int)n_prob, B.seg_off, B.mat_off, d_slot,
+                       d_sched, B.mat, d_ho);
+    hipLaunchKernelGGL(k_ho_sched, dim3(lblocks), dim3(CP_TPB), 0, c->stream, (const int64_t*)d_ho, (int)n_prob,
+                       (const int32_t*)d_tn, (const int32_t*)d_tprob, (const int64_t*)B.seg_off, (const int64_t*)d_slot,
+                       d_prob, d_sched);
+    HIPCHK(c, hipGetLastError());
+    HIPCHK(c, hipEventRecord(c->ev_side[1], c->stream));
+    HIPCHK(c, hipStreamWaitEvent(c->side, c->ev_side[1], 0));
+    HIPCHK(c, hipMemcpyAsync(h_ho, d_ho, HO_N * sizeof(int64_t), hipMemcpyDeviceToHost, c->side));
+    HIPCHK(c, hipMemcpyAsync(h_seg, B.seg_off, (np + 1) * sizeof(int64_t), hipMemcpyDeviceToHost, c->side));
+    HIPCHK(c, hipMemcpyAsync(h_redo, d_redo, 3 * nr * sizeof(int64_t), hipMemcpyDeviceToHost, c->side));
+    if (cap.chunks > 0) {
+        Timer t(c, SPKD_T_CHUNK_STATS);
+        hipLaunchKernelGGL(k_chunk_stats, dim3((unsigned)cap.chunks), dim3(STATS_TPB), 0, c->stream, d_frames,
+                           (const Chunk*)d_chunks, (double*)d_partial);
+    }
+    {
+        Timer t(c, SPKD_T_REDUCE_SETS);
+        hipLaunchKernelGGL(k_reduce_sets, dim3((unsigned)cap.redo), dim3(STATS_TPB), 0, c->stream,
+                           (const double*)d_partial, (const int64_t*)d_setoff, (double*)d_redo_stats);
+    }
+    hipLaunchKernelGGL(k_records_from_map_dev, dim3((unsigned)cap.lines), dim3(256), 0, c->stream, (const double*)d_seg_stats,
+                       dv.n_ev, (const int64_t*)d_ix, (const double*)d_redo_stats, (const int64_t*)d_ho, B.ex, B.pk, c->d_err);
+    {
+        const int64_t per_block = Ak.kind == SPKD_KL2 ? PT_WAVES : 4 * PT_WAVES;
+        Timer t(c, SPKD_T_CLUSTER_PREP);
+        hipLaunchKernelGGL(k_cluster_prep, dim3((unsigned)((cap.lines + per_block - 1) / per_block)), dim3(PT_WAVES * WAVE), 0,
+                           c->stream, (const double*)B.ex, (int64_t)0, Ak.kind, B.ld, B.aux, c->d_err, c->pinv_cur,
+                           (const int64_t*)(d_ho + HO_N_EFF));
+    }
+    {
+        auto kmat = Ak.kind == SPKD_GLR ? k_matrix<true> : k_matrix<false>;
+        Timer t(c, SPKD_T_MATRIX);
+        hipLaunchKernelGGL(kmat, dim3((unsigned)(cap.list * HO_XCDS)), dim3(MX_WAVES * WAVE), 0, c->stream,
+                           (const double*)B.ex, (const double*)B.pk, (const int64_t*)B.seg_off, (const int32_t*)d_prob,
+                           (const int32_t*)d_sched, Ak.variant, Ak.kind, Ak.lambdac, (const double*)B.ld,
+                           (const double*)B.aux, B.mat, (const int64_t*)B.mat_off, B.smax, B.smin, c->d_err);
+    }
+    {
+        auto kahc = Ak.kind == SPKD_GLR ? k_ahc<true> : k_ahc<false>;
+        if (lds > 48 * 1024)
+            (void)hipFuncSetAttribute((const void*)kahc, hipFuncAttributeMaxDynamicSharedMemorySize, (int)lds);
+        Timer t(c, SPKD_T_AHC);
+        hipLaunchKernelGGL(kahc, dim3((unsigned)n_prob), dim3(AHC_TPB), lds, c->stream,
+                           B.ex, B.pk, (const int64_t*)B.seg_off, Ak.variant, Ak.kind, Ak.max_spk, Ak.lambdac,
+                           Ak.threshold, B.ld, B.aux, B.mat, (const int64_t*)B.mat_off, d_alive, d_tmp,
+                           d_rmin, d_rcache, d_n, d_a, d_b, d_merge_d, B.smax, B.smin, d_fmax, d_fmin, c->d_err,
+                           c->pinv_cur);
+    }
+    HIPCHK(c, hipGetLastError());
+    HIPCHK(c, hipMemcpyAsync(nm, d_n, np * sizeof(int32_t), hipMemcpyDeviceToHost, c->stream));
+    HIPCHK(c, hipMemcpyAsync(ma, d_a, nl * sizeof(int32_t), hipMemcpyDeviceToHost, c->stream));
+    HIPCHK(c, hipMemcpyAsync(mb, d_b, nl * sizeof(int32_t), hipMemcpyDeviceToHost, c->stream));
+    HIPCHK(c, hipMemcpyAsync(md, d_merge_d, nl * sizeof(double), hipMemcpyDeviceToHost, c->stream));
+    HIPCHK(c, hipMemcpyAsync(cnt2, c->d_counter, sizeof cnt2, hipMemcpyDeviceToHost, c->stream));
+    const spkd_status st = call.finish();
+    c->last_gw_items = (int64_t)cnt2[1];
+    const int status = (int)(h_ho[HO_STATUS] & 0xffffffff);
+    if (status & HO_SLOW) { res->fallback = SPKD_STEP_SLOW_PATH; return SPKD_OK; }
+    if (st != SPKD_OK) return st;
+    if (status) { res->fallback = SPKD_STEP_CAPACITY; return SPKD_OK; }
+    const int64_t n = h_ho[HO_N_LINES], n_redo = h_ho[HO_N_REDO];
+    if (n < n_turns || n > cap.lines || h_ho[HO_N_EFF] != n || h_seg[n_prob] != n || n_redo < 0 || n_redo > cap.redo)
+        return fail(c, SPKD_EHIP, "internal error: the hand-off's counts do not agree");
+    if (spkd_labels_from_merges_batch(n_prob, h_seg, nm, ma, mb, lab) != SPKD_OK)
+        return fail(c, SPKD_EHIP, "internal error: merge log does not replay");
+    c->hw_lines = n;
+    c->hw_redo = n_redo;
+    c->hw_chunks = h_ho[HO_N_CHUNKS];
+    c->hw_cells = h_ho[HO_CELLS];
+    c->hw_nmax = h_ho[HO_N_MAX];
+    c->hw_list = h_ho[HO_LONGEST];
+    view->n_lines = n;
+    view->n_redo = n_redo;
+    view->n_win = h_nwin;
+    view->times = h_times;
+    view->turn = h_tn;
+    view->frame_b = h_fb;
+    view->frame_e = h_fb + nl;
+    view->index = (flags & SPKD_STEP_WANT_INDEX) ? h_ix : nullptr;
+    view->d_index = d_ix;
+    view->redo_line = h_redo;
+    view->redo_begin = h_redo + nr;
+    view->redo_end = h_redo + 2 * nr;
+    res->fallback = SPKD_STEP_DONE;
+    res->seg_off = h_seg;
+    res->n_merges = nm;
+    res->merge_a = ma;
+    res->merge_b = mb;
+    res->merge_d = md;
+    res->labels = lab;
     return SPKD_OK;
 }
 
@@ -1408,61 +1733,26 @@
     return call.finish();
 }
 
-static const double kPow10[23] = {1e0, 1e1, 1e2, 1e3, 1e4, 1e5, 1e6, 1e7, 1e8, 1e9, 1e10, 1e11,
-                                  1e12, 1e13, 1e14, 1e15, 1e16, 1e17, 1e18, 1e19, 1e20, 1e21, 1e22};
-static const uint64_t kPow10u[20] = {1ull, 10ull, 100ull, 1000ull, 10000ull, 100000ull, 1000000ull,
-                                     10000000ull, 100000000ull, 1000000000ull, 10000000000ull,
-                                     100000000000ull, 1000000000000ull, 10000000000000ull,
-                                     100000000000000ull, 1000000000000000ull, 10000000000000000ull,
-                                     100000000000000000ull, 1000000000000000000ull,
-                                     10000000000000000000ull};
-
-static bool roundtrip_fast(double x, double* out) {
-    if (!(x >= 1e-3 && x < 1e11)) return false;
-    int e10 = (int)std::floor(std::log10(x));
-    if (e10 < -3) e10 = -3;
-    if (e10 >= 0) { if (x < kPow10[e10]) --e10; else if (e10 + 1 <= 22 && x >= kPow10[e10 + 1]) ++e10; }
-    else { if (x * kPow10[-e10] < 1.0) --e10; else if (x * kPow10[-e10 - 1] >= 1.0) ++e10; }
-    if (e10 < -3 || e10 > 10) return false;
-    int s = 11 - e10;
-    int k;
-    const double fr = std::frexp(x, &k);
-    const uint64_t m = (uint64_t)std::ldexp(fr, 53);
-    k -= 53;
-    unsigned __int128 prod = (unsigned __int128)m * kPow10u[s];
-    uint64_t q;
-    if (k >= 0) {
-        if (k > 20) return false;
-        q = (uint64_t)(prod << k);
-    } else {
-        const int sh = -k;
-        if (sh >= 120) return false;
-        const unsigned __int128 one = 1;
-        const unsigned __int128 fl = prod >> sh;
-        const unsigned __int128 remn = prod & ((one << sh) - 1);
-        const unsigned __int128 half = one << (sh - 1);
-        q = (uint64_t)fl;
-        if (remn > half || (remn == half && (q & 1))) ++q;
-    }
-    if (q >= 1000000000000ull) {
-        if (q != 1000000000000ull) return false;
-        q = 100000000000ull;
-        s -= 1;
-    } else if (q < 100000000000ull) {
-        return false;
-    }
-    *out = s >= 0 ? (double)q / kPow10[s] : (double)q * kPow10[-s];
-    return true;
-}
-
 static void roundtrip_range(double* v, int64_t lo, int64_t hi) {
     char buf[64];
     for (int64_t i = lo; i < hi; ++i) {
         double r;
-        if (roundtrip_fast(v[i], &r)) { v[i] = r; continue; }
+        if (py2_roundtrip_fast(v[i], &r)) { v[i] = r; continue; }
         std::snprintf(buf, sizeof buf, "%.12g", v[i]);
         v[i] = std::strtod(buf, nullptr);
     }
+}
+
+int64_t spkd_py2_roundtrip_rule(const double* v, int64_t n, double* out, int32_t* decided) {
+    if (n < 0 || (n > 0 && (!v || !out || !decided))) return -1;
+    int64_t cnt = 0;
+    for (int64_t i = 0; i < n; ++i) {
+        double r = v[i];
+        decided[i] = py2_roundtrip_fast(v[i], &r) ? 1 : 0;
+        out[i] = r;
+        cnt += decided[i];
+    }
+    return cnt;
 }
 
 void spkd_py2_roundtrip(double* v, int64_t n) {
diff --git a/speaker-diarization_amd/hipabi.py b/speaker-diarization_amd/hipabi.py
--- a/speaker-diarization_amd/hipabi.py
+++ b/speaker-diarization_amd/hipabi.py
@@ -17,8 +17,8 @@
 EXPORTS = ['spkd_abi_version', 'spkd_create', 'spkd_create_on_stream', 'spkd_destroy', 'spkd_last_error', 'spkd_sync',
            'spkd_malloc', 'spkd_free', 'spkd_memcpy_h2d', 'spkd_memcpy_d2h', 'spkd_memcpy_d2d',
            'spkd_last_kernel_ms', 'spkd_last_gw_items', 'spkd_set_stats', 'spkd_pair_terms',
-           'spkd_distance_matrix', 'spkd_gw_event_capacity', 'spkd_gw_event_capacity_p', 'spkd_gw', 'spkd_gw_ex', 'spkd_gw_fused', 'spkd_gw_batch', 'spkd_ahc_fused', 'spkd_gather_stats', 'spkd_mfcc',
-           'spkd_sw_window_count', 'spkd_sw', 'spkd_ahc', 'spkd_ahc_matrix', 'spkd_distance_rows', 'spkd_cluster_in', 'spkd_py2_roundtrip',
+           'spkd_distance_matrix', 'spkd_gw_event_capacity', 'spkd_gw_event_capacity_p', 'spkd_gw', 'spkd_gw_ex', 'spkd_gw_fused', 'spkd_gw_batch', 'spkd_ahc_fused', 'spkd_batch_step', 'spkd_gather_stats', 'spkd_mfcc',
+           'spkd_sw_window_count', 'spkd_sw', 'spkd_ahc', 'spkd_ahc_matrix', 'spkd_distance_rows', 'spkd_cluster_in', 'spkd_py2_roundtrip', 'spkd_py2_roundtrip_rule',
            'spkd_labels_from_merges', 'spkd_labels_from_merges_batch', 'spkd_count_flags', 'spkd_gw_lines',
            'spkd_gmm_loglik', 'spkd_vad_viterbi']
 
@@ -42,7 +42,14 @@
                 ('redo_end', C.c_void_p)]
 
 
+class BatchStepResult(C.Structure):
+    _fields_ = [('fallback', C.c_int32), ('reserved', C.c_int32), ('seg_off', C.c_void_p), ('n_merges', C.c_void_p),
+                ('merge_a', C.c_void_p), ('merge_b', C.c_void_p), ('merge_d', C.c_void_p), ('labels', C.c_void_p)]
+
+
 AHC_AUTO, AHC_MONO, AHC_WIDE = 0, 1, 2
+STEP_WANT_INDEX, STEP_FORCE_SLOW = 1, 2
+STEP_DONE, STEP_NOT_APPLICABLE, STEP_CAPACITY, STEP_SLOW_PATH = range(4)
 
 
 class MfccParams(C.Structure):
@@ -156,6 +163,10 @@
     lib.spkd_gw_batch.argtypes = [vp, vp, i64, vp, vp, i64, P(CdParams), vp, vp, vp, vp, vp, vp, C.c_int, P(GwLinesView)]
     lib.spkd_ahc_fused.argtypes = [vp, vp, i64, vp, i64, vp, vp, i64, vp, vp, vp, i64, P(AhcParams),
                                    P(vp), P(vp), P(vp), P(vp), P(vp)]
+    lib.spkd_batch_step.argtypes = [vp, vp, i64, vp, vp, i64, P(CdParams), vp, vp, vp, vp, vp, vp, i64, vp, P(AhcParams),
+                                    C.c_int, P(GwLinesView), P(BatchStepResult)]
+    lib.spkd_py2_roundtrip_rule.argtypes = [vp, i64, vp, vp]
+    lib.spkd_py2_roundtrip_rule.restype = i64
     lib.spkd_gather_stats.argtypes = [vp, vp, i64, vp, vp, i64, i64, vp]
     lib.spkd_mfcc.argtypes = [vp, vp, i64, P(MfccParams), vp, vp, vp, vp, vp, vp, P(i64)]
     lib.spkd_sw_window_count.argtypes = [i64, dbl, dbl]
@@ -196,6 +207,15 @@
     if v.size:
         load_library().spkd_py2_roundtrip(_ptr(v), v.size)
     return v
+
+
+def py2_roundtrip_rule(values):
+    v = np.ascontiguousarray(values, dtype=np.float64)
+    out = np.empty_like(v)
+    decided = np.zeros(v.size, dtype=np.int32)
+    if v.size and load_library().spkd_py2_roundtrip_rule(_ptr(v), v.size, _ptr(out), _ptr(decided)) < 0:
+        raise SpkdError(SPKD_EINVAL, 'py2_roundtrip_rule')
+    return out, decided.astype(bool)
 
 
 def labels_from_merges(n, a, b):
@@ -473,6 +493,9 @@
             if st != SPKD_EOVERFLOW:
                 break
         self.check(st, allow=(SPKD_ENONFINITE,))
+        return self._lines_dict(st, off, nev, d_seg, view, nt, want_index)
+
+    def _lines_dict(self, st, off, nev, d_seg, view, nt, want_index):
         n, nr = int(view.n_lines), int(view.n_redo)
         return dict(status=st, off=off, n_ev=nev, d_seg=d_seg, n_lines=n, n_win=_view(view.n_win, nt if n else 0, np.int32),
                     times=_view(view.times, 2 * n, np.float64).reshape(-1, 2), turn=_view(view.turn, n, np.int32),
@@ -480,6 +503,38 @@
                     index=_view(view.index, n, np.int64) if want_index else None, d_index=view.d_index,
                     redo_line=_view(view.redo_line, nr, np.int64), redo_begin=_view(view.redo_begin, nr, np.int64),
                     redo_end=_view(view.redo_end, nr, np.int64))
+
+    def batch_step(self, d_frames, n_frames, begins, ends, params, turn_start_s, turn_end_s, file_off, file_len,
+                   turn_problem, n_problems, seg_stats, ahc_params, tight=True, first_guess_scale=1.0,
+                   want_index=False, force_slow=False):
+        force_slow = force_slow or getattr(self, 'step_force_slow', False)
+        c = np.ascontiguousarray
+        b = c(begins, dtype=np.int64)
+        e = c(ends, dtype=np.int64)
+        nt = len(b)
+        host = [c(turn_start_s, dtype=np.float64), c(turn_end_s, dtype=np.float64), c(file_off, dtype=np.int64),
+                c(file_len, dtype=np.int64), c(turn_problem, dtype=np.int32)]
+        if any(len(a) != nt for a in host):
+            raise SpkdError(SPKD_EINVAL, 'one entry per turn')
+        off = next(_gw_capacity_ladder(e - b, params, tight, first_guess_scale))
+        nev = int(off[-1])
+        d_seg = seg_stats(nev)
+        view, res = GwLinesView(), BatchStepResult()
+        flags = (STEP_WANT_INDEX if want_index else 0) | (STEP_FORCE_SLOW if force_slow else 0)
+        st = self.lib.spkd_batch_step(self.h, C.c_void_p(d_frames), n_frames, _ptr(b), _ptr(e), nt, C.byref(params),
+                                      _ptr(off), *[_ptr(a) for a in host], int(n_problems), C.c_void_p(d_seg),
+                                      C.byref(ahc_params), flags, C.byref(view), C.byref(res))
+        count = self.__dict__.setdefault('step_fallbacks', {})
+        key = 'status_%d' % st if st != SPKD_OK else ('done', 'not_applicable', 'capacity', 'slow_path')[res.fallback]
+        count[key] = count.get(key, 0) + 1
+        if st != SPKD_OK or res.fallback != STEP_DONE:
+            return None
+        lines = self._lines_dict(st, off, nev, d_seg, view, nt, want_index)
+        npb, n = int(n_problems), lines['n_lines']
+        return lines, dict(status=st, seg_off=_view(res.seg_off, npb + 1, np.int64),
+                           n_merges=_view(res.n_merges, npb, np.int32), a=_view(res.merge_a, n, np.int32),
+                           b=_view(res.merge_b, n, np.int32), d=_view(res.merge_d, n, np.float64),
+                           labels=_view(res.labels, n, np.int32))
 
     def ahc_fused(self, d_frames, n_frames, d_records, n_records, d_line_index, seg_off, redo_line, redo_begin,
                   redo_end, params):
diff --git a/speaker-diarization_amd/pipeline.py b/speaker-diarization_amd/pipeline.py
--- a/speaker-diarization_amd/pipeline.py
+++ b/speaker-diarization_amd/pipeline.py
@@ -218,20 +218,31 @@
     owner, foff, fn, ls, le, tb, te = table
     ls, le = np.ascontiguousarray(ls), np.ascontiguousarray(le)
     p = _cd_params(cd, rate)
+    ap = _ahc_params(cl)
+    seg_alloc = lambda n_rec: ctx.dev_scratch('fused_segment_stats', max(n_rec, 1) * hipabi.REC * 8)
+    turn_problem = np.cumsum(np.concatenate(([0], owner[1:] != owner[:-1]))).astype(np.int32)
     _t1 = time.perf_counter()
-    r = ctx.gw_batch(d_frames, total_frames, tb, te, p, ls, le, foff, fn,
-                     lambda n_rec: ctx.dev_scratch('fused_segment_stats', max(n_rec, 1) * hipabi.REC * 8),
-                     tight=True, first_guess_scale=first_guess_scale, want_index=detail is not None)
-    _t2 = time.perf_counter()
-    _detector_done(ctx, timings, tb, te, r)
-    line_file = owner[r['turn']]
-    bounds = np.searchsorted(line_file, np.arange(len(files) + 1))
-    _t3 = time.perf_counter()
-    seg_off = _problems(np.diff(bounds))[1]
-    ap = _ahc_params(cl)
-    _t4 = time.perf_counter()
-    a = ctx.ahc_fused(d_frames, total_frames, r['d_seg'], r['n_ev'], r['d_index'], seg_off, r['redo_line'],
-                      r['redo_begin'], r['redo_end'], ap)
+    step = ctx.batch_step(d_frames, total_frames, tb, te, p, ls, le, foff, fn, turn_problem, int(turn_problem[-1]) + 1,
+                          seg_alloc, ap, tight=True, first_guess_scale=first_guess_scale, want_index=detail is not None)
+    if step is not None:
+        r, a = step
+        _t2 = _t3 = _t4 = time.perf_counter()
+        _detector_done(ctx, timings, tb, te, r)
+        line_file = owner[r['turn']]
+        bounds = np.searchsorted(line_file, np.arange(len(files) + 1))
+        seg_off = a['seg_off']
+    else:
+        r = ctx.gw_batch(d_frames, total_frames, tb, te, p, ls, le, foff, fn, seg_alloc,
+                         tight=True, first_guess_scale=first_guess_scale, want_index=detail is not None)
+        _t2 = time.perf_counter()
+        _detector_done(ctx, timings, tb, te, r)
+        line_file = owner[r['turn']]
+        bounds = np.searchsorted(line_file, np.arange(len(files) + 1))
+        _t3 = time.perf_counter()
+        seg_off = _problems(np.diff(bounds))[1]
+        _t4 = time.perf_counter()
+        a = ctx.ahc_fused(d_frames, total_frames, r['d_seg'], r['n_ev'], r['d_index'], seg_off, r['redo_line'],
+                          r['redo_begin'], r['redo_end'], ap)
     _t5 = time.perf_counter()
     if timings is not None:
         _time_stats(ctx, timings, r['n_lines'], r['redo_begin'], r['redo_end'])
```

New measurement: 1463, median of 6. No clear change (+0.5%).
